# bendalab/audian

Hardware: AMD Instinct MI355X
Metric: Msamples/s spectrogram+bandpass, 64ch x 96kHz (higher is better)
Workload: dtype f32 I/O, f64 IIR state; 1 GPU; BASELINE configs[2]: synthetic 64 ch/GPU x 600 s x 96 kHz float32; bandpass 300-3000 Hz order 2 -> spectrogram nfft 2048 hop 1024 + envelope 20 Hz; channels_per_gpu=64, frames=57600000, spectrogram_frames=56250, parallelism=channel shard x1, streams=one compute stream, envelope_forward=state checkpoints, fused into the band-pass kernel, envelope_buffer=best of 4 allocations by memset time (hipdsp_malloc_probed), spectrogram=FFT waves inside the forward sweep (filtered tiles from LDS)

## Files before the change

audian_amd/_lib.py:

```python

import ctypes
import os

_HERE = os.path.dirname(os.path.abspath(__file__))
LIB_PATH = os.environ.get('AUDIAN_AMD_LIB') or os.path.join(_HERE, 'libhip_dsp.so')

OK, ERR_INVALID, ERR_HIP, ERR_UNSUPPORTED, ERR_TOO_SHORT, ERR_NOMEM = range(6)
MAX_SECTIONS = 4


class HipDspError(RuntimeError):

    def __init__(self, status, message):
        super().__init__(f'libhip_dsp error {status}: {message}')
        self.status = status


if not os.path.exists(LIB_PATH) and os.path.exists('/opt/rocm/bin/hipcc') and \
   os.environ.get('AUDIAN_AMD_NO_AUTOBUILD') != '1':
    import subprocess as _sp
    try:
        _sp.check_call(['make', '-C', os.path.join(_HERE, 'csrc'), '-j4', '-s'])
    except Exception:
        pass

if not os.path.exists(LIB_PATH):
    raise ImportError(
        f'{LIB_PATH} is missing: build the HIP extension first '
        '(`make -C audian_amd/csrc` or `python -c "import __graft_entry__ as g; g.build()"`). '
        'audian_amd has no CPU fallback.')

import sys as _sys
if 'torch' not in _sys.modules and (int(os.environ.get('WORLD_SIZE', '1')) > 1 or
                                    os.environ.get('AUDIAN_AMD_TORCH') == '1'):
    import torch as _torch

lib = ctypes.CDLL(LIB_PATH)


def hip_runtime_path():
    with open('/proc/self/maps') as f:
        return sorted({ln.split()[-1] for ln in f if 'libamdhip64' in ln})

_vp = ctypes.c_void_p
_i64 = ctypes.c_int64
_int = ctypes.c_int
_dbl = ctypes.c_double
_sz = ctypes.c_size_t
_pp = ctypes.POINTER(ctypes.c_void_p)

_SIGNATURES = {
    'hipdsp_version': ([], _int),
    'hipdsp_last_error': ([], ctypes.c_char_p),
    'hipdsp_device_count': ([ctypes.POINTER(_int)], _int),
    'hipdsp_ctx_create': ([_int, _vp, _pp], _int),
    'hipdsp_ctx_destroy': ([_vp], _int),
    'hipdsp_ctx_set_stream': ([_vp, _vp], _int),
    'hipdsp_ctx_synchronize': ([_vp], _int),
    'hipdsp_ctx_set_max_segments': ([_vp, _int], _int),
    'hipdsp_ctx_set_option': ([_vp, ctypes.c_char_p, ctypes.c_longlong], _int),
    'hipdsp_ctx_reserve': ([_vp, _sz], _int),
    'hipdsp_ctx_set_mid_event': ([_vp, _vp], _int),
    'hipdsp_stream_create': ([_vp, _pp], _int),
    'hipdsp_stream_destroy': ([_vp, _vp], _int),
    'hipdsp_graph_begin': ([_vp], _int),
    'hipdsp_graph_end': ([_vp, _pp], _int),
    'hipdsp_graph_launch': ([_vp, _vp], _int),
    'hipdsp_graph_destroy': ([_vp, _vp], _int),
    'hipdsp_malloc': ([_vp, _sz, _pp], _int),
    'hipdsp_malloc_probed': ([_vp, _sz, _int, _pp], _int),
    'hipdsp_free': ([_vp, _vp], _int),
    'hipdsp_pool_stats': ([_vp, ctypes.POINTER(_sz), ctypes.POINTER(ctypes.c_uint64), ctypes.POINTER(ctypes.c_uint64)], _int),
    'hipdsp_pool_trim': ([_vp], _int),
    'hipdsp_memset': ([_vp, _vp, _int, _sz], _int),
    'hipdsp_memcpy_h2d': ([_vp, _vp, _vp, _sz], _int),
    'hipdsp_memcpy_d2h': ([_vp, _vp, _vp, _sz], _int),
    'hipdsp_memcpy_d2d': ([_vp, _vp, _vp, _sz], _int),
    'hipdsp_host_malloc': ([_vp, _sz, _pp], _int),
    'hipdsp_host_free': ([_vp, _vp], _int),
    'hipdsp_memcpy_h2d_async': ([_vp, _vp, _vp, _sz], _int),
    'hipdsp_memcpy2d_d2d': ([_vp, _vp, _sz, _vp, _sz, _sz, _sz], _int),
    'hipdsp_event_create': ([_vp, _pp], _int),
    'hipdsp_event_destroy': ([_vp, _vp], _int),
    'hipdsp_event_record': ([_vp, _vp], _int),
    'hipdsp_event_wait': ([_vp, _vp], _int),
    'hipdsp_event_elapsed_ms': ([_vp, _vp, _vp, ctypes.POINTER(ctypes.c_float)], _int),
    'hipdsp_pack_f64': ([_vp, _vp, _vp, _i64, _i64, _i64], _int),
    'hipdsp_pack_f32': ([_vp, _vp, _vp, _i64, _i64, _i64], _int),
    'hipdsp_unpack_f64': ([_vp, _vp, _i64, _vp, _i64, _i64], _int),
    'hipdsp_unpack_spectrum_f64': ([_vp, _vp, _i64, _vp, _i64, _i64, _i64], _int),
    'hipdsp_sosplan_create': ([_vp, _pp], _int),
    'hipdsp_sosplan_destroy': ([_vp, _vp], _int),
    'hipdsp_sosplan_set': ([_vp, _vp, _vp, _int], _int),
    'hipdsp_sosplan_set_host': ([_vp, _vp, _vp, _int], _int),
    'hipdsp_sosplan_upload': ([_vp, _vp], _int),
    'hipdsp_sos_plan_host': ([_vp, _int, ctypes.POINTER(_i64), ctypes.POINTER(_int), _vp], _int),
    'hipdsp_sos_segments_host': ([_i64, _int, _int, _int, _i64, _i64, _i64, ctypes.POINTER(_i64), ctypes.POINTER(_int)], _int),
    'hipdsp_sosplan_info': ([_vp, _vp, ctypes.POINTER(_i64), ctypes.POINTER(_int)], _int),
    'hipdsp_sosfilt': ([_vp, _vp, _vp, _i64, _vp, _i64, _i64, _i64, _i64], _int),
    'hipdsp_envelope': ([_vp, _vp, _vp, _i64, _vp, _i64, _i64, _i64, _i64, _int, _dbl, _int], _int),
    'hipdsp_envelope_multi': ([_vp, _vp, _int, _vp, _i64, _vp, _i64, _i64, _i64, _i64, _int, _dbl, _int], _int),
    'hipdsp_sosfilt_envelope': ([_vp, _vp, _vp, _vp, _i64, _vp, _i64, _vp, _i64, _i64, _i64, _int, _dbl, _int, _int, _i64], _int),
    'hipdsp_chain_forward': ([_vp, _vp, _vp, _vp, _i64, _vp, _i64, _i64, _i64, _int, _dbl, _int, _int, _dbl, _vp, _vp, _i64, _i64, _i64,
                              _i64, _i64], _int),
    'hipdsp_chain_backward': ([_vp, _vp, _vp, _i64, _vp, _i64, _i64, _i64, _int, _dbl, _int, _int, _int, _dbl, _vp, _i64, _i64], _int),
    'hipdsp_chain_backward_plan': ([_vp, _vp, _i64, _i64, ctypes.POINTER(_i64), ctypes.POINTER(_i64), ctypes.POINTER(_int)], _int),
    'hipdsp_chain_plan': ([_vp, _vp, _vp, _i64, _i64, ctypes.POINTER(_i64), ctypes.POINTER(_int)], _int),
    'hipdsp_spectrogram': ([_vp, _vp, _i64, _i64, _i64, _int, _int, _dbl, _vp, _vp, _i64, _i64], _int),
    'hipdsp_decibel': ([_vp, _vp, _vp, _i64, _dbl, _dbl], _int),
    'hipdsp_decibel_image': ([_vp, _vp, _vp, _i64, _i64, _dbl, _dbl], _int),
    'hipdsp_decibel_image_decimate': ([_vp, _vp, _vp, _i64, _i64, _i64, _i64, _i64, _dbl, _dbl], _int),
    'hipdsp_channel_mean': ([_vp, _vp, _i64, ctypes.POINTER(_int), _int, _i64, _i64, _dbl, _vp], _int),
    'hipdsp_stride_copy': ([_vp, _vp, _i64, _i64, _vp], _int),
    'hipdsp_max_nonneg': ([_vp, _vp, _i64, _vp], _int),
    'hipdsp_band_order_stats': ([_vp, _vp, _i64, _i64, _i64, _i64, _vp], _int),
    'hipdsp_unwrap': ([_vp, _vp, _i64, _i64, _i64, _dbl, _dbl, _int, _int, _vp, _i64], _int),
    'hipdsp_pcm_unpack': ([_vp, _vp, _int, _i64, _i64, _dbl, _vp, _i64], _int),
    'hipdsp_minmax_decimate': ([_vp, _vp, _i64, _i64, _i64, _i64, _i64, _vp, _i64], _int),
    'hipdsp_pcm_minmax': ([_vp, _vp, _int, _i64, _i64, _i64, _dbl, _dbl, _dbl, _int, _int, _vp, _i64], _int),
    'hipdsp_mean_spectrum_db': ([_vp, _vp, _i64, _i64, _i64, _dbl, _dbl, _dbl, _vp], _int),
    'hipdsp_comm_unique_id': ([_vp], _int),
    'hipdsp_comm_create': ([_vp, _vp, _int, _int, _pp], _int),
    'hipdsp_comm_destroy': ([_vp, _vp], _int),
    'hipdsp_allgather_f32': ([_vp, _vp, _vp, _vp, _i64], _int),
    'hipdsp_copy_probe': ([_vp, _vp, _vp, _sz], _int),
    'hipdsp_synth': ([_vp, _vp, _i64, _i64, _i64, _dbl, ctypes.c_uint64, _i64, _i64], _int),
}

for _name, (_args, _res) in _SIGNATURES.items():
    _fn = getattr(lib, _name)
    _fn.argtypes = _args
    _fn.restype = _res


def last_error():
    return lib.hipdsp_last_error().decode('utf-8', 'replace')


def check(status):
    if status == OK:
        return
    msg = last_error()
    if status == ERR_TOO_SHORT:
        raise ValueError(msg)
    if status == ERR_UNSUPPORTED:
        raise NotImplementedError(msg)
    if status == ERR_NOMEM:
        raise MemoryError(msg)
    if status == ERR_INVALID:
        raise ValueError(msg)
    raise HipDspError(status, msg)
```

audian_amd/csrc/chain.hip:

```cpp
#include "chain_fwd.h"

namespace {

__global__ __launch_bounds__(256) void env_nan_fill_kernel(const double *__restrict__ ckpt, long long ckpt_pitch, long long n_tiles,
                                                           int DE, float *__restrict__ env, long long env_pitch, long long T)
{
    const long long ch = blockIdx.y;
    const double *e = ckpt + ch * ckpt_pitch + n_tiles * DE;
    bool bad = false;
    for (int r = 0; r < DE; r++) bad = bad || !(fabs(e[r]) <= 1.7976931348623157e308);
    if (!bad) return;
    for (long long i = (long long)blockIdx.x * blockDim.x + threadIdx.x; i < T; i += (long long)gridDim.x * blockDim.x)
        env[ch * env_pitch + i] = __builtin_nanf("");
}

struct ChainBwdArgs {
    BwdArgs b;
    float *psd;
    long long psd_pitch;
    long long n_valid;
    const float *tables;
    float scale;
    long long units;
    int debug;
// ... 183 lines not shown
            if (rt >= rt_lo) {
                if (tile + TILE <= T) {
#pragma unroll
                    for (int k = 0; k < 8; k++) {
                        float4 v = lds[lds_slot(8 * k + (lane >> 3), lane & 7)];
                        if (a.b.clamp) {
                            v.x = fmaxf(v.x, 0.f); v.y = fmaxf(v.y, 0.f); v.z = fmaxf(v.z, 0.f); v.w = fmaxf(v.w, 0.f);
                        }
                        f4u t; t.x = v.x; t.y = v.y; t.z = v.z; t.w = v.w;
                        *reinterpret_cast<f4u *>(out + (tile + 256 * k + 4 * lane)) = t;
                    }
                    asm volatile("s_waitcnt vmcnt(7)" ::: "memory");
                } else {
#pragma unroll
                    for (int k = 0; k < 8; k++) {
                        float4 v = lds[lds_slot(8 * k + (lane >> 3), lane & 7)];
                        if (a.b.clamp) {
                            v.x = fmaxf(v.x, 0.f); v.y = fmaxf(v.y, 0.f); v.z = fmaxf(v.z, 0.f); v.w = fmaxf(v.w, 0.f);
                        }
                        store_four(out, tile + 256 * k + 4 * lane, v, 0, T, 0);
                    }
                    asm volatile("s_waitcnt vmcnt(0)" ::: "memory");
                }
            } else {
                asm volatile("s_waitcnt vmcnt(0)" ::: "memory");
            }
            WAVE_SYNC();
        }
        asm volatile("s_waitcnt vmcnt(0)" ::: "memory");
    } else {
        __builtin_amdgcn_s_setprio(3);
        float2 *fb = fbs[pair];
        const float *tlf = reinterpret_cast<const float *>(tiles[pair]);
        const float2 *tw2 = tab, *tw3 = tab + TW2, *twn = tab + TW2 + TW3, *win = tab + TW2 + TW3 + TWN;
        float *oc = a.psd + ch * a.psd_pitch;
        v2f cur_[16], nxt_[8];
#pragma unroll
        for (int j = 0; j < 16; j++) cur_[j] = (v2f){0.f, 0.f};
#pragma unroll
        for (int j = 0; j < 8; j++) nxt_[j] = (v2f){0.f, 0.f};
        bool have_next = false;
        float piv = 0.f;
        bool have_piv = false;
        int it = 0;
        for (long long rt = rt_start; rt < rt_hi; rt++) {
            it++;
            const long long tidx = a.b.n_tiles - 1 - rt;
            CHAIN_WAIT_FOR(ready, it, it);
#pragma unroll
            for (int j = 0; j < 16; j++)
                cur_[j] = *reinterpret_cast<const v2f *>(tlf + lds_float_index(2 * lane + 128 * j));
            {
                const bool withhold = (a.debug & 8) && blockIdx.x == 0 && pair == 0 && rt == rt_start;
                if (!withhold) CHAIN_POST(taken, it);
            }
            const long long f = 2 * tidx + 1;
            if (rt >= rt_lo && have_next && f < a.n_valid) {
                v2f w[16];
#pragma unroll
                for (int i = 0; i < 8; i++) { w[i] = cur_[8 + i]; w[8 + i] = nxt_[i]; }
                psd_frame_pivot<NFFT, 64, R1, R2, R3, false>(w, fb, tw2, tw3, twn, win, lane, PsdScale{a.scale, 0.5f * a.scale, 2.f * a.scale}, true,
                                                             bin_sink<false>(oc + f * (long long)F, nullptr, 0), piv, have_piv);
            }
#pragma unroll
            for (int j = 0; j < 8; j++) nxt_[j] = cur_[j];
            have_next = true;
        }
    }
}

#undef CHAIN_WAIT_FOR
#undef CHAIN_POST
#undef CHAIN_FAIR

}

extern "C" {

int hipdsp_chain_forward(hipdsp_ctx *ctx, const hipdsp_sosplan *fplan, const hipdsp_sosplan *eplan,
                         const float *x, int64_t x_pitch, float *yf, int64_t yf_pitch, int64_t channels,
                         int64_t frames, int rectify, double gain, int nfft, int hop, double fs, float *psd,
                         float *db_out, int64_t frames_out, int64_t psd_pitch, int64_t spec_frames,
                         int64_t spec_first, int64_t env_first)
{
    HD_REQUIRE(ctx != nullptr && fplan != nullptr, "NULL argument");
    HD_REQUIRE(channels >= 0 && frames >= 0 && frames_out >= 0, "negative size");
    HD_REQUIRE(frames_out < (1LL << 31) - (1LL << 16), "frames_out %lld: the fused sweep counts frames in 32 bits", (long long)frames_out);
    HD_REQUIRE(spec_first >= 0 && spec_first <= frames, "spec_first %lld not in [0, frames=%lld]", (long long)spec_first,
               (long long)frames);
    HD_REQUIRE(spec_frames >= 0 && spec_first + spec_frames <= frames, "spec_first %lld + spec_frames %lld beyond frames=%lld",
               (long long)spec_first, (long long)spec_frames, (long long)frames);
    HD_REQUIRE(env_first >= 0 && env_first <= frames, "env_first %lld not in [0, frames=%lld]", (long long)env_first,
               (long long)frames);
    HD_REQUIRE(fs > 0, "fs must be positive");
    const int SF = fplan->host->n_sections, SE = eplan ? eplan->host->n_sections : 0;
    HD_REQUIRE(SF > 0 && (SE > 0 || eplan == nullptr), "plan has no coefficients");
    const bool shape_ok = (nfft == 2048 && (hop == 1024 || hop == 512)) || (nfft == 1024 && (hop == 512 || hop == 256)) ||
                          (nfft == 512 && hop == 256) || (nfft == 256 && hop == 128);
    if (!shape_ok || SF > 4 || SE > 2 || frames < 4 * TILE ||
        fplan->host->warm >= (1LL << 40) || (eplan && eplan->host->warm >= (1LL << 40))) {
        hipdsp_set_error("the fused forward sweep covers nfft/hop 2048/1024, 2048/512, 1024/512, 1024/256, 512/256 and 256/128, a band-pass of "
                         "at most four and an envelope of at most two sections that decay, and traces of at least %d "
                         "frames: use hipdsp_sosfilt_envelope + hipdsp_spectrogram", 4 * TILE);
        return HIPDSP_ERR_UNSUPPORTED;
    }
    HD_CHECK_HIP(hipSetDevice(ctx->device));
    {
        const int frc = hd_device_fault(ctx);
        if (frc != HIPDSP_OK) return frc;
    }
    const int edge = eplan ? eplan->host->edge : 0;
    if (eplan && frames - env_first <= edge) {
        hipdsp_set_error("The length of the input vector x must be greater than padlen, which is %d.", edge);
        return HIPDSP_ERR_TOO_SHORT;
    }
    if (channels == 0) return HIPDSP_OK;
    HD_REQUIRE(channels <= 65535, "more than 65535 channels");
    HD_REQUIRE(x != nullptr && yf != nullptr && (psd != nullptr || frames_out == 0), "NULL data pointer");
    HD_REQUIRE(x_pitch >= frames && yf_pitch >= frames, "pitch smaller than row length");
    HD_NO_OVERLAP(x, x_pitch, frames, yf, yf_pitch, frames, channels, "x and yf");
    const long long F = nfft / 2 + 1;
    if (psd_pitch == 0) psd_pitch = frames_out * F;
    HD_REQUIRE(psd_pitch >= frames_out * F, "psd_pitch smaller than one channel");
    const long long sframes = spec_frames > 0 ? spec_frames : frames - spec_first;
    long long nsource = (frames_out - 1) * (long long)hop + nfft;
    if (nsource > sframes) nsource = sframes;
    long long n_valid = 0;
    if (frames_out > 0 && nsource >= nfft) n_valid = (nsource - (nfft - hop)) / hop;
    if (n_valid > frames_out) n_valid = frames_out;
    double wss = 0.0;
    for (int i = 0; i < nfft; i++) {
        const double w = 0.5 - 0.5 * cos(2.0 * M_PI * (double)i / (double)nfft);
        wss += w * w;
    }
    ChainArgs a;
    memset(&a, 0, sizeof(a));
    int rc = hd_fft_tables(ctx, nfft, &a.tables);
    if (rc != HIPDSP_OK) return rc;
    const GridShift gs = hd_grid_shift(spec_first, env_first, hop, edge, SE > 0);
    HD_REQUIRE(gs.lead < TILE, "grid shift %lld", gs.lead);
    const long long T = frames + gs.lead;
    const long long n_tiles = (T + edge + TILE - 1) / TILE;
    const long long ckpt_pitch = (n_tiles + 1) * 2 * SE;
    void *work = nullptr;
    if (SE > 0) {
        rc = hipdsp_scratch(ctx, sizeof(double) * (size_t)ckpt_pitch * (size_t)channels, &work);
        if (rc != HIPDSP_OK) return rc;
    }
    hd_note_sweep(ctx, gs.lead, gs.env0, frames, channels, SE);
    a.c.in = x - gs.lead; a.c.yf = yf - gs.lead; a.c.ckpt = (double *)work;
    a.c.in_pitch = x_pitch; a.c.yf_pitch = yf_pitch; a.c.ckpt_pitch = ckpt_pitch;
    a.c.T = T; a.c.edge = edge; a.c.rectify = rectify; a.c.gain = rectify ? gain : 1.0;
    a.c.lead = gs.lead; a.c.env0 = gs.env0; a.frame_off = gs.frame_off;
    a.psd = psd; a.db = db_out; a.psd_pitch = psd_pitch; a.n_valid = n_valid;
    a.scale = (float)(1.0 / (fs * wss));
    a.scale_half = 0.5f * a.scale; a.scale_twice = 2.f * a.scale;
    a.warm_total = fplan->host->warm;
    a.debug = ctx->chain_debug;
    a.fault = ctx->fault_dev;
    a.split = (ctx->chain_split_frames && nfft == 2048 && hop == 1024 && !db_out && gs.lead == 0 && gs.env0 == 0) ? 1 : 0;
    constexpr int P = CHAIN_P;
    plan_segments_chain(ctx, T, channels, a.warm_total, &a.c.seg_len, &a.c.n_seg);
    a.units = channels * a.c.n_seg;
    if (a.c.n_seg > 1) {
        rc = hd_seg_flags(ctx, (size_t)a.units, &a.c.flags);
        if (rc != HIPDSP_OK) return rc;
    }
    a.n_iter = (int)((a.warm_total + a.c.seg_len + edge + TILE - 1) / TILE) + 1;
    long long blocks = (a.units + P - 1) / P;
    {
        const long long cus = ctx->n_cus - ctx->chain_reserve_cus > 0 ? ctx->n_cus - ctx->chain_reserve_cus : 1;
        if (a.units < cus * P) {
            blocks = a.units < cus ? a.units : cus;
            a.unit_stride = blocks;
        }
    }
    HD_REQUIRE(blocks <= 0x7fffffffLL, "grid too large");
    if (frames_out > n_valid && frames_out - n_valid <= 16 && !(ctx->chain_debug & 32)) {
        a.tail_end = frames_out;
    } else if (frames_out > n_valid) {
        const long long n = (frames_out - n_valid) * F;
        unsigned gx = (unsigned)((n + 1023) / 1024 > 4096 ? 4096 : (n + 1023) / 1024);
        hipLaunchKernelGGL(zero_rows_kernel, dim3(gx, (unsigned)channels), dim3(256), 0, ctx->stream,
                           psd + n_valid * F, (long long)psd_pitch, n, 0.f);
        if (db_out && !(ctx->chain_debug & 32))
            hipLaunchKernelGGL(zero_rows_kernel, dim3(gx, (unsigned)channels), dim3(256), 0, ctx->stream,
                               db_out + n_valid * F, (long long)psd_pitch, n, -INFINITY);
    }
    const SosPlanDev *edev_ = eplan ? eplan->dev : nullptr;
    const bool flags = (ctx->chain_debug & 4) == 0;
    const bool stamp = (ctx->chain_debug & 32) && db_out && SF == 2 && SE == 1 && flags && nfft == 2048 && hop == 1024;
    int (*launch)(int, int, int, int, int, unsigned, hipStream_t, const SosPlanDev *, const SosPlanDev *, const void *, size_t) =
        (nfft == 2048 && hop == 1024) ? hd_chain_fwd_launch_2048_1024 : (nfft == 2048) ? hd_chain_fwd_launch_2048_512 :
        (nfft == 1024 && hop == 512) ? hd_chain_fwd_launch_1024_512 : (nfft == 1024) ? hd_chain_fwd_launch_1024_256 :
        (nfft == 512) ? hd_chain_fwd_launch_512_256 : hd_chain_fwd_launch_256_128;
    if (launch(SF, SE, flags ? 1 : 0, (db_out && !stamp) ? 1 : 0, stamp ? 1 : 0, (unsigned)blocks, ctx->stream, fplan->dev, edev_,
               &a, sizeof(a)) != 0) {
        hipdsp_set_error("the barrier variant of the fused sweep is built for nfft 2048 / hop 1024 and plans of one or two sections");
        return HIPDSP_ERR_UNSUPPORTED;
    }
    if (stamp) return hd_launch_status("chain_fwd_kernel");
    rc = hd_launch_status("chain_fwd_kernel");
    if (rc != HIPDSP_OK) return rc;
    FloodArgs fl;
    memset(&fl, 0, sizeof(fl));
    fl.flags = a.c.flags; fl.n_seg = a.c.n_seg; fl.seg_len = a.c.seg_len;
    fl.y = yf; fl.y_pitch = yf_pitch; fl.T = T; fl.skip = gs.lead;
    fl.psd = psd; fl.db = db_out; fl.psd_pitch = psd_pitch; fl.n_valid = n_valid;
    fl.F = (int)F; fl.nfft = nfft; fl.hop = hop; fl.frame_off = gs.frame_off;
    if (SE == 0) return launch_flood(ctx, fl, channels);
    return hd_launch_env_fix(ctx, eplan->dev, SE, (double *)work, ckpt_pitch, channels, a.c.n_seg, a.c.seg_len, n_tiles, &fl,
                             (int)((gs.env0 - gs.env0 % TILE) / a.c.seg_len));
}

int hipdsp_chain_backward(hipdsp_ctx *ctx, const hipdsp_sosplan *eplan, const float *yf, int64_t yf_pitch, float *env,
                          int64_t env_pitch, int64_t channels, int64_t frames, int rectify, double gain, int clamp,
                          int nfft, int hop, double fs, float *psd, int64_t frames_out, int64_t psd_pitch)
{
    HD_REQUIRE(ctx != nullptr && eplan != nullptr, "NULL argument");
    HD_REQUIRE(channels >= 0 && frames >= 0 && frames_out >= 0, "negative size");
    HD_REQUIRE(fs > 0, "fs must be positive");
    const int SE = eplan->host->n_sections;
    HD_REQUIRE(SE > 0, "plan has no coefficients");
    if (nfft != 2048 || hop != 1024 || SE > 2 || frames < 4 * TILE || eplan->host->warm >= (1LL << 40)) {
        hipdsp_set_error("the backward sweep with the odd frames fused in covers nfft 2048 / hop 1024, envelope plans of at "
                         "most two decaying sections and traces of at least %d frames", 4 * TILE);
        return HIPDSP_ERR_UNSUPPORTED;
    }
    HD_CHECK_HIP(hipSetDevice(ctx->device));
    {
        const int frc = hd_device_fault(ctx);
        if (frc != HIPDSP_OK) return frc;
    }
    const int edge = eplan->host->edge;
    if (frames <= edge) {
        hipdsp_set_error("The length of the input vector x must be greater than padlen, which is %d.", edge);
        return HIPDSP_ERR_TOO_SHORT;
    }
    if (channels == 0) return HIPDSP_OK;
    HD_REQUIRE(channels <= 65535, "more than 65535 channels");
    HD_REQUIRE(yf != nullptr && env != nullptr && (psd != nullptr || frames_out == 0), "NULL data pointer");
    HD_REQUIRE(yf_pitch >= frames && env_pitch >= frames, "pitch smaller than row length");
    HD_NO_OVERLAP(yf, yf_pitch, frames, env, env_pitch, frames, channels, "yf and env");
    const long long F = nfft / 2 + 1;
    if (psd_pitch == 0) psd_pitch = frames_out * F;
    HD_REQUIRE(psd_pitch >= frames_out * F, "psd_pitch smaller than one channel");
    long long nsource = (frames_out - 1) * (long long)hop + nfft;
    if (nsource > frames) nsource = frames;
    long long n_valid = 0;
    if (frames_out > 0 && nsource >= nfft) n_valid = (nsource - (nfft - hop)) / hop;
    if (n_valid > frames_out) n_valid = frames_out;
    double wss = 0.0;
    for (int i = 0; i < nfft; i++) {
        const double w = 0.5 - 0.5 * cos(2.0 * M_PI * (double)i / (double)nfft);
        wss += w * w;
    }
    ChainBwdArgs a;
    memset(&a, 0, sizeof(a));
    int rc = hd_fft_tables(ctx, nfft, &a.tables);
    if (rc != HIPDSP_OK) return rc;
    const long long n_tiles = (frames + edge + TILE - 1) / TILE;
    const long long ckpt_pitch = (n_tiles + 1) * 2 * SE;
    void *work = nullptr;
    if (ctx->sweep_frames != frames || ctx->sweep_channels != channels || ctx->sweep_sections != SE ||
        ctx->sweep_lead != 0 || ctx->sweep_env0 != 0) {
        hipdsp_set_error("hipdsp_chain_backward: the last forward sweep on this context left tile states for %lld channels x "
                         "%lld frames, %d sections, grid shift %lld, envelope from %lld -- not for %lld x %lld, %d on the "
                         "unshifted grid (hipdsp_chain_forward with spec_first = env_first = 0)",
                         ctx->sweep_channels, ctx->sweep_frames, ctx->sweep_sections, ctx->sweep_lead, ctx->sweep_env0,
                         (long long)channels, (long long)frames, SE);
        return HIPDSP_ERR_INVALID;
    }
    rc = hd_scratch_parked(ctx, sizeof(double) * (size_t)ckpt_pitch * (size_t)channels, &work);
    if (rc != HIPDSP_OK) return rc;
    a.b.in = yf; a.b.in_pitch = yf_pitch;
    a.b.out = env; a.b.out_pitch = env_pitch;
    a.b.ckpt = (const double *)work; a.b.ckpt_pitch = ckpt_pitch;
    a.b.T = frames; a.b.skip = 0; a.b.n_tiles = n_tiles; a.b.edge = edge;
    a.b.rectify = rectify; a.b.clamp = clamp; a.b.gain = rectify ? gain : 1.0;
    constexpr int P = 8;
    long long seg_len = 0;
    plan_segments_chain(ctx, n_tiles * TILE, channels, eplan->host->warm, &seg_len, &a.b.n_seg);
    a.b.seg_tiles = seg_len / TILE;
    a.b.warm_tiles = eplan->host->warm / TILE;
    a.psd = psd; a.psd_pitch = psd_pitch; a.n_valid = n_valid;
    a.scale = (float)(1.0 / (fs * wss));
    a.units = channels * a.b.n_seg;
    a.debug = ctx->chain_debug;
    a.fault = ctx->fault_dev;
    const long long blocks = (a.units + P - 1) / P;
    HD_REQUIRE(blocks <= 0x7fffffffLL, "grid too large");
    dim3 grid((unsigned)blocks), block(128 * P);
    if (SE == 1) hipLaunchKernelGGL((chain_bwd_kernel<1, P>), grid, block, 0, ctx->stream, eplan->dev, a);
    else hipLaunchKernelGGL((chain_bwd_kernel<2, P>), grid, block, 0, ctx->stream, eplan->dev, a);
    rc = hd_launch_status("chain_bwd_kernel");
    if (rc != HIPDSP_OK) return rc;
    hipLaunchKernelGGL(env_nan_fill_kernel, dim3(64, (unsigned)channels), dim3(256), 0, ctx->stream, (const double *)work,
                       ckpt_pitch, n_tiles, 2 * SE, env, (long long)env_pitch, (long long)frames);
    return hd_launch_status("env_nan_fill_kernel");
}

int hipdsp_chain_backward_plan(hipdsp_ctx *ctx, const hipdsp_sosplan *eplan, int64_t channels, int64_t frames,
                               int64_t *first_border, int64_t *segment_frames, int *n_segments)
{
    HD_REQUIRE(ctx != nullptr && eplan != nullptr, "NULL argument");
    HD_REQUIRE(first_border != nullptr && segment_frames != nullptr && n_segments != nullptr, "NULL output");
    HD_REQUIRE(channels >= 1 && frames >= 1, "bad size");
    HD_REQUIRE(eplan->host->n_sections > 0, "plan has no coefficients");
    const long long n_tiles = (frames + eplan->host->edge + TILE - 1) / TILE;
    long long len = 0;
    int n = 0;
    plan_segments_chain(ctx, n_tiles * TILE, channels, eplan->host->warm, &len, &n);
    *first_border = n_tiles * TILE - len;
    *segment_frames = len;
    *n_segments = n;
    return HIPDSP_OK;
}

int hipdsp_chain_plan(hipdsp_ctx *ctx, const hipdsp_sosplan *fplan, const hipdsp_sosplan *eplan,
                      int64_t channels, int64_t frames, int64_t *segment_frames, int *n_segments)
{
    HD_REQUIRE(ctx != nullptr && fplan != nullptr, "NULL argument");
    HD_REQUIRE(segment_frames != nullptr && n_segments != nullptr, "NULL output");
    HD_REQUIRE(channels >= 1 && frames >= 1, "bad size");
    HD_REQUIRE(fplan->host->n_sections > 0 && (eplan == nullptr || eplan->host->n_sections > 0), "plan has no coefficients");
    long long len = 0;
    int n = 0;
    plan_segments_chain(ctx, frames, channels, fplan->host->warm, &len, &n);
    *segment_frames = len;
    *n_segments = n;
    return HIPDSP_OK;
}

}
```

audian_amd/csrc/chain_fwd.h:

```cpp
#pragma once
#include "sos_device.h"
#define STOCKHAM_SPLIT_MORE
#include "fft_device.h"
#include <cmath>

#define HD_CHAIN_FWD_DECL(n, h)                                                                                     \
    int hd_chain_fwd_launch_##n##_##h(int SF, int SE, int flags, int want_db, int stamp, unsigned blocks, hipStream_t stream, \
                                      const SosPlanDev *fdev, const SosPlanDev *edev, const void *args, size_t args_size)
HD_CHAIN_FWD_DECL(2048, 1024);
HD_CHAIN_FWD_DECL(2048, 512);
HD_CHAIN_FWD_DECL(1024, 512);
HD_CHAIN_FWD_DECL(1024, 256);
HD_CHAIN_FWD_DECL(512, 256);
HD_CHAIN_FWD_DECL(256, 128);
#undef HD_CHAIN_FWD_DECL

#ifdef CHAIN_AB_PLAIN_SUM
#define CHAIN_MSUM_ADD(x) do { } while (0)
#define CHAIN_MSUM_ON false
#else
#define CHAIN_MSUM_ADD(x) msum_ += (x)
#define CHAIN_MSUM_ON true
#endif

// ... 231 lines not shown
        const float pv = (l == 0) ? ph : pk_last;
        if (LPF == 64 || keep) {
            st_bin(out.psd, bo_h, 0, pv);
            if (DB) st_bin(out.db, bo_h, 0, to_db(pv));
        }
    }
}

#define FPT_OK(hop, g) ((2048 / (hop)) % (g) == 0)
#ifndef CHAIN_FFT_STORES
#define CHAIN_FFT_STORES 1
#endif
template <int SF, int SE, int NP, bool FLAGS, bool DB, int NFFT = 2048, int HOP = 1024, bool STAMP = false>
__global__ __launch_bounds__(128 * NP, NP / 2) void chain_fwd_kernel(const SosPlanDev *__restrict__ PF0,
                                                                   const SosPlanDev *__restrict__ PE0, ChainArgs a)
{
    static_assert(SF > 0 && SE >= 0 && NP % 2 == 0, "band-pass in front; whole waves per SIMD");
    constexpr int DF = 2 * SF, DE = SE > 0 ? 2 * SE : 1;
    static_assert((NFFT == 2048 || NFFT == 1024 || NFFT == 512 || NFFT == 256) && TILE % HOP == 0 && HOP % 128 == 0 &&
                  HOP <= NFFT && NFFT <= TILE, "frames must be register windows of a tile");
    static_assert(NFFT != 256 || HOP == 128, "256-sample frames: the reference's default, 50 % overlap");
    constexpr int M = NFFT / 2, F = M + 1, MP = M + M / 16;
    constexpr int LPF = NFFT >= 1024 ? 64 : (NFFT == 512 ? 32 : 16);
    constexpr int G = 64 / LPF;
    constexpr int R1 = NFFT == 2048 ? 16 : 8, R2 = NFFT == 256 ? 4 : R1, R3 = NFFT == 1024 ? 8 : 4;
    constexpr int TW2 = (R2 - 1) * R1, TW3 = R1 * R2, TWN = M / 2 + 1, NTAB = TW2 + TW3 + TWN + M;
    constexpr int PPL = NFFT / 128;
    static_assert(FPT_OK(HOP, G), "whole groups of frames per tile");
    constexpr int FPT = TILE / HOP;
    constexpr int PREV = (NFFT - HOP) / 128;
    constexpr bool FFT_STORES = CHAIN_FFT_STORES && FLAGS && G != 4;
    __shared__ float4 tiles[NP][64 * 8];
    __shared__ float rprevs[NP][64];
    __shared__ float2 fbs[NP][G * MP];
    __shared__ float2 tab[NTAB];
    __shared__ int ready[NP], taken[NP];
    __shared__ float2 fmeans[2][NP][16];
    __shared__ int prog[2 * NP];
    if (threadIdx.x < NP) { ready[threadIdx.x] = 0; taken[threadIdx.x] = 0; }
    if (threadIdx.x < 2 * NP) prog[threadIdx.x] = 0;
    const int tid = threadIdx.x;
    const int wave = __builtin_amdgcn_readfirstlane(tid >> 6);
    const int lane = tid & 63;
    const int pair = wave < NP ? wave : wave - NP;
#define CHAIN_FAIR(iter, behind_prio, ahead_prio)                                                        \
    do {                                                                                                 \
        if (FLAGS && !(a.debug & 128)) {                                                                 \
            if (lane == 0) __hip_atomic_store(&prog[wave], (iter), __ATOMIC_RELAXED, __HIP_MEMORY_SCOPE_WORKGROUP); \
            const int other_ = __builtin_amdgcn_readfirstlane(                                           \
                __hip_atomic_load(&prog[wave ^ (NP / 2)], __ATOMIC_RELAXED, __HIP_MEMORY_SCOPE_WORKGROUP)); \
            set_issue_priority(other_ < (iter) ? (ahead_prio) : (behind_prio));                          \
        }                                                                                                \
    } while (0)
    __shared__ int abort_wg;
    if (threadIdx.x == 0) abort_wg = 0;
    bool gave_up = false;
#define CHAIN_WAIT_FOR(arr, want, iter)                                             \
    do {                                                                            \
        if (!gave_up) {                                                             \
            for (int spin_ = 0;; spin_++) {                                         \
                if (__builtin_amdgcn_readfirstlane(__hip_atomic_load(&arr[pair], __ATOMIC_RELAXED, __HIP_MEMORY_SCOPE_WORKGROUP)) >= (want)) break; \
                if ((spin_ & 1023) == 1023) {                                       \
                    const bool told = __builtin_amdgcn_readfirstlane(__hip_atomic_load(&abort_wg, __ATOMIC_RELAXED, __HIP_MEMORY_SCOPE_WORKGROUP)) != 0; \
                    if (told || spin_ >= (1 << 23) - 1) {                           \
                        gave_up = true;                                             \
                        if (!told && lane == 0) {                                   \
                            __hip_atomic_store(&abort_wg, 1, __ATOMIC_RELAXED, __HIP_MEMORY_SCOPE_WORKGROUP); \
                            a.fault[1] = (int)blockIdx.x; a.fault[2] = pair; a.fault[3] = (iter); \
                            __hip_atomic_store(&a.fault[0], HD_FAULT_CHAIN_HANDOVER, __ATOMIC_RELEASE, __HIP_MEMORY_SCOPE_SYSTEM); \
                        }                                                           \
                        break;                                                      \
                    }                                                               \
                }                                                                   \
                __builtin_amdgcn_s_sleep(1);                                        \
            }                                                                       \
            __builtin_amdgcn_fence(__ATOMIC_ACQUIRE, "workgroup", "local");        \
        }                                                                           \
    } while (0)
#define CHAIN_POST(arr, value)                                                      \
    do {                                                                            \
        __builtin_amdgcn_fence(__ATOMIC_RELEASE, "workgroup", "local");            \
        if (lane == 0) __hip_atomic_store(&arr[pair], (value), __ATOMIC_RELAXED, __HIP_MEMORY_SCOPE_WORKGROUP); \
    } while (0)
    {
        const float2 *src = reinterpret_cast<const float2 *>(a.tables);
        for (int i = tid; i < NTAB; i += 128 * NP) tab[i] = src[i];
    }
    __syncthreads();

    const long long unit = a.unit_stride ? (long long)pair * a.unit_stride + blockIdx.x : (long long)blockIdx.x * NP + pair;
    const bool unit_ok = unit < a.units;
    const int seg = unit_ok ? (int)(unit % a.c.n_seg) : 0;
    const long long ch = unit_ok ? unit / a.c.n_seg : 0;
    const long long T = a.c.T;
    const int edge = a.c.edge;
    const long long lo = (long long)seg * a.c.seg_len;
    long long hi = lo + a.c.seg_len;
    const bool last_seg = hi >= T;
    if (hi > T) hi = T;
    const long long lead = a.c.lead;
    const long long env_tile0 = a.c.env0 - a.c.env0 % TILE;
    const bool env_true = lo <= env_tile0 && env_tile0 < hi;
    const long long env_start = env_true ? env_tile0 : (lo > env_tile0 ? lo : (1LL << 62));
    long long start = lo - PF0->warm;
    if (start < 0) start = 0;
    long long loop_end = last_seg ? T + edge : hi;
    if (!unit_ok) loop_end = start;
    const int TT = (int)(T / TILE);
    const int lo_t = (int)(lo / TILE), start_t = (int)(start / TILE), base_t = lo_t - (int)(a.warm_total / TILE);
    const int end_t = (int)((loop_end + TILE - 1) / TILE);
    const int hi_full_t = (int)(hi / TILE), hi_ceil_t = (int)((hi + TILE - 1) / TILE);
    const int lead_t = lead > 0 ? 1 : 0;
    const int env_start_t = env_start >= (1LL << 62) ? 0x7fffffff : (int)(env_start / TILE);

    const long long dbg_c0 = (a.debug & 16) ? clock64() : 0, dbg_w0 = (a.debug & 16) ? wall_clock64() : 0;
    long long st_acc[16];
#pragma unroll
    for (int i = 0; i < 16; i++) st_acc[i] = 0;
    long long st_last = STAMP ? clock64() : 0;
#define STAMP_AT(i)                                              \
    do {                                                         \
        if (STAMP) {                                             \
            const long long t_ = clock64();                      \
            st_acc[(i)] += t_ - st_last;                         \
            st_last = t_;                                        \
        }                                                        \
    } while (0)
    if (wave < NP) {
        float4 *lds = tiles[pair];
        float *ldsf = reinterpret_cast<float *>(lds);
        float *rprev = rprevs[pair];
        const float *in = a.c.in + ch * a.c.in_pitch;
        float *yf = a.c.yf + ch * a.c.yf_pitch;
        double *ckpt = SE > 0 ? a.c.ckpt + ch * a.c.ckpt_pitch : nullptr;
        double cf_[DF], ce_[DE];
#pragma unroll
        for (int r = 0; r < DF; r++) cf_[r] = 0.0;
#pragma unroll
        for (int r = 0; r < DE; r++) ce_[r] = 0.0;
        rprev[lane] = 0.f;
        double eprev_ = 0.0;
        v4f nx[8];
        bool pre = false;
        int pending = 0;
        const int top_full_t = TT - 1;
        auto fetch = [&](int t0) {
#pragma unroll
            for (int k = 0; k < 8; k++) nx[k] = asm_load16(in + (long long)t0 * TILE + 256 * k + 4 * lane);
        };
        auto prefetchable = [&](int t0) { return t0 >= start_t && t0 < end_t && t0 < TT && t0 >= lead_t; };
        pre = prefetchable(base_t);
        fetch(pre ? base_t : top_full_t);
        asm volatile("s_waitcnt vmcnt(0)" ::: "memory");

        for (int it = 0; it < a.n_iter; it++) {
            const int tt = base_t + it;
            const bool active = tt >= start_t && tt < end_t;
            if (!(a.debug & 64)) CHAIN_FAIR(it, 1, 0);
            if (FLAGS && pending) {
                CHAIN_WAIT_FOR(taken, pending, it);
                pending = 0;
            }
            if (active) {
                if (pre) {
#pragma unroll
                    for (int k = 0; k < 8; k++) {
                        asm volatile("" : "+v"(nx[k]));
                        lds[lds_slot(8 * k + (lane >> 3), lane & 7)] = make_float4(nx[k].x, nx[k].y, nx[k].z, nx[k].w);
                    }
                } else {
                    const long long tile = (long long)tt * TILE;
#pragma unroll 1
                    for (int k = 0; k < 8; k++) {
                        const long long p = tile + 256 * k + 4 * lane;
                        auto at = [&](long long q) { return in + (q < lead ? lead : (q < T ? q : T - 1)); };
                        auto ok = [&](long long q) { return q >= lead && q < T; };
                        v4f t;
                        t.x = asm_load4(at(p));
                        t.y = asm_load4(at(p + 1));
                        t.z = asm_load4(at(p + 2));
                        t.w = asm_load4(at(p + 3));
                        asm volatile("s_waitcnt vmcnt(0)" ::: "memory");
                        asm volatile("" : "+v"(t));
                        lds[lds_slot(8 * k + (lane >> 3), lane & 7)] =
                            make_float4(ok(p) ? t.x : 0.f, ok(p + 1) ? t.y : 0.f, ok(p + 2) ? t.z : 0.f, ok(p + 3) ? t.w : 0.f);
                    }
                }
            }
            WAVE_SYNC();
            {
                const int next = tt + 1;
                pre = prefetchable(next);
                fetch(pre ? next : top_full_t);
            }
            STAMP_AT(0);
            double etap[DE];
#pragma unroll
            for (int r = 0; r < DE; r++) etap[r] = 0.0;
            double msum_ = 0.0;
            if (active && !(a.debug & 2)) {
                const double tgain = a.c.gain;
                const SosPlanDev *PEt = PLAN_OF(SE > 0 ? PE0 : PF0);
#define CASC_S SF
#define CASC_PLAN() PLAN_OF(PF0)
#define CASC_CARRY cf_
#define CASC_IN(v) (v)
#define CASC_ROLLED_GROUPS
#define CASC_UNIT_OK (SF <= 2)
#define CASC_STAMP(n) STAMP_AT(1 + (n))
#define CASC_TAP(j, e, y)                                                               \
    do {                                                                                \
        const double ed_ = (double)(e);                                                 \
        CHAIN_MSUM_ADD(ed_);                                                            \
        if constexpr (SE > 0) {                                                         \
            if (((j) & 3) == 0) PEt = PLAN_OF(PE0);                                     \
            const double rd_ = fabs(ed_);                                               \
            _Pragma("unroll") for (int r_ = 0; r_ < DE; r_++) etap[r_] = fma(PEt->G[(j) * DE + r_], rd_, etap[r_]); \
        }                                                                               \
    } while (0)
#include "sos_cascade.inc"
#undef CASC_TAP
#undef CASC_STAMP
#undef CASC_UNIT_OK
#undef CASC_ROLLED_GROUPS
#undef CASC_S
#undef CASC_PLAN
#undef CASC_CARRY
#undef CASC_IN
#pragma unroll
                for (int r = 0; r < DE; r++) etap[r] *= tgain;
            }
            if (active && CHAIN_MSUM_ON) {
                constexpr int LR = NFFT / 32, HR = HOP / 32;
                const double pfx = wave_prefix_sum(msum_);
                const double tot = wave_read_lane63(pfx);
                const double yrot = (LR == 64 || lane >= 64 - LR) ? eprev_ : pfx;
                const double xrot = LR == 64 ? yrot : __shfl(yrot, (lane - LR) & 63, 64);
                const double mean = (pfx - xrot) * (1.0 / (double)NFFT);
                eprev_ = pfx - tot;
                const float mhi = (float)mean;
                const float mcorr = (float)((mean - (double)mhi) * (0.5 * (double)NFFT));
                if (((lane + 1) & (HR - 1)) == 0) fmeans[it & 1][pair][(lane + 1) / HR - 1] = make_float2(mhi, mcorr);
            }
            WAVE_SYNC();
            if (FLAGS) { if (active) CHAIN_POST(ready, it + 1); }
            else __syncthreads();
            if (FFT_STORES && active && tt >= lo_t && tt < hi_full_t && tt >= lead_t) {
                asm volatile("s_waitcnt vmcnt(0)" ::: "memory");
                STAMP_AT(4);
            } else if (active && tt >= lo_t && tt < hi_full_t && tt >= lead_t) {
#pragma unroll
                for (int k = 0; k < 8; k++) {
                    const float4 v = lds[lds_slot(8 * k + (lane >> 3), lane & 7)];
                    f4u t; t.x = v.x; t.y = v.y; t.z = v.z; t.w = v.w;
                    *reinterpret_cast<f4u *>(yf + (long long)tt * TILE + 256 * k + 4 * lane) = t;
                }
                asm volatile("s_waitcnt vmcnt(7)" ::: "memory");
                STAMP_AT(4);
            } else {
                if (active && tt >= lo_t && tt < hi_ceil_t) {
                    const long long tile = (long long)tt * TILE;
#pragma unroll
                    for (int k = 0; k < 8; k++)
                        store_four(yf, tile + 256 * k + 4 * lane, lds[lds_slot(8 * k + (lane >> 3), lane & 7)],
                                   lo > lead ? lo : lead, hi, 0);
                }
                asm volatile("s_waitcnt vmcnt(0)" ::: "memory");
            }
            const bool last_tile = tt + 1 >= end_t;
            const bool quiet = SE > 0 && active && tt >= env_start_t && a.c.rectify && tt + 1 < TT &&
                               !(env_true && tt == env_start_t) && (!last_tile || !last_seg) && !(a.debug & 2);
            if (FLAGS) {
                if (active) {
                    if (quiet || SE == 0 || tt < env_start_t) pending = it + 1;
                    else CHAIN_WAIT_FOR(taken, it + 1, it);
                }
            } else {
                __syncthreads();
            }
            if constexpr (SE > 0) {
            if (quiet) {
                if ((tt > lo_t || env_true) && lane == 0) {
#pragma unroll
                    for (int r = 0; r < DE; r++) ckpt[(long long)tt * DE + r] = ce_[r];
                }
#define CASC_S SE
#define CASC_PLAN() PLAN_OF(PE0)
#define CASC_CARRY ce_
#define CASC_IN(v) (v)
#define CASC_F_IN etap
#define CASC_NO_OUTPUT
#define CASC_ROLLED_GROUPS
#define CASC_STAMP(n) STAMP_AT(5 + (n))
#include "sos_cascade.inc"
#undef CASC_STAMP
#undef CASC_ROLLED_GROUPS
#undef CASC_NO_OUTPUT
#undef CASC_F_IN
#undef CASC_S
#undef CASC_PLAN
#undef CASC_CARRY
#undef CASC_IN
                if (last_tile && lane == 0) {
#pragma unroll
                    for (int r = 0; r < DE; r++) ckpt[(long long)(tt + 1) * DE + r] = ce_[r];
                }
                WAVE_SYNC();
            } else if (active && tt >= env_start_t && !(a.debug & 2)) {
                const long long tile = (long long)tt * TILE;
                if (a.c.rectify) {
#pragma unroll
                    for (int q = 0; q < 8; q++) {
                        float4 v = lds[lds_slot(lane, q)];
                        v = make_float4(fabsf(v.x), fabsf(v.y), fabsf(v.z), fabsf(v.w));
                        lds[lds_slot(lane, q)] = v;
                    }
                }
                WAVE_SYNC();
                auto rval = [&](long long j) -> float {
                    return j >= tile ? ldsf[lds_float_index((int)(j - tile))] : rprev[64 - (int)(tile - j)];
                };
                if (tt >= TT) {
                    float pv = 0.f;
                    long long pj = -1;
                    if (lane < edge) {
                        pj = T + lane;
                        if (pj >= tile && pj < tile + TILE) pv = 2.f * rval(T - 1) - rval(T - 2 - lane);
                    }
                    WAVE_SYNC();
                    if (lane < edge && pj >= tile && pj < tile + TILE) ldsf[lds_float_index((int)(pj - tile))] = pv;
                    WAVE_SYNC();
                }
                if (env_true && tt == env_start_t && a.c.env0 > 0) {
                    const SosPlanDev *Pz = PLAN_OF(PE0);
                    const float e0 = env_left_fill(ldsf, lane, (int)(a.c.env0 - tile), edge);
                    const double x0 = a.c.gain * (double)e0;
#pragma unroll
                    for (int r = 0; r < DE; r++) ce_[r] = Pz->zi[r] * x0;
                } else if (env_true && tt == env_start_t) {
                    const SosPlanDev *Pz = PLAN_OF(PE0);
                    const double r0 = (double)ldsf[lds_float_index(0)];
                    const double x0 = a.c.gain * (2.0 * r0 - (double)ldsf[lds_float_index(edge)]);
#pragma unroll
                    for (int r = 0; r < DE; r++) ce_[r] = Pz->zi[r] * x0;
                    for (int i = 0; i < edge; i++) {
                        double cur = a.c.gain * (2.0 * r0 - (double)ldsf[lds_float_index(edge - i)]);
#pragma unroll
                        for (int s2 = 0; s2 < SE; s2++) {
                            const double y = fma(Pz->coef[s2][0], cur, ce_[2 * s2]);
                            ce_[2 * s2] = fma(-Pz->coef[s2][3], y, fma(Pz->coef[s2][1], cur, ce_[2 * s2 + 1]));
                            ce_[2 * s2 + 1] = fma(-Pz->coef[s2][4], y, Pz->coef[s2][2] * cur);
                            cur = y;
                        }
                    }
                }
                if ((tt > lo_t || env_true) && lane == 0) {
#pragma unroll
                    for (int r = 0; r < DE; r++) ckpt[(long long)tt * DE + r] = ce_[r];
                }
                {
                    {
                        const float4 keep0 = lds[lds_slot(62 + ((lane >> 3) & 1), lane & 7)];
                        WAVE_SYNC();
                        if (lane < 16) {
                            rprev[4 * lane] = keep0.x; rprev[4 * lane + 1] = keep0.y;
                            rprev[4 * lane + 2] = keep0.z; rprev[4 * lane + 3] = keep0.w;
                        }
                    }
#define CASC_S SE
#define CASC_PLAN() PLAN_OF(PE0)
#define CASC_CARRY ce_
#define CASC_IN(v) (v)
#define CASC_GAIN a.c.gain
#define CASC_NO_OUTPUT
#define CASC_ROLLED_GROUPS
#include "sos_cascade.inc"
#undef CASC_ROLLED_GROUPS
#undef CASC_NO_OUTPUT
#undef CASC_GAIN
#undef CASC_S
#undef CASC_PLAN
#undef CASC_CARRY
#undef CASC_IN
                    if (last_tile && lane == 0) {
#pragma unroll
                        for (int r = 0; r < DE; r++) ckpt[(long long)(tt + 1) * DE + r] = ce_[r];
                    }
                }
                WAVE_SYNC();
            }
            }
        }
        asm volatile("s_waitcnt vmcnt(0)" ::: "memory");
        if (unit_ok && a.c.flags != nullptr && lane == 0) a.c.flags[unit] = state_not_finite(cf_) ? 1 : 0;
        STAMP_AT(7);
        if ((a.debug & 16) && blockIdx.x == 0 && wave == 0 && lane == 0) {
            long long *dbg = reinterpret_cast<long long *>(a.psd);
            dbg[0] = clock64() - dbg_c0;
            dbg[1] = wall_clock64() - dbg_w0;
        }
    } else {
        PsdScale fscale = {a.scale, a.scale_half, a.scale_twice};
        int foff = a.frame_off, fsplit = a.split, fdebug = a.debug, n_iter = a.n_iter;
        int nvalid = (int)a.n_valid;
        asm volatile("" : "+s"(fscale.one), "+s"(fscale.half), "+s"(fscale.twice), "+s"(foff), "+s"(fsplit), "+s"(fdebug),
                     "+s"(n_iter), "+s"(nvalid));
        if (!(fdebug & 64)) __builtin_amdgcn_s_setprio(3);
        float2 *fb = fbs[pair];
        const float *tlf = reinterpret_cast<const float *>(tiles[pair]);
        const float2 *tw2 = tab, *tw3 = tab + TW2, *twn = tab + TW2 + TW3, *win = tab + TW2 + TW3 + TWN;
        float *oc = a.psd + ch * a.psd_pitch;
        float *dc = DB ? a.db + ch * a.psd_pitch : nullptr;
        float *yfc = a.c.yf + ch * a.c.yf_pitch;
        const int st_lo_t = lo_t > lead_t ? lo_t : lead_t;
        v2f cur_[16], prv_[PREV > 0 ? PREV : 1];
#pragma unroll
        for (int j = 0; j < 16; j++) cur_[j] = (v2f){0.f, 0.f};
#pragma unroll
        for (int j = 0; j < (PREV > 0 ? PREV : 1); j++) prv_[j] = (v2f){0.f, 0.f};
        v2f bb_[G == 4 ? 20 : 1], pv_[4];
#pragma unroll
        for (int j = 0; j < 4; j++) pv_[j] = (v2f){0.f, 0.f};
        bool have_prev = false;
        for (int it = 0; it < n_iter; it++) {
            const int tt = base_t + it;
            const bool active = tt >= start_t && tt < end_t;
            if (!(fdebug & 64)) CHAIN_FAIR(it, 3, 2);
            if (FLAGS) { if (active) CHAIN_WAIT_FOR(ready, it + 1, it); }
            else __syncthreads();
            STAMP_AT(8);
            if (active) {
                if constexpr (G == 4) {
                    const int gq = lane >> 4, l16 = lane & 15;
#pragma unroll
                    for (int j = 0; j < 5; j++)
#pragma unroll
                        for (int tq = 0; tq < 4; tq++) {
                            const int b = 4 * gq - 1 + j;
// ... 119 lines not shown
```

audian_amd/csrc/common.h:

```cpp
#pragma once
#include <hip/hip_runtime.h>
#include <cstdarg>
#include <cstdint>
#include <cstdio>
#include <cstring>
#include "../../include/hip_dsp.h"

void hipdsp_set_error(const char *fmt, ...);

struct hipdsp_ctx {
    int device;
    hipStream_t stream;
    int max_segments;
    int n_cus;
    void *scratch;
    size_t scratch_bytes;
    hipEvent_t mid_event;
    void *fft_tables[20];
    int force_generic_fft;
    void *fft_tables2[20];
    int sos_waves_per_cu;
    int sos_waves_min;
    int chain_pairs;
    int sos_debug;
    int sos_single_wave_wg;
    int sos_prefetch;
    int spec_no_half;
    int spec_fpw, spec_kernel;
    int spec_debug;
    int chain_debug;
    int chain_split_frames;
    int chain_reserve_cus;
    long long *sos_trace;
    long long sos_trace_rows;
    int sos_fair;
    int sos_split;
    int sos_no_pin;
    struct hd_pool *pool;
    volatile int *fault_host;
    int *fault_dev;
    int graphs_alive;
    unsigned char *seg_flags;
    size_t seg_flags_cap;
    long long sweep_lead, sweep_env0, sweep_frames, sweep_channels;
    int sweep_sections;
};

int hd_seg_flags(hipdsp_ctx *ctx, size_t units, unsigned char **out);

#define HD_FAULT_CHAIN_HANDOVER 1
#define HD_FAULT_SPLIT_HANDOVER 2

int hd_device_fault(hipdsp_ctx *ctx);

struct hipdsp_graph {
    hipGraph_t graph;
    hipGraphExec_t exec;
};

#define HD_CHECK_HIP(expr)                                                        \
    do {                                                                          \
        hipError_t _e = (expr);                                                   \
        if (_e != hipSuccess) {                                                   \
            hipdsp_set_error("%s failed: %s (%s:%d)", #expr, hipGetErrorString(_e), \
                             __FILE__, __LINE__);                                 \
            return HIPDSP_ERR_HIP;                                                \
        }                                                                         \
    } while (0)

#define HD_REQUIRE(cond, ...)                                                     \
    do {                                                                          \
        if (!(cond)) {                                                            \
            hipdsp_set_error(__VA_ARGS__);                                        \
            return HIPDSP_ERR_INVALID;                                            \
        }                                                                         \
    } while (0)

static inline int hd_launch_status(const char *what)
{
    hipError_t e = hipGetLastError();
    if (e != hipSuccess) {
        hipdsp_set_error("launch of %s failed: %s", what, hipGetErrorString(e));
        return HIPDSP_ERR_HIP;
    }
    return HIPDSP_OK;
}

static inline bool hd_planar_overlap(const float *a, long long a_pitch, long long a_frames, const float *b, long long b_pitch,
                                     long long b_frames, long long channels)
{
    if (a == nullptr || b == nullptr || channels <= 0 || a_frames <= 0 || b_frames <= 0) return false;
    const char *a0 = (const char *)a, *a1 = (const char *)(a + (channels - 1) * a_pitch + a_frames);
    const char *b0 = (const char *)b, *b1 = (const char *)(b + (channels - 1) * b_pitch + b_frames);
    return a0 < b1 && b0 < a1;
}
#define HD_NO_OVERLAP(a, ap, af, b, bp, bf, channels, what)                                             \
    HD_REQUIRE(!hd_planar_overlap((a), (ap), (af), (b), (bp), (bf), (channels)), what " must not overlap")

int hipdsp_scratch(hipdsp_ctx *ctx, size_t bytes, void **out);
int hd_scratch_parked(hipdsp_ctx *ctx, size_t bytes, void **out);
int hd_fft_tables(hipdsp_ctx *ctx, int nfft, const float **dev);
```

audian_amd/csrc/ctx.hip:

```cpp
#include "common.h"
#include <map>
#include <unordered_map>
#include <vector>

static thread_local char g_err[512] = "";

struct hd_block {
    void *ptr;
    hipStream_t stream;
    hipEvent_t freed;
};

struct hd_pool {
    std::multimap<size_t, hd_block> cached;
    std::unordered_map<void *, size_t> live;
    std::vector<hipEvent_t> spare_events;
    size_t cached_bytes = 0;
    size_t limit = (size_t)1 << 30;
    size_t max_block = (size_t)256 << 20;
    unsigned long long hits = 0, misses = 0;
};

static void pool_trim(hd_pool *p)
{
    for (auto &kv : p->cached) {
        (void)hipFree(kv.second.ptr);
        if (kv.second.freed) p->spare_events.push_back(kv.second.freed);
    }
    p->cached.clear();
    p->cached_bytes = 0;
}

static void pool_destroy_events(hd_pool *p)
{
    for (hipEvent_t e : p->spare_events) (void)hipEventDestroy(e);
    p->spare_events.clear();
}

void hipdsp_set_error(const char *fmt, ...)
{
    va_list ap;
    va_start(ap, fmt);
    vsnprintf(g_err, sizeof(g_err), fmt, ap);
    va_end(ap);
}

extern "C" {

int hipdsp_version(void) { return HIPDSP_VERSION; }

const char *hipdsp_last_error(void) { return g_err; }

int hipdsp_device_count(int *count)
{
    HD_REQUIRE(count != nullptr, "count is NULL");
    HD_CHECK_HIP(hipGetDeviceCount(count));
    return HIPDSP_OK;
}

int hipdsp_ctx_create(int device, void *stream, hipdsp_ctx **out)
{
    HD_REQUIRE(out != nullptr, "out is NULL");
    *out = nullptr;
    int n = 0;
    HD_CHECK_HIP(hipGetDeviceCount(&n));
    HD_REQUIRE(device >= 0 && device < n, "device %d out of range (%d devices)", device, n);
    HD_CHECK_HIP(hipSetDevice(device));
    hipDeviceProp_t prop;
    HD_CHECK_HIP(hipGetDeviceProperties(&prop, device));
    if (strncmp(prop.gcnArchName, "gfx950", 6) != 0) {
        hipdsp_set_error("device %d is %s; libhip_dsp is built for gfx950 (MI355X) only",
                         device, prop.gcnArchName);
        return HIPDSP_ERR_UNSUPPORTED;
    }
    hipdsp_ctx *ctx = new hipdsp_ctx();
    ctx->device = device;
    ctx->stream = (hipStream_t)stream;
    ctx->max_segments = 0;
    ctx->n_cus = prop.multiProcessorCount;
    ctx->scratch = nullptr;
    ctx->scratch_bytes = 0;
    ctx->mid_event = nullptr;
    for (int i = 0; i < 20; i++) ctx->fft_tables[i] = nullptr;
    ctx->force_generic_fft = 0;
    ctx->spec_fpw = ctx->spec_kernel = 0;
    ctx->chain_debug = 0;
    ctx->sos_no_pin = 0;
    ctx->sos_trace = nullptr;
    ctx->sos_fair = 0;
    ctx->chain_reserve_cus = 0;
    ctx->chain_split_frames = 0;
    ctx->sos_waves_per_cu = 0;
    ctx->sos_waves_min = 0;
    ctx->sos_trace_rows = 0;
    ctx->sos_single_wave_wg = 0;
    ctx->sos_debug = 0;
    ctx->chain_pairs = 0;
    ctx->spec_no_half = 0;
    ctx->pool = new hd_pool();
    ctx->sos_prefetch = 1;
    for (int i = 0; i < 20; i++) ctx->fft_tables2[i] = nullptr;
    ctx->fault_host = nullptr;
    ctx->fault_dev = nullptr;
    ctx->graphs_alive = 0;
    ctx->seg_flags = nullptr;
    ctx->seg_flags_cap = 0;
    {
        void *h = nullptr, *d = nullptr;
        hipError_t e = hipHostMalloc(&h, 64, hipHostMallocMapped);
        if (e == hipSuccess) {
            memset(h, 0, 64);
            e = hipHostGetDevicePointer(&d, h, 0);
        }
        if (e != hipSuccess) {
            if (h) (void)hipHostFree(h);
            delete ctx->pool;
            delete ctx;
            HD_CHECK_HIP(e);
        }
        ctx->fault_host = (volatile int *)h;
        ctx->fault_dev = (int *)d;
    }
    {
        void *f = nullptr;
        const hipError_t e = hipMalloc(&f, (size_t)1 << 20);
        if (e != hipSuccess) {
            (void)hipHostFree((void *)ctx->fault_host);
            delete ctx->pool;
            delete ctx;
            HD_CHECK_HIP(e);
        }
        ctx->seg_flags = (unsigned char *)f;
        ctx->seg_flags_cap = (size_t)1 << 20;
    }
    *out = ctx;
    return HIPDSP_OK;
}

int hipdsp_ctx_destroy(hipdsp_ctx *ctx)
{
    if (!ctx) return HIPDSP_OK;
    if (ctx->pool) {
        pool_trim(ctx->pool);
        pool_destroy_events(ctx->pool);
        delete ctx->pool;
    }
    if (ctx->scratch) (void)hipFree(ctx->scratch);
    if (ctx->seg_flags) (void)hipFree(ctx->seg_flags);
    if (ctx->fault_host) (void)hipHostFree((void *)ctx->fault_host);
    for (int i = 0; i < 20; i++)
        if (ctx->fft_tables[i]) (void)hipFree(ctx->fft_tables[i]);
    for (int i = 0; i < 20; i++)
        if (ctx->fft_tables2[i]) (void)hipFree(ctx->fft_tables2[i]);
    delete ctx;
    return HIPDSP_OK;
}

int hipdsp_ctx_set_stream(hipdsp_ctx *ctx, void *stream)
{
    HD_REQUIRE(ctx != nullptr, "ctx is NULL");
    ctx->stream = (hipStream_t)stream;
    return HIPDSP_OK;
}

int hipdsp_ctx_synchronize(hipdsp_ctx *ctx)
{
    HD_REQUIRE(ctx != nullptr, "ctx is NULL");
    HD_CHECK_HIP(hipStreamSynchronize(ctx->stream));
    return hd_device_fault(ctx);
}

int hipdsp_ctx_set_max_segments(hipdsp_ctx *ctx, int max_segments)
{
    HD_REQUIRE(ctx != nullptr, "ctx is NULL");
    HD_REQUIRE(max_segments >= 0, "max_segments must be >= 0");
    ctx->max_segments = max_segments;
    return HIPDSP_OK;
}

int hipdsp_ctx_set_option(hipdsp_ctx *ctx, const char *name, long long value)
{
    HD_REQUIRE(ctx != nullptr && name != nullptr, "NULL argument");
    if (strcmp(name, "max_segments") == 0) return hipdsp_ctx_set_max_segments(ctx, (int)value);
    if (strcmp(name, "force_generic_fft") == 0) { ctx->force_generic_fft = value != 0; return HIPDSP_OK; }
    if (strcmp(name, "spec_fpw") == 0) { ctx->spec_fpw = (int)value; return HIPDSP_OK; }
    if (strcmp(name, "sos_waves_per_cu") == 0) { ctx->sos_waves_per_cu = (int)value; return HIPDSP_OK; }
    if (strcmp(name, "sos_waves_min") == 0) { ctx->sos_waves_min = (int)value; return HIPDSP_OK; }
    if (strcmp(name, "chain_pairs") == 0) {
        HD_REQUIRE(value >= 0 && value <= 8, "chain_pairs %lld not in [0, 8]", value);
        ctx->chain_pairs = (int)value;
        return HIPDSP_OK;
    }
    if (strcmp(name, "sos_debug") == 0) { ctx->sos_debug = (int)value; return HIPDSP_OK; }
    if (strcmp(name, "sos_single_wave_wg") == 0) { ctx->sos_single_wave_wg = value != 0; return HIPDSP_OK; }
    if (strcmp(name, "sos_prefetch") == 0) { ctx->sos_prefetch = value != 0; return HIPDSP_OK; }
    if (strcmp(name, "pool_limit_mb") == 0) {
        HD_REQUIRE(value >= 0, "pool_limit_mb must be >= 0");
        ctx->pool->limit = (size_t)value << 20;
        ctx->pool->max_block = ctx->pool->limit > ((size_t)256 << 20) ? ctx->pool->limit : ((size_t)256 << 20);
        if (ctx->pool->cached_bytes > ctx->pool->limit) {
            HD_CHECK_HIP(hipStreamSynchronize(ctx->stream));
            pool_trim(ctx->pool);
        }
        return HIPDSP_OK;
    }
    if (strcmp(name, "spec_no_half") == 0) { ctx->spec_no_half = value != 0; return HIPDSP_OK; }
    if (strcmp(name, "spec_kernel") == 0) { ctx->spec_kernel = (int)value; return HIPDSP_OK; }
    if (strcmp(name, "spec_debug") == 0) { ctx->spec_debug = (int)value; return HIPDSP_OK; }
    if (strcmp(name, "chain_debug") == 0) { ctx->chain_debug = (int)value; return HIPDSP_OK; }
    if (strcmp(name, "sos_no_pin") == 0) { ctx->sos_no_pin = value != 0; return HIPDSP_OK; }
    if (strcmp(name, "sos_split") == 0) {
#ifdef HIPDSP_WITH_ENVSPLIT
        ctx->sos_split = value != 0;
        return HIPDSP_OK;
#else
        if (value == 0) return HIPDSP_OK;
        hipdsp_set_error("\"sos_split\": this library was built without envsplit.hip (make SPLIT=1)");
        return HIPDSP_ERR_UNSUPPORTED;
#endif
    }
    if (strcmp(name, "sos_fair") == 0) { ctx->sos_fair = value != 0; return HIPDSP_OK; }
    if (strcmp(name, "sos_trace_rows") == 0) { ctx->sos_trace_rows = value; return HIPDSP_OK; }
    if (strcmp(name, "sos_trace") == 0) {
        HD_REQUIRE(value == 0 || ctx->sos_trace_rows > 0, "set \"sos_trace_rows\" (capacity of the buffer in rows of 9 int64) first");
        ctx->sos_trace = reinterpret_cast<long long *>((uintptr_t)value);
        return HIPDSP_OK;
    }
    if (strcmp(name, "chain_split_frames") == 0) { ctx->chain_split_frames = value != 0; return HIPDSP_OK; }
    if (strcmp(name, "chain_reserve_cus") == 0) {
        HD_REQUIRE(value >= 0 && value < ctx->n_cus, "chain_reserve_cus %lld not in [0, %d)", value, ctx->n_cus);
        ctx->chain_reserve_cus = (int)value;
        return HIPDSP_OK;
    }
    if (strcmp(name, "n_cus") == 0) {
        HD_REQUIRE(value >= 1 && value <= 1024, "n_cus out of range");
        HD_REQUIRE(value > ctx->chain_reserve_cus, "n_cus %lld would leave no CU beside the %d of \"chain_reserve_cus\"", value,
                   ctx->chain_reserve_cus);
        ctx->n_cus = (int)value;
        return HIPDSP_OK;
    }
    hipdsp_set_error("unknown option '%s'", name);
    return HIPDSP_ERR_INVALID;
}

int hipdsp_ctx_set_mid_event(hipdsp_ctx *ctx, void *event)
{
    HD_REQUIRE(ctx != nullptr, "ctx is NULL");
    ctx->mid_event = (hipEvent_t)event;
    return HIPDSP_OK;
}

int hipdsp_ctx_reserve(hipdsp_ctx *ctx, size_t bytes)
{
    void *p;
    return hipdsp_scratch(ctx, bytes, &p);
}

int hipdsp_malloc(hipdsp_ctx *ctx, size_t bytes, void **dptr)
{
    HD_REQUIRE(ctx != nullptr && dptr != nullptr, "NULL argument");
    *dptr = nullptr;
    if (bytes == 0) return HIPDSP_OK;
    HD_CHECK_HIP(hipSetDevice(ctx->device));
    hd_pool *p = ctx->pool;
    const size_t want = (bytes + 511) & ~(size_t)511;
    hipStreamCaptureStatus capturing = hipStreamCaptureStatusNone;
    if (ctx->stream) (void)hipStreamIsCapturing(ctx->stream, &capturing);
    auto it = p->cached.lower_bound(want);
    while (it != p->cached.end() && it->first <= want + want / 4 + 4096 && it->second.stream != ctx->stream &&
           (it->second.freed == nullptr || capturing != hipStreamCaptureStatusNone))
        ++it;
    if (it != p->cached.end() && it->first <= want + want / 4 + 4096) {
        const hd_block b = it->second;
        if (b.freed) {
            if (b.stream != ctx->stream) HD_CHECK_HIP(hipStreamWaitEvent(ctx->stream, b.freed, 0));
            p->spare_events.push_back(b.freed);
        }
        *dptr = b.ptr;
        p->live[*dptr] = it->first;
        p->cached_bytes -= it->first;
        p->cached.erase(it);
        p->hits++;
        return HIPDSP_OK;
    }
    hipError_t e = hipMalloc(dptr, want);
    if (e == hipErrorOutOfMemory && !p->cached.empty()) {
        (void)hipGetLastError();
        pool_trim(p);
        e = hipMalloc(dptr, want);
    }
    if (e == hipErrorOutOfMemory) {
        (void)hipGetLastError();
        hipdsp_set_error("hipMalloc(%zu bytes) out of memory", bytes);
        return HIPDSP_ERR_NOMEM;
    }
    HD_CHECK_HIP(e);
    p->live[*dptr] = want;
    p->misses++;
    return HIPDSP_OK;
}

int hipdsp_malloc_probed(hipdsp_ctx *ctx, size_t bytes, int tries, void **dptr)
{
    HD_REQUIRE(ctx != nullptr && dptr != nullptr, "NULL argument");
    *dptr = nullptr;
    hipStreamCaptureStatus capturing = hipStreamCaptureStatusNone;
    if (ctx->stream) (void)hipStreamIsCapturing(ctx->stream, &capturing);
    if (tries > 8) tries = 8;
    if (tries <= 1 || bytes < ((size_t)64 << 20) || capturing != hipStreamCaptureStatusNone) return hipdsp_malloc(ctx, bytes, dptr);
    void *cand[8];
    float ms[8];
    int n = 0;
    for (; n < tries; n++) {
        const int rc = hipdsp_malloc(ctx, bytes, &cand[n]);
        if (rc != HIPDSP_OK) {
            if (n == 0) return rc;
            (void)hipGetLastError();
            break;
        }
    }
    hipEvent_t e0 = nullptr, e1 = nullptr;
    hipError_t e = hipEventCreate(&e0);
    if (e == hipSuccess) e = hipEventCreate(&e1);
    int best = 0;
    if (e == hipSuccess) {
        for (int i = 0; i < n && e == hipSuccess; i++) {
            e = hipMemsetAsync(cand[i], 0, bytes, ctx->stream);
            if (e == hipSuccess) e = hipEventRecord(e0, ctx->stream);
            for (int k = 0; k < 3 && e == hipSuccess; k++) e = hipMemsetAsync(cand[i], 0, bytes, ctx->stream);
            if (e == hipSuccess) e = hipEventRecord(e1, ctx->stream);
            if (e == hipSuccess) e = hipEventSynchronize(e1);
            ms[i] = 0.f;
            if (e == hipSuccess) e = hipEventElapsedTime(&ms[i], e0, e1);
            if (e == hipSuccess && ms[i] < ms[best]) best = i;
        }
    }
    if (e0) (void)hipEventDestroy(e0);
    if (e1) (void)hipEventDestroy(e1);
    for (int i = 0; i < n; i++)
        if (i != best) (void)hipdsp_free(ctx, cand[i]);
    if (e != hipSuccess) {
        (void)hipdsp_free(ctx, cand[best]);
        HD_CHECK_HIP(e);
    }
    *dptr = cand[best];
    return HIPDSP_OK;
}

int hipdsp_free(hipdsp_ctx *ctx, void *dptr)
{
    HD_REQUIRE(ctx != nullptr, "ctx is NULL");
    if (!dptr) return HIPDSP_OK;
    hd_pool *p = ctx->pool;
    auto it = p->live.find(dptr);
    if (it == p->live.end()) {
        HD_CHECK_HIP(hipFree(dptr));
        return HIPDSP_OK;
    }
    const size_t size = it->second;
    p->live.erase(it);
    if (size <= p->max_block && p->cached_bytes + size <= p->limit) {
        hd_block b{dptr, ctx->stream, nullptr};
        hipStreamCaptureStatus st = hipStreamCaptureStatusNone;
        if (ctx->stream) (void)hipStreamIsCapturing(ctx->stream, &st);
        if (st == hipStreamCaptureStatusNone) {
            hipError_t e = hipSuccess;
            if (!p->spare_events.empty()) {
                b.freed = p->spare_events.back();
                p->spare_events.pop_back();
            } else {
                e = hipEventCreateWithFlags(&b.freed, hipEventDisableTiming);
                if (e != hipSuccess) b.freed = nullptr;
            }
// ... 119 lines not shown
int hipdsp_stream_create(hipdsp_ctx *ctx, void **stream)
{
    HD_REQUIRE(ctx != nullptr && stream != nullptr, "NULL argument");
    HD_CHECK_HIP(hipSetDevice(ctx->device));
    hipStream_t s;
    HD_CHECK_HIP(hipStreamCreateWithFlags(&s, hipStreamNonBlocking));
    *stream = (void *)s;
    return HIPDSP_OK;
}

int hipdsp_stream_destroy(hipdsp_ctx *ctx, void *stream)
{
    HD_REQUIRE(ctx != nullptr, "ctx is NULL");
    if (stream) {
        if (ctx->stream == (hipStream_t)stream) ctx->stream = nullptr;
        HD_CHECK_HIP(hipStreamDestroy((hipStream_t)stream));
    }
    return HIPDSP_OK;
}

int hipdsp_graph_begin(hipdsp_ctx *ctx)
{
    HD_REQUIRE(ctx != nullptr, "ctx is NULL");
    HD_REQUIRE(ctx->stream != nullptr, "stream capture needs a non-default stream "
               "(hipdsp_stream_create + hipdsp_ctx_set_stream)");
    HD_CHECK_HIP(hipSetDevice(ctx->device));
    HD_CHECK_HIP(hipStreamBeginCapture(ctx->stream, hipStreamCaptureModeThreadLocal));
    return HIPDSP_OK;
}

int hipdsp_graph_end(hipdsp_ctx *ctx, hipdsp_graph **out)
{
    HD_REQUIRE(ctx != nullptr && out != nullptr, "NULL argument");
    *out = nullptr;
    hipGraph_t g = nullptr;
    HD_CHECK_HIP(hipStreamEndCapture(ctx->stream, &g));
    hipGraphExec_t exec = nullptr;
    hipError_t e = hipGraphInstantiate(&exec, g, nullptr, nullptr, 0);
    if (e != hipSuccess) {
        (void)hipGraphDestroy(g);
        HD_CHECK_HIP(e);
    }
    hipdsp_graph *h = new hipdsp_graph();
    h->graph = g;
    h->exec = exec;
    ctx->graphs_alive++;
    *out = h;
    return HIPDSP_OK;
}

int hipdsp_graph_launch(hipdsp_ctx *ctx, hipdsp_graph *graph)
{
    HD_REQUIRE(ctx != nullptr && graph != nullptr, "NULL argument");
    HD_CHECK_HIP(hipGraphLaunch(graph->exec, ctx->stream));
    return HIPDSP_OK;
}

int hipdsp_graph_destroy(hipdsp_ctx *ctx, hipdsp_graph *graph)
{
    HD_REQUIRE(ctx != nullptr, "ctx is NULL");
    if (graph) {
        (void)hipGraphExecDestroy(graph->exec);
        (void)hipGraphDestroy(graph->graph);
        delete graph;
        if (ctx->graphs_alive > 0) ctx->graphs_alive--;
    }
    return HIPDSP_OK;
}

int hipdsp_event_create(hipdsp_ctx *ctx, void **event)
{
    HD_REQUIRE(ctx != nullptr && event != nullptr, "NULL argument");
    hipEvent_t ev;
    HD_CHECK_HIP(hipEventCreate(&ev));
    *event = (void *)ev;
    return HIPDSP_OK;
}

int hipdsp_event_destroy(hipdsp_ctx *ctx, void *event)
{
    HD_REQUIRE(ctx != nullptr, "ctx is NULL");
    if (event) HD_CHECK_HIP(hipEventDestroy((hipEvent_t)event));
    return HIPDSP_OK;
}

int hipdsp_event_record(hipdsp_ctx *ctx, void *event)
{
    HD_REQUIRE(ctx != nullptr && event != nullptr, "NULL argument");
    HD_CHECK_HIP(hipEventRecord((hipEvent_t)event, ctx->stream));
    return HIPDSP_OK;
}

int hipdsp_event_wait(hipdsp_ctx *ctx, void *event)
{
    HD_REQUIRE(ctx != nullptr && event != nullptr, "NULL argument");
    HD_CHECK_HIP(hipStreamWaitEvent(ctx->stream, (hipEvent_t)event, 0));
    return HIPDSP_OK;
}

int hipdsp_event_elapsed_ms(hipdsp_ctx *ctx, void *start, void *stop, float *ms)
{
    HD_REQUIRE(ctx != nullptr && start && stop && ms, "NULL argument");
    HD_CHECK_HIP(hipEventSynchronize((hipEvent_t)stop));
    HD_CHECK_HIP(hipEventElapsedTime(ms, (hipEvent_t)start, (hipEvent_t)stop));
    return hd_device_fault(ctx);
}

}

int hd_device_fault(hipdsp_ctx *ctx)
{
    if (!ctx || !ctx->fault_host) return HIPDSP_OK;
    const int code = ctx->fault_host[0];
    if (code == 0) return HIPDSP_OK;
    const int a = ctx->fault_host[1], b = ctx->fault_host[2], c = ctx->fault_host[3];
    ctx->fault_host[0] = 0;
    if (code == HD_FAULT_CHAIN_HANDOVER)
        hipdsp_set_error("chain_fwd_kernel: a wave of workgroup %d (pair %d) gave up waiting for its partner's "
                         "LDS hand-over in iteration %d; the outputs of that launch are invalid", a, b, c);
    else
        hipdsp_set_error("a kernel reported device fault %d (%d, %d, %d)", code, a, b, c);
    return HIPDSP_ERR_HIP;
}

int hd_seg_flags(hipdsp_ctx *ctx, size_t units, unsigned char **out)
{
    if (units > ctx->seg_flags_cap) {
        hipStreamCaptureStatus st = hipStreamCaptureStatusNone;
        if (ctx->stream) (void)hipStreamIsCapturing(ctx->stream, &st);
        if (st != hipStreamCaptureStatusNone || ctx->graphs_alive > 0) {
            hipdsp_set_error("a sweep of %zu (channel, segment) units during a stream capture or next to captured graphs of "
                             "this context: run one of that size once before capturing", units);
            return HIPDSP_ERR_INVALID;
        }
        HD_CHECK_HIP(hipStreamSynchronize(ctx->stream));
        if (ctx->seg_flags) HD_CHECK_HIP(hipFree(ctx->seg_flags));
        ctx->seg_flags = nullptr;
        ctx->seg_flags_cap = 0;
        void *f = nullptr;
        const hipError_t e = hipMalloc(&f, units);
        if (e == hipErrorOutOfMemory) {
            (void)hipGetLastError();
            hipdsp_set_error("hipMalloc(%zu bytes) for the segment flags: out of memory", units);
            return HIPDSP_ERR_NOMEM;
        }
        HD_CHECK_HIP(e);
        ctx->seg_flags = (unsigned char *)f;
        ctx->seg_flags_cap = units;
    }
    *out = ctx->seg_flags;
    return HIPDSP_OK;
}

int hd_scratch_parked(hipdsp_ctx *ctx, size_t bytes, void **out)
{
    HD_REQUIRE(ctx != nullptr && out != nullptr, "NULL argument");
    if (ctx->sweep_frames < 0 || ctx->scratch == nullptr || bytes > ctx->scratch_bytes) {
        hipdsp_set_error("no forward sweep's tile states are parked in this context's scratch (another call has used the "
                         "scratch since, or none has run): run the forward sweep again");
        return HIPDSP_ERR_INVALID;
    }
    *out = ctx->scratch;
    return HIPDSP_OK;
}

int hipdsp_scratch(hipdsp_ctx *ctx, size_t bytes, void **out)
{
    HD_REQUIRE(ctx != nullptr && out != nullptr, "NULL argument");
    ctx->sweep_frames = -1;
    if (bytes > ctx->scratch_bytes) {
        hipStreamCaptureStatus st = hipStreamCaptureStatusNone;
        if (ctx->stream) (void)hipStreamIsCapturing(ctx->stream, &st);
        if (st != hipStreamCaptureStatusNone) {
            hipdsp_set_error("scratch of %zu bytes needed during stream capture; call "
                             "hipdsp_ctx_reserve() before capturing", bytes);
            return HIPDSP_ERR_INVALID;
        }
        if (ctx->scratch && ctx->graphs_alive > 0) {
            hipdsp_set_error("scratch would have to grow from %zu to %zu bytes while %d captured graph(s) of this "
                             "context still point into it; hipdsp_ctx_reserve() the largest size before capturing",
                             ctx->scratch_bytes, bytes, ctx->graphs_alive);
            return HIPDSP_ERR_INVALID;
        }
        HD_CHECK_HIP(hipStreamSynchronize(ctx->stream));
        if (ctx->scratch) HD_CHECK_HIP(hipFree(ctx->scratch));
        ctx->scratch = nullptr;
        ctx->scratch_bytes = 0;
        hipError_t e = hipMalloc(&ctx->scratch, bytes);
        if (e == hipErrorOutOfMemory) {
            (void)hipGetLastError();
            hipdsp_set_error("scratch hipMalloc(%zu bytes) out of memory", bytes);
            return HIPDSP_ERR_NOMEM;
        }
        HD_CHECK_HIP(e);
        ctx->scratch_bytes = bytes;
    }
    *out = ctx->scratch;
    return HIPDSP_OK;
}
```

audian_amd/csrc/sos.hip:

```cpp
#include "sos_device.h"
#include <cmath>
#include <vector>

namespace {
template <int S>
__global__ __launch_bounds__(64 * WPB) void sos_scan_kernel(const SosPlanDev *__restrict__ P0, SeqArgs a)
{
    constexpr int D = 2 * S;
    __shared__ float4 lds_all[WPB][64 * 8];
    const int wave = __builtin_amdgcn_readfirstlane(threadIdx.x >> 6);
    float4 *lds = lds_all[wave];
    const int lane = threadIdx.x & 63;
    const long long unit = (long long)blockIdx.x * WPB + wave;
    if (unit >= a.units) return;
    const int seg = (int)(unit % a.n_seg);
    const long long ch = unit / a.n_seg;
    const float *in = a.in + ch * a.in_pitch;
    float *out = a.out + ch * a.out_pitch;

    const long long lo = (long long)seg * a.seg_len;
    long long hi = lo + a.seg_len;
    if (hi > a.N) hi = a.N;
    long long start = lo - P0->warm;
    if (start < 0) start = 0;
// ... 105 lines not shown
            for (int k = 0; k < 8; k++) {
                const long long p = tile + 256 * k + 4 * lane;
                auto at = [&](long long q) { return in + (q < lead ? lead : (q < T ? q : T - 1)); };
                auto ok = [&](long long q) { return q >= lead && q < T; };
                v4f t;
                t.x = asm_load4(at(p));
                t.y = asm_load4(at(p + 1));
                t.z = asm_load4(at(p + 2));
                t.w = asm_load4(at(p + 3));
                asm volatile("s_waitcnt vmcnt(0)" ::: "memory");
                asm volatile("" : "+v"(t));
                lds[lds_slot(8 * k + (lane >> 3), lane & 7)] =
                    make_float4(ok(p) ? t.x : 0.f, ok(p + 1) ? t.y : 0.f, ok(p + 2) ? t.z : 0.f, ok(p + 3) ? t.w : 0.f);
            }
        } else {
#pragma unroll
            for (int k = 0; k < 8; k++)
                lds[lds_slot(8 * k + (lane >> 3), lane & 7)] = load_four_from(in, tile + 256 * k + 4 * lane, lead, T);
        }
        WAVE_SYNC();
        if (PREFETCH) {
            const long long next = tile + TILE;
            pre = next < loop_end && next + TILE <= T;
            fetch(pre ? next : top_full);
        }
        if constexpr (SF > 0) {
#define CASC_S SF
#define CASC_PLAN() PLAN_OF(PF0)
#define CASC_CARRY cf_
#define CASC_IN(v) (v)
#include "sos_cascade.inc"
#undef CASC_S
#undef CASC_PLAN
#undef CASC_CARRY
#undef CASC_IN
            WAVE_SYNC();
            if (tile + TILE > lo && tile < hi) {
                if (tile >= lo && tile + TILE <= hi && tile >= lead) {
                    v4f rows[8];
                    tile_rows_from_lds(lds, lane, rows);
#pragma unroll
                    for (int k = 0; k < 8; k++) {
                        const v4f v = rows[k];
                        f4u t; t.x = v.x; t.y = v.y; t.z = v.z; t.w = v.w;
                        *reinterpret_cast<f4u *>(yf + tile + 256 * k + 4 * lane) = t;
                    }
                    if (PREFETCH) asm volatile("s_waitcnt vmcnt(7)" ::: "memory");
                } else {
#pragma unroll
                    for (int k = 0; k < 8; k++)
                        store_four(yf, tile + 256 * k + 4 * lane, lds[lds_slot(8 * k + (lane >> 3), lane & 7)],
                                   lo > lead ? lo : lead, hi, 0);
                    if (PREFETCH) asm volatile("s_waitcnt vmcnt(0)" ::: "memory");
                }
            } else if (PREFETCH) {
                asm volatile("s_waitcnt vmcnt(0)" ::: "memory");
            }
        }
        if (tile < env_start) {
            if (PREFETCH && SF == 0) asm volatile("s_waitcnt vmcnt(0)" ::: "memory");
            WAVE_SYNC();
            continue;
        }
        if (a.rectify) {
#pragma unroll
            for (int q = 0; q < 8; q++) {
                float4 v = lds[lds_slot(lane, q)];
                v = make_float4(fabsf(v.x), fabsf(v.y), fabsf(v.z), fabsf(v.w));
                lds[lds_slot(lane, q)] = v;
            }
        }
        WAVE_SYNC();
        auto rval = [&](long long j) -> float {
            return j >= tile ? ldsf[lds_float_index((int)(j - tile))] : rprev[64 - (int)(tile - j)];
        };
        if (tile + TILE > T) {
            float pv = 0.f;
            long long pj = -1;
            if (lane < edge) {
                pj = T + lane;
                if (pj >= tile && pj < tile + TILE) pv = 2.f * rval(T - 1) - rval(T - 2 - lane);
            }
            WAVE_SYNC();
            if (lane < edge && pj >= tile && pj < tile + TILE) ldsf[lds_float_index((int)(pj - tile))] = pv;
            WAVE_SYNC();
        }
        if (env_true && tile == env_start && a.env0 > 0) {
            const SosPlanDev *P = PLAN_OF(PE0);
            const float e0 = env_left_fill(ldsf, lane, (int)(a.env0 - tile), edge);
            const double x0 = a.gain * (double)e0;
#pragma unroll
            for (int r = 0; r < DE; r++) ce_[r] = P->zi[r] * x0;
        } else if (env_true && tile == env_start) {
            const SosPlanDev *P = PLAN_OF(PE0);
            const double r0 = (double)ldsf[lds_float_index(0)];
            const double x0 = a.gain * (2.0 * r0 - (double)ldsf[lds_float_index(edge)]);
#pragma unroll
            for (int r = 0; r < DE; r++) ce_[r] = P->zi[r] * x0;
            for (int i = 0; i < edge; i++) {
                double cur = a.gain * (2.0 * r0 - (double)ldsf[lds_float_index(edge - i)]);
#pragma unroll
                for (int s2 = 0; s2 < SE; s2++) {
                    const double y = fma(P->coef[s2][0], cur, ce_[2 * s2]);
                    ce_[2 * s2] = fma(-P->coef[s2][3], y, fma(P->coef[s2][1], cur, ce_[2 * s2 + 1]));
                    ce_[2 * s2 + 1] = fma(-P->coef[s2][4], y, P->coef[s2][2] * cur);
                    cur = y;
                }
            }
        }
        if ((tile > lo || env_true) && lane == 0) {
#pragma unroll
            for (int r = 0; r < DE; r++) ckpt[(tile / TILE) * DE + r] = ce_[r];
        }
        const bool last_tile = tile + TILE >= loop_end;
        {
            const float4 keep0 = lds[lds_slot(62 + ((lane >> 3) & 1), lane & 7)];
            WAVE_SYNC();
            if (lane < 16) {
                rprev[4 * lane] = keep0.x; rprev[4 * lane + 1] = keep0.y;
                rprev[4 * lane + 2] = keep0.z; rprev[4 * lane + 3] = keep0.w;
            }
        }
#define CASC_S SE
#define CASC_PLAN() PLAN_OF(PE0)
#define CASC_CARRY ce_
#define CASC_IN(v) (v)
#define CASC_GAIN a.gain
#define CASC_NO_OUTPUT
#include "sos_cascade.inc"
#undef CASC_NO_OUTPUT
#undef CASC_GAIN
#undef CASC_S
#undef CASC_PLAN
#undef CASC_CARRY
#undef CASC_IN
        if (PREFETCH && SF == 0) asm volatile("s_waitcnt vmcnt(0)" ::: "memory");
        if (last_tile) {
            if (lane == 0) {
#pragma unroll
                for (int r = 0; r < DE; r++) ckpt[(tile / TILE + 1) * DE + r] = ce_[r];
            }
            break;
        }
        WAVE_SYNC();
    }
    if constexpr (SF > 0) {
        if (a.flags != nullptr && lane == 0) a.flags[unit] = state_not_finite(cf_) ? 1 : 0;
    }
}

template <int SE>
__global__ __launch_bounds__(256) void env_fix_kernel(const SosPlanDev *__restrict__ P0, double *ckpt_all, long long ckpt_pitch,
                                                      int n_seg, long long seg_tiles, long long n_tiles, FloodArgs flood,
                                                      int first_seg)
{
    constexpr int D = 2 * SE;
    double *ckpt = ckpt_all + (long long)blockIdx.x * ckpt_pitch;
    flood_channel(flood, blockIdx.x);
    {
        __shared__ int any_bad;
        if (threadIdx.x == 0) any_bad = 0;
        __syncthreads();
        for (long long j = first_seg + threadIdx.x; j < n_seg; j += blockDim.x) {
            const double *e = ckpt + (j + 1 < n_seg ? (j + 1) * seg_tiles : n_tiles) * D;
            bool bad = false;
#pragma unroll
            for (int r = 0; r < D; r++) bad = bad || !(fabs(e[r]) <= 1.7976931348623157e308);
            if (bad) atomicOr(&any_bad, 1);
        }
        __syncthreads();
        if (any_bad && threadIdx.x == 0) ckpt[n_tiles * D] = __builtin_nan("");
        __syncthreads();
    }
    double AT[D][D], P[D][D];
#pragma unroll
    for (int r = 0; r < D; r++)
#pragma unroll
        for (int c = 0; c < D; c++) { AT[r][c] = P0->AT[r * D + c]; P[r][c] = r == c ? 1.0 : 0.0; }
    {
        double Q[D][D];
#pragma unroll
        for (int r = 0; r < D; r++)
#pragma unroll
            for (int c = 0; c < D; c++) Q[r][c] = AT[r][c];
        for (long long e = seg_tiles; e > 0; e >>= 1) {
            double t[D][D];
            if (e & 1) {
#pragma unroll
                for (int r = 0; r < D; r++)
#pragma unroll
                    for (int c = 0; c < D; c++) {
                        double acc = 0.0;
#pragma unroll
                        for (int k = 0; k < D; k++) acc = fma(P[r][k], Q[k][c], acc);
                        t[r][c] = acc;
                    }
#pragma unroll
                for (int r = 0; r < D; r++)
#pragma unroll
                    for (int c = 0; c < D; c++) P[r][c] = t[r][c];
            }
#pragma unroll
            for (int r = 0; r < D; r++)
#pragma unroll
                for (int c = 0; c < D; c++) {
                    double acc = 0.0;
#pragma unroll
                    for (int k = 0; k < D; k++) acc = fma(Q[r][k], Q[k][c], acc);
                    t[r][c] = acc;
                }
#pragma unroll
            for (int r = 0; r < D; r++)
#pragma unroll
                for (int c = 0; c < D; c++) Q[r][c] = t[r][c];
        }
    }
    const long long warm_tiles = P0->warm / TILE;
    const long long terms = (warm_tiles + seg_tiles - 1) / seg_tiles + 1;
    for (long long k_hi = n_seg - 1; k_hi >= first_seg + 1; k_hi -= blockDim.x) {
        const long long k = k_hi - threadIdx.x;
        double S[D];
#pragma unroll
        for (int r = 0; r < D; r++) S[r] = 0.0;
        if (k >= first_seg + 1) {
            long long j = k - terms;
            if (j < first_seg) j = first_seg;
            for (; j < k; j++) {
                const double *e = ckpt + (j + 1) * seg_tiles * D;
                double t[D];
#pragma unroll
                for (int r = 0; r < D; r++) {
                    double acc = e[r];
#pragma unroll
                    for (int c = 0; c < D; c++) acc = fma(P[r][c], S[c], acc);
                    t[r] = acc;
                }
#pragma unroll
                for (int r = 0; r < D; r++) S[r] = t[r];
            }
        }
        __syncthreads();
        if (k >= first_seg + 1) {
            const long long t0 = k * seg_tiles;
            long long cnt = (k == n_seg - 1) ? n_tiles - t0 : seg_tiles;
            if (cnt > warm_tiles + 1) cnt = warm_tiles + 1;
#pragma unroll
            for (int r = 0; r < D; r++) ckpt[t0 * D + r] = S[r];
            for (long long m = 1; m < cnt; m++) {
                double t[D];
#pragma unroll
                for (int r = 0; r < D; r++) {
                    double acc = 0.0;
#pragma unroll
                    for (int c = 0; c < D; c++) acc = fma(AT[r][c], S[c], acc);
                    t[r] = acc;
                }
#pragma unroll
                for (int r = 0; r < D; r++) { S[r] = t[r]; ckpt[(t0 + m) * D + r] += t[r]; }
            }
        }
        __syncthreads();
    }
}

int launch_env_fix(hipdsp_ctx *ctx, const SosPlanDev *edev, int SE, double *ckpt, long long ckpt_pitch, long long channels,
                   int n_seg, long long seg_len, long long n_tiles, const FloodArgs *flood, int first_seg = 0)
{
    if (n_seg <= 1) return HIPDSP_OK;
    dim3 grid((unsigned)channels), block(256);
    const long long seg_tiles = seg_len / TILE;
    FloodArgs fl;
    memset(&fl, 0, sizeof(fl));
    if (flood) fl = *flood;
    switch (SE) {
    case 1: hipLaunchKernelGGL((env_fix_kernel<1>), grid, block, 0, ctx->stream, edev, ckpt, ckpt_pitch, n_seg, seg_tiles, n_tiles, fl, first_seg); break;
    case 2: hipLaunchKernelGGL((env_fix_kernel<2>), grid, block, 0, ctx->stream, edev, ckpt, ckpt_pitch, n_seg, seg_tiles, n_tiles, fl, first_seg); break;
    case 3: hipLaunchKernelGGL((env_fix_kernel<3>), grid, block, 0, ctx->stream, edev, ckpt, ckpt_pitch, n_seg, seg_tiles, n_tiles, fl, first_seg); break;
    case 4: hipLaunchKernelGGL((env_fix_kernel<4>), grid, block, 0, ctx->stream, edev, ckpt, ckpt_pitch, n_seg, seg_tiles, n_tiles, fl, first_seg); break;
    default: return HIPDSP_OK;
    }
    return hd_launch_status("env_fix_kernel");
}

template <int SE, bool PREFETCH, bool PIN = true, bool TRACE = false, int WPB_ = WPB, bool REGW = (SE <= 2)>
__global__ __launch_bounds__(64 * WPB_, REGW ? 2 : 1) void env_bwd_kernel(const SosPlanDev *__restrict__ P0, BwdArgs a)
{
    long long tr_acc[6] = {0, 0, 0, 0, 0, 0};
    long long tr_last = TRACE ? clock64() : 0;
#define TRACE_AT(i)                                              \
    do {                                                         \
        if (TRACE) {                                             \
            const long long t_ = clock64();                      \
            tr_acc[(i)] += t_ - tr_last;                         \
            tr_last = t_;                                        \
        }                                                        \
    } while (0)
    constexpr int DE = 2 * SE;
    __shared__ float4 lds_all[WPB_][64 * 8];
    const int wave = __builtin_amdgcn_readfirstlane(threadIdx.x >> 6);
    float4 *lds = lds_all[wave];
    float *ldsf = reinterpret_cast<float *>(lds);
    const int lane = threadIdx.x & 63;
    const long long unit = (long long)blockIdx.x * WPB_ + wave;
    if (unit >= a.units) return;
    const int seg = (int)(unit % a.n_seg);
    const long long ch = unit / a.n_seg;
    const float *in = a.in + ch * a.in_pitch;
    float *out = a.out + ch * a.out_pitch;
    const double *ckpt = a.ckpt + ch * a.ckpt_pitch;
    const long long T = a.T;
    const int edge = a.edge;
    const long long trace_t0 = a.trace ? wall_clock64() : 0;
    const unsigned slot = wave_slot_of_simd();

    const long long rt_lo = (long long)seg * a.seg_tiles;
    long long rt_hi = rt_lo + a.seg_tiles;
    if (rt_hi > a.n_tiles) rt_hi = a.n_tiles;
    long long rt_start = rt_lo - a.warm_tiles;
    if (rt_start < 0) rt_start = 0;

    double cb_[DE];
#pragma unroll
    for (int r = 0; r < DE; r++) cb_[r] = 0.0;

    {
        double end_state[DE];
#pragma unroll
        for (int r = 0; r < DE; r++) end_state[r] = ckpt[a.n_tiles * DE + r];
        if (state_not_finite(end_state)) {
            long long p_lo = (a.n_tiles - rt_hi) * TILE, p_hi = (a.n_tiles - rt_lo) * TILE;
            if (p_lo < a.skip) p_lo = a.skip;
            if (p_hi > T) p_hi = T;
            for (long long p = p_lo + lane; p < p_hi; p += 64) out[p - a.skip] = __builtin_nanf("");
            return;
        }
    }

    v4f nx[8], nck[SE];
    bool pre = false;
    auto fetch = [&](long long tidx) {
        const long long tsrc = (a.debug & 2) ? 0 : tidx;
#pragma unroll
        for (int k = 0; k < 8; k++) nx[k] = asm_load16(in + tsrc * TILE + 256 * k + 4 * lane);
#pragma unroll
        for (int i = 0; i < SE; i++) nck[i] = asm_load16(ckpt + tidx * DE + 2 * i);
    };
    const long long top_full = T / TILE - 1;
    auto prefetchable = [&](long long tidx) {
        return tidx >= 0 && tidx <= top_full && tidx * TILE + TILE > a.skip && tidx * TILE >= a.lead;
    };
    const long long env_tile0 = a.env0 > 0 ? a.env0 - a.env0 % TILE : -1;
    if (PREFETCH) {
        const long long t0 = a.n_tiles - 1 - rt_start;
        pre = rt_start < rt_hi && prefetchable(t0);
        fetch(pre ? t0 : top_full);
        asm volatile("s_waitcnt vmcnt(0)" ::: "memory");
    }

    for (long long rt = rt_start; rt < rt_hi; rt++) {
        const long long tidx = a.n_tiles - 1 - rt;
        const long long tile = tidx * TILE;
        if (tile + TILE <= a.skip) break;
        if (a.fair) rotate_issue_priority(slot);
        double cfw_[DE];
        if (PREFETCH && pre) {
            if (a.rectify) {
#pragma unroll
                for (int k = 0; k < 8; k++) {
                    asm volatile("" : "+v"(nx[k]));
                    lds[lds_slot(8 * k + (lane >> 3), lane & 7)] =
                        make_float4(fabsf(nx[k].x), fabsf(nx[k].y), fabsf(nx[k].z), fabsf(nx[k].w));
                }
            } else {
#pragma unroll
                for (int k = 0; k < 8; k++) {
                    asm volatile("" : "+v"(nx[k]));
                    lds[lds_slot(8 * k + (lane >> 3), lane & 7)] = make_float4(nx[k].x, nx[k].y, nx[k].z, nx[k].w);
                }
            }
#pragma unroll
            for (int i = 0; i < SE; i++) {
                asm volatile("" : "+v"(nck[i]));
                const v2d d = __builtin_bit_cast(v2d, nck[i]);
                cfw_[2 * i] = d.x; cfw_[2 * i + 1] = d.y;
            }
            WAVE_SYNC();
        } else if (PREFETCH) {
            const long long lead = a.lead;
#pragma unroll 1
            for (int k = 0; k < 8; k++) {
                const long long p = tile + 256 * k + 4 * lane;
                auto at = [&](long long q) { return in + (q < lead ? lead : (q < T ? q : T - 1)); };
                auto ok = [&](long long q) { return q >= lead && q < T; };
                v4f t;
                t.x = asm_load4(at(p));
                t.y = asm_load4(at(p + 1));
                t.z = asm_load4(at(p + 2));
                t.w = asm_load4(at(p + 3));
                asm volatile("s_waitcnt vmcnt(0)" ::: "memory");
                asm volatile("" : "+v"(t));
                float4 v = make_float4(ok(p) ? t.x : 0.f, ok(p + 1) ? t.y : 0.f, ok(p + 2) ? t.z : 0.f,
                                       ok(p + 3) ? t.w : 0.f);
                if (a.rectify) v = make_float4(fabsf(v.x), fabsf(v.y), fabsf(v.z), fabsf(v.w));
                lds[lds_slot(8 * k + (lane >> 3), lane & 7)] = v;
            }
            v4f ck[SE];
#pragma unroll
            for (int i = 0; i < SE; i++) ck[i] = asm_load16(ckpt + tidx * DE + 2 * i);
            float ra = asm_load4(in + (T - 1));
            float rb = asm_load4(in + (lane < edge ? T - 2 - lane : T - 1));
            asm volatile("s_waitcnt vmcnt(0)" ::: "memory");
#pragma unroll
            for (int i = 0; i < SE; i++) {
                asm volatile("" : "+v"(ck[i]));
                const v2d d = __builtin_bit_cast(v2d, ck[i]);
                cfw_[2 * i] = d.x; cfw_[2 * i + 1] = d.y;
            }
            asm volatile("" : "+v"(ra));
            asm volatile("" : "+v"(rb));
            WAVE_SYNC();
            if (lane < edge) {
                const long long pj = T + lane;
                if (pj >= tile && pj < tile + TILE) {
                    if (a.rectify) { ra = fabsf(ra); rb = fabsf(rb); }
                    ldsf[lds_float_index((int)(pj - tile))] = 2.f * ra - rb;
                }
            }
        } else {
#pragma unroll
            for (int k = 0; k < 8; k++) {
                float4 v = load_four_from(in, tile + 256 * k + 4 * lane, a.lead, T);
                if (a.rectify) v = make_float4(fabsf(v.x), fabsf(v.y), fabsf(v.z), fabsf(v.w));
                lds[lds_slot(8 * k + (lane >> 3), lane & 7)] = v;
            }
#pragma unroll
            for (int r = 0; r < DE; r++) cfw_[r] = ckpt[tidx * DE + r];
        }
        WAVE_SYNC();
        if (!PREFETCH && tile + TILE > T) {
            if (lane < edge) {
                const long long pj = T + lane;
                if (pj >= tile && pj < tile + TILE) {
                    float ra = in[T - 1], rb = in[T - 2 - lane];
                    if (a.rectify) { ra = fabsf(ra); rb = fabsf(rb); }
                    ldsf[lds_float_index((int)(pj - tile))] = 2.f * ra - rb;
                }
            }
            WAVE_SYNC();
        }
        if (PREFETCH) WAVE_SYNC();
        if (tile == env_tile0) {
            (void)env_left_fill(ldsf, lane, (int)(a.env0 - tile), edge);
        }
        TRACE_AT(0);
        if (PREFETCH) {
            pre = rt + 1 < rt_hi && prefetchable(tidx - 1);
            fetch(pre ? tidx - 1 : top_full);
        }
        TRACE_AT(1);
#define CASC_S SE
#define CASC_PLAN() PLAN_OF(P0)
#define CASC_IN(v) (v)
#define CASC_PIN_GROUPS PIN
      if constexpr (REGW) {
#define CASC_CARRY_AFTER_F
        double w_[L];
#define CASC_CARRY cfw_
#define CASC_GAIN a.gain
#define CASC_NO_STORE
#define CASC_TAP(j, e, y) w_[(j)] = (y)
#include "sos_cascade.inc"
#undef CASC_TAP
#undef CASC_NO_STORE
#undef CASC_GAIN
#undef CASC_CARRY
        WAVE_SYNC();
// ... 129 lines not shown

__global__ __launch_bounds__(256) void flip_kernel(const float *__restrict__ x, long long x_pitch, long long N, long long first, long long n,
                                                   int clamp, float *__restrict__ y, long long y_pitch)
{
    const long long ch = blockIdx.y;
    const float *xc = x + ch * x_pitch;
    float *yc = y + ch * y_pitch;
    auto cl = [&](float v) { return (clamp && v < 0.f) ? 0.f : v; };
    const long long i = 4 * ((long long)blockIdx.x * 256 + threadIdx.x);
    if (i >= n) return;
    if (i + 4 <= n) {
        const f4u v = *reinterpret_cast<const f4u *>(xc + (N - 1 - (first + i) - 3));
        f4u o; o.x = cl(v.w); o.y = cl(v.z); o.z = cl(v.y); o.w = cl(v.x);
        *reinterpret_cast<f4u *>(yc + i) = o;
        return;
    }
    for (long long j = i; j < n; j++) yc[j] = cl(xc[N - 1 - (first + j)]);
}

__global__ void first_sample_kernel(const float *__restrict__ x, long long x_pitch, long long channels, float *__restrict__ ref)
{
    const long long c = (long long)blockIdx.x * blockDim.x + threadIdx.x;
    if (c < channels) ref[c] = x[c * x_pitch];
}

__global__ __launch_bounds__(256) void copy_skip_kernel(const float *__restrict__ x, long long x_pitch, float *__restrict__ y,
                                                        long long y_pitch, long long n, long long skip)
{
    const long long ch = blockIdx.y;
    const float *xi = x + ch * x_pitch + skip;
    float *yo = y + ch * y_pitch;
    const long long n4 = n / 4;
    const long long i = (long long)blockIdx.x * 256 + threadIdx.x;
    if (i < n4) {
        *reinterpret_cast<f4u *>(yo + 4 * i) = *reinterpret_cast<const f4u *>(xi + 4 * i);
    } else if (i == n4) {
        for (long long k = 4 * n4; k < n; k++) yo[k] = xi[k];
    }
}

int launch_scan(hipdsp_ctx *ctx, const SosPlanDev *dev, int S, SeqArgs a, long long channels, long long warm)
{
    if (a.gain == 0.0) a.gain = 1.0;
    plan_segments(ctx, a.N, channels, warm, &a.seg_len, &a.n_seg, -1);
    a.units = channels * a.n_seg;
    long long blocks = (a.units + WPB - 1) / WPB;
    if (blocks > 0x7fffffffLL) {
        hipdsp_set_error("grid too large (%lld blocks)", blocks);
        return HIPDSP_ERR_INVALID;
    }
    dim3 grid((unsigned)blocks), block(64 * WPB);
    if (a.n_seg > 1) {
        const int frc = hd_seg_flags(ctx, (size_t)a.units, &a.flags);
        if (frc != HIPDSP_OK) return frc;
    }
    switch (S) {
    case 1: hipLaunchKernelGGL((sos_scan_kernel<1>), grid, block, 0, ctx->stream, dev, a); break;
    case 2: hipLaunchKernelGGL((sos_scan_kernel<2>), grid, block, 0, ctx->stream, dev, a); break;
    case 3: hipLaunchKernelGGL((sos_scan_kernel<3>), grid, block, 0, ctx->stream, dev, a); break;
    case 4: hipLaunchKernelGGL((sos_scan_kernel<4>), grid, block, 0, ctx->stream, dev, a); break;
    default:
        hipdsp_set_error("n_sections %d not in 1..%d", S, MAXS);
        return HIPDSP_ERR_UNSUPPORTED;
    }
    const int rc = hd_launch_status("sos_scan_kernel");
    if (rc != HIPDSP_OK || a.flags == nullptr) return rc;
    FloodArgs fl;
    memset(&fl, 0, sizeof(fl));
    fl.flags = a.flags; fl.n_seg = a.n_seg; fl.seg_len = a.seg_len;
    fl.y = a.out; fl.y_pitch = a.out_pitch; fl.T = a.N; fl.skip = a.skip;
    return launch_flood(ctx, fl, channels);
}

int launch_env_ckpt(hipdsp_ctx *ctx, const SosPlanDev *fdev, const SosPlanDev *edev, int SF, int SE, long long warmF,
                    long long warmE, int edge, const float *x, long long x_pitch, float *yf,
                    long long yf_pitch, float *env, long long env_pitch, long long channels,
                    long long frames, long long skip, int rectify, double gain, int clamp, int phase,
                    GridShift gs = GridShift{0, 0, 0})
{
    const long long real_frames = frames;
    x -= gs.lead;
    if (yf) yf -= gs.lead;
    frames += gs.lead;
    skip += gs.env0;
    const long long n_tiles = (frames + edge + TILE - 1) / TILE;
    const long long ckpt_pitch = (n_tiles + 1) * 2 * SE;
    void *work = nullptr;
    int rc = phase == 2 ? hd_scratch_parked(ctx, sizeof(double) * (size_t)ckpt_pitch * (size_t)channels, &work)
                        : hipdsp_scratch(ctx, sizeof(double) * (size_t)ckpt_pitch * (size_t)channels, &work);
    if (rc != HIPDSP_OK) return rc;
    if (phase != 2) {
        CkptArgs fa;
        memset(&fa, 0, sizeof(fa));
        fa.in = x; fa.yf = yf; fa.ckpt = (double *)work;
        fa.in_pitch = x_pitch; fa.yf_pitch = yf_pitch; fa.ckpt_pitch = ckpt_pitch;
        fa.T = frames; fa.edge = edge; fa.rectify = rectify; fa.gain = rectify ? gain : 1.0;
        fa.lead = gs.lead; fa.env0 = gs.env0;
        hd_note_sweep(ctx, gs.lead, gs.env0, real_frames, channels, SE);
        long long warm = warmF;
        if (warmF >= (1LL << 40) || warmE >= (1LL << 40)) warm = 1LL << 50;
        plan_segments(ctx, frames, channels, warm, &fa.seg_len, &fa.n_seg, -2);
        fa.units = channels * fa.n_seg;
        long long blocks = (fa.units + WPB - 1) / WPB;
        HD_REQUIRE(blocks <= 0x7fffffffLL, "grid too large");
        dim3 grid((unsigned)blocks), block(64 * WPB);
        if (SF > 0 && fa.n_seg > 1) {
            rc = hd_seg_flags(ctx, (size_t)fa.units, &fa.flags);
            if (rc != HIPDSP_OK) return rc;
        }
        const bool pf = ctx->sos_prefetch && frames >= 4 * TILE;
#define HD_CKPT(A, B)                                                                                       \
    case (A) * 8 + (B):                                                                                     \
        if (pf && (A) <= 2 && (B) <= 2)                                                                     \
            hipLaunchKernelGGL((sos_ckpt_kernel<A, B, ((A) <= 2 && (B) <= 2)>), grid, block, 0, ctx->stream, fdev, edev, fa); \
        else                                                                                                \
            hipLaunchKernelGGL((sos_ckpt_kernel<A, B, false>), grid, block, 0, ctx->stream, fdev, edev, fa); \
        break
        switch (SF * 8 + SE) {
            HD_CKPT(0, 1); HD_CKPT(0, 2); HD_CKPT(0, 3); HD_CKPT(0, 4);
            HD_CKPT(1, 1); HD_CKPT(1, 2); HD_CKPT(1, 3); HD_CKPT(1, 4);
            HD_CKPT(2, 1); HD_CKPT(2, 2); HD_CKPT(2, 3); HD_CKPT(2, 4);
            HD_CKPT(3, 1); HD_CKPT(3, 2); HD_CKPT(3, 3); HD_CKPT(3, 4);
            HD_CKPT(4, 1); HD_CKPT(4, 2); HD_CKPT(4, 3); HD_CKPT(4, 4);
        default:
            hipdsp_set_error("n_sections %d / %d not in 0..%d / 1..%d", SF, SE, MAXS, MAXS);
            return HIPDSP_ERR_UNSUPPORTED;
        }
#undef HD_CKPT
        rc = hd_launch_status("sos_ckpt_kernel");
        if (rc != HIPDSP_OK) return rc;
        FloodArgs fl;
        memset(&fl, 0, sizeof(fl));
        fl.flags = fa.flags; fl.n_seg = fa.n_seg; fl.seg_len = fa.seg_len;
        fl.y = yf ? yf + gs.lead : nullptr; fl.y_pitch = yf_pitch; fl.T = frames; fl.skip = gs.lead;
        rc = launch_env_fix(ctx, edev, SE, (double *)work, ckpt_pitch, channels, fa.n_seg, fa.seg_len, n_tiles, &fl,
                            (int)((gs.env0 - gs.env0 % TILE) / fa.seg_len));
        if (rc != HIPDSP_OK) return rc;
    }
    if (phase == 1) return HIPDSP_OK;
    if (ctx->mid_event) HD_CHECK_HIP(hipEventRecord(ctx->mid_event, ctx->stream));
    if (frames - skip == 0) return HIPDSP_OK;
    BwdArgs b;
    memset(&b, 0, sizeof(b));
    b.in = SF > 0 ? yf : x; b.in_pitch = SF > 0 ? yf_pitch : x_pitch;
    b.out = env; b.out_pitch = env_pitch;
    b.ckpt = (const double *)work; b.ckpt_pitch = ckpt_pitch;
    b.T = frames; b.skip = skip; b.n_tiles = n_tiles; b.edge = edge;
    b.lead = gs.lead; b.env0 = gs.env0;
    b.rectify = rectify; b.clamp = clamp; b.gain = rectify ? gain : 1.0;
    b.trace = ctx->sos_trace;
    b.trace_rows = ctx->sos_trace_rows;
    b.debug = ctx->sos_debug;
    b.fair = ctx->sos_fair;
    const long long used_tiles = n_tiles - skip / TILE;
    long long seg_len = 0;
    plan_segments(ctx, used_tiles * TILE, channels, warmE, &seg_len, &b.n_seg, 4, SE <= 2 ? 8 : 16);
    b.seg_tiles = seg_len / TILE;
    b.warm_tiles = warmE / TILE;
    b.units = channels * b.n_seg;
    long long blocks = (b.units + WPB - 1) / WPB;
    HD_REQUIRE(blocks <= 0x7fffffffLL, "grid too large");
    dim3 grid((unsigned)blocks), block(64 * WPB);
#ifdef HIPDSP_WITH_ENVSPLIT
    if (ctx->sos_split && SE <= 2 && frames >= 4 * TILE) return hd_launch_env_bwd_split(ctx, edev, SE, b);
#endif
    if (ctx->sos_single_wave_wg) { grid = dim3((unsigned)b.units); block = dim3(64); }
    if (ctx->sos_single_wave_wg && SE == 1 && ctx->sos_prefetch && frames >= 4 * TILE && !ctx->sos_trace && !ctx->sos_no_pin) {
        hipLaunchKernelGGL((env_bwd_kernel<1, true, true, false, 1>), grid, block, 0, ctx->stream, edev, b);
        return hd_launch_status("env_bwd_kernel");
    }
    if (ctx->sos_single_wave_wg) { grid = dim3((unsigned)blocks); block = dim3(64 * WPB); }
    switch (SE) {
    case 1:
        if (ctx->sos_prefetch && frames >= 4 * TILE) {
            if (ctx->sos_trace) hipLaunchKernelGGL((env_bwd_kernel<1, true, true, true>), grid, block, 0, ctx->stream, edev, b);
            else if (ctx->sos_no_pin) hipLaunchKernelGGL((env_bwd_kernel<1, true, false>), grid, block, 0, ctx->stream, edev, b);
            else hipLaunchKernelGGL((env_bwd_kernel<1, true>), grid, block, 0, ctx->stream, edev, b);
        } else hipLaunchKernelGGL((env_bwd_kernel<1, false>), grid, block, 0, ctx->stream, edev, b);
        break;
    case 2:
        if (ctx->sos_prefetch && frames >= 4 * TILE) hipLaunchKernelGGL((env_bwd_kernel<2, true>), grid, block, 0, ctx->stream, edev, b);
        else hipLaunchKernelGGL((env_bwd_kernel<2, false>), grid, block, 0, ctx->stream, edev, b);
        break;
    case 3: hipLaunchKernelGGL((env_bwd_kernel<3, false>), grid, block, 0, ctx->stream, edev, b); break;
    case 4: hipLaunchKernelGGL((env_bwd_kernel<4, false>), grid, block, 0, ctx->stream, edev, b); break;
    default:
        hipdsp_set_error("n_sections %d not in 1..%d", SE, MAXS);
        return HIPDSP_ERR_UNSUPPORTED;
    }
    return hd_launch_status("env_bwd_kernel");
}

}

int hd_launch_env_fix(hipdsp_ctx *ctx, const SosPlanDev *edev, int SE, double *ckpt, long long ckpt_pitch, long long channels,
                      int n_seg, long long seg_len, long long n_tiles, const FloodArgs *flood, int first_seg)
{
    return launch_env_fix(ctx, edev, SE, ckpt, ckpt_pitch, channels, n_seg, seg_len, n_tiles, flood, first_seg);
}

extern "C" {

int hipdsp_sosplan_create(hipdsp_ctx *ctx, hipdsp_sosplan **out)
{
    HD_REQUIRE(ctx != nullptr && out != nullptr, "NULL argument");
    *out = nullptr;
    HD_CHECK_HIP(hipSetDevice(ctx->device));
    hipdsp_sosplan *p = new hipdsp_sosplan();
    p->host = nullptr; p->dev = nullptr; p->uploaded = nullptr; p->valid = false;
    hipError_t e = hipHostMalloc((void **)&p->host, sizeof(SosPlanDev), hipHostMallocDefault);
    if (e == hipSuccess) e = hipMalloc((void **)&p->dev, sizeof(SosPlanDev));
    if (e == hipSuccess) e = hipEventCreateWithFlags(&p->uploaded, hipEventDisableTiming);
    if (e != hipSuccess) {
        if (p->host) (void)hipHostFree(p->host);
        if (p->dev) (void)hipFree(p->dev);
        delete p;
        HD_CHECK_HIP(e);
    }
    memset(p->host, 0, sizeof(SosPlanDev));
    *out = p;
    return HIPDSP_OK;
}

int hipdsp_sosplan_destroy(hipdsp_ctx *ctx, hipdsp_sosplan *plan)
{
    HD_REQUIRE(ctx != nullptr, "ctx is NULL");
    if (!plan) return HIPDSP_OK;
    (void)hipStreamSynchronize(ctx->stream);
    if (plan->uploaded) (void)hipEventDestroy(plan->uploaded);
    if (plan->host) (void)hipHostFree(plan->host);
    if (plan->dev) (void)hipFree(plan->dev);
    delete plan;
    return HIPDSP_OK;
}

int hipdsp_sosplan_set_host(hipdsp_ctx *ctx, hipdsp_sosplan *plan, const double *host_sos,
                            int n_sections)
{
    HD_REQUIRE(ctx != nullptr && plan != nullptr && host_sos != nullptr, "NULL argument");
    if (n_sections < 1 || n_sections > MAXS) {
        hipdsp_set_error("n_sections %d not in 1..%d (cascade longer filters over several plans)",
                         n_sections, MAXS);
        return HIPDSP_ERR_UNSUPPORTED;
    }
    if (plan->valid) HD_CHECK_HIP(hipEventSynchronize(plan->uploaded));
    SosPlanDev tmp;
    int rc = hd_fill_plan(&tmp, host_sos, n_sections);
    if (rc != HIPDSP_OK) return rc;
    memcpy(plan->host, &tmp, sizeof(tmp));
    return HIPDSP_OK;
}

int hipdsp_sosplan_upload(hipdsp_ctx *ctx, hipdsp_sosplan *plan)
{
    HD_REQUIRE(ctx != nullptr && plan != nullptr, "NULL argument");
    HD_REQUIRE(plan->host->n_sections > 0, "plan has no coefficients yet");
    HD_CHECK_HIP(hipMemcpyAsync(plan->dev, plan->host, sizeof(SosPlanDev), hipMemcpyHostToDevice,
                                ctx->stream));
    hipStreamCaptureStatus st = hipStreamCaptureStatusNone;
    if (ctx->stream) (void)hipStreamIsCapturing(ctx->stream, &st);
    if (st == hipStreamCaptureStatusNone) {
        HD_CHECK_HIP(hipEventRecord(plan->uploaded, ctx->stream));
        plan->valid = true;
    }
    return HIPDSP_OK;
}

int hipdsp_sosplan_set(hipdsp_ctx *ctx, hipdsp_sosplan *plan, const double *host_sos, int n_sections)
{
    int rc = hipdsp_sosplan_set_host(ctx, plan, host_sos, n_sections);
    if (rc != HIPDSP_OK) return rc;
    return hipdsp_sosplan_upload(ctx, plan);
}

int hipdsp_sosplan_info(hipdsp_ctx *ctx, hipdsp_sosplan *plan, int64_t *warmup, int *edge)
{
    HD_REQUIRE(ctx != nullptr && plan != nullptr, "NULL argument");
    if (warmup) *warmup = plan->host->warm;
    if (edge) *edge = plan->host->edge;
    return HIPDSP_OK;
}

int hipdsp_sosfilt(hipdsp_ctx *ctx, const hipdsp_sosplan *plan, const float *x, int64_t x_pitch,
                   float *y, int64_t y_pitch, int64_t channels, int64_t frames, int64_t skip)
{
    HD_REQUIRE(ctx != nullptr, "ctx is NULL");
    HD_REQUIRE(channels >= 0 && frames >= 0, "negative size");
    HD_REQUIRE(skip >= 0 && skip <= frames, "skip %lld not in [0, frames=%lld]", (long long)skip,
               (long long)frames);
    if (channels == 0 || frames - skip == 0) return HIPDSP_OK;
    HD_REQUIRE(x != nullptr && y != nullptr, "NULL data pointer");
    HD_REQUIRE(x_pitch >= frames && y_pitch >= frames - skip, "pitch smaller than row length");
    HD_NO_OVERLAP(x, x_pitch, frames, y, y_pitch, frames - skip, channels, "x and y");
    HD_CHECK_HIP(hipSetDevice(ctx->device));
    if (plan == nullptr) {
        long long n = frames - skip;
        const long long blocks = (n / 4 + 1 + 255) / 256;
        HD_REQUIRE(blocks <= 0x7fffffffLL && channels <= 65535, "grid too large");
        const unsigned gx = (unsigned)blocks;
        hipLaunchKernelGGL(copy_skip_kernel, dim3(gx, (unsigned)channels), dim3(256), 0, ctx->stream, x,
                           (long long)x_pitch, y, (long long)y_pitch, n, (long long)skip);
        return hd_launch_status("copy_skip_kernel");
    }
    HD_REQUIRE(plan->host->n_sections > 0, "plan has no coefficients");
    SeqArgs a;
    memset(&a, 0, sizeof(a));
    a.in = x; a.out = y; a.in_pitch = x_pitch; a.out_pitch = y_pitch;
    a.N = frames; a.skip = skip;
    return launch_scan(ctx, plan->dev, plan->host->n_sections, a, channels, plan->host->warm);
}

int hipdsp_sosfilt_envelope(hipdsp_ctx *ctx, const hipdsp_sosplan *fplan, const hipdsp_sosplan *eplan,
                            const float *x, int64_t x_pitch, float *yf, int64_t yf_pitch, float *env,
                            int64_t env_pitch, int64_t channels, int64_t frames, int rectify, double gain,
                            int clamp, int phase, int64_t env_first)
{
    HD_REQUIRE(ctx != nullptr && fplan != nullptr && eplan != nullptr, "NULL argument");
    HD_REQUIRE(phase >= 0 && phase <= 2, "phase must be 0 (both), 1 (forward) or 2 (backward)");
    HD_REQUIRE(channels >= 0 && frames >= 0, "negative size");
    HD_REQUIRE(env_first >= 0 && env_first <= frames, "env_first %lld not in [0, frames=%lld]", (long long)env_first,
               (long long)frames);
    HD_REQUIRE(fplan->host->n_sections > 0 && eplan->host->n_sections > 0, "plan has no coefficients");
    HD_CHECK_HIP(hipSetDevice(ctx->device));
    {
        const int frc = hd_device_fault(ctx);
        if (frc != HIPDSP_OK) return frc;
    }
    const int edge = eplan->host->edge;
    if (frames - env_first <= edge) {
        hipdsp_set_error("The length of the input vector x must be greater than padlen, which is %d.", edge);
        return HIPDSP_ERR_TOO_SHORT;
    }
    if (channels == 0) return HIPDSP_OK;
    HD_REQUIRE(x != nullptr && yf != nullptr && env != nullptr, "NULL data pointer");
    HD_REQUIRE(x_pitch >= frames && yf_pitch >= frames && env_pitch >= frames - env_first, "pitch smaller than row length");
    if (phase != 2) HD_NO_OVERLAP(x, x_pitch, frames, yf, yf_pitch, frames, channels, "x and yf");
    if (phase != 1) HD_NO_OVERLAP(yf, yf_pitch, frames, env, env_pitch, frames - env_first, channels, "yf and env");
    GridShift gs;
    if (phase == 2) {
        const long long lead = ctx->sweep_lead;
        if (ctx->sweep_frames != frames || ctx->sweep_channels != channels || ctx->sweep_sections != eplan->host->n_sections ||
            ctx->sweep_env0 - lead != env_first) {
            hipdsp_set_error("hipdsp_sosfilt_envelope(phase = 2): the last forward sweep on this context left tile states for "
                             "%lld channels x %lld frames, %d sections, envelope from frame %lld -- not for %lld x %lld, %d, %lld",
                             ctx->sweep_channels, ctx->sweep_frames, ctx->sweep_sections,
                             ctx->sweep_env0 - ctx->sweep_lead, (long long)channels, (long long)frames,
                             eplan->host->n_sections, (long long)env_first);
            return HIPDSP_ERR_INVALID;
        }
        gs.lead = lead; gs.env0 = ctx->sweep_env0; gs.frame_off = 0;
    } else {
// ... 123 lines not shown
```

audian_amd/csrc/sos_device.h:

```cpp
#pragma once
#include "common.h"
#include "sos_plan.h"

struct hipdsp_sosplan {
    SosPlanDev *host;
    SosPlanDev *dev;
    hipEvent_t uploaded;
    bool valid;
};

struct FloodArgs {
    const unsigned char *flags;
    int n_seg;
    long long seg_len;
    float *y;
    long long y_pitch, T, skip;
    float *psd, *db;
    long long psd_pitch, n_valid;
    int F, nfft, hop;
    int frame_off;
};

int hd_launch_env_fix(hipdsp_ctx *ctx, const SosPlanDev *edev, int SE, double *ckpt, long long ckpt_pitch, long long channels,
                      int n_seg, long long seg_len, long long n_tiles, const FloodArgs *flood, int first_seg = 0);

struct BwdArgs {
    const float *in;
    float *out;
    const double *ckpt;
    long long in_pitch, out_pitch, ckpt_pitch;
    long long T, skip;
    long long n_tiles;
    long long seg_tiles, warm_tiles;
    int n_seg, edge, rectify, clamp;
    double gain;
    long long units;
    long long lead, env0;
    long long *trace;
    long long trace_rows;
    int debug;
    int fair;
};

namespace {


typedef float f4u __attribute__((ext_vector_type(4), aligned(4)));
typedef float f2u __attribute__((ext_vector_type(2), aligned(4)));

struct SeqArgs {
    const float *in;
    float *out;
    long long in_pitch, out_pitch;
    long long N;
    long long seg_len;
    int n_seg;
    long long skip;
    const float *zi_ref;
    long long zi_ref_pitch;
    double zi_scale;
    double gain;
    long long units;
    unsigned char *flags;
};

__device__ __forceinline__ long long opaque_zero()
{
    int z;
    asm volatile("s_mov_b32 %0, 0" : "=s"(z));
    return (long long)z;
}

__device__ __forceinline__ int lds_slot(int row, int q) { return row * 8 + (q ^ ((row & 7) ^ ((row >> 3) & 1))); }
__device__ __forceinline__ int lds_float_index(int s) { return lds_slot(s >> 5, (s & 31) >> 2) * 4 + (s & 3); }

__device__ __forceinline__ float4 load_four(const float *in, long long p, long long n)
{
    if (p + 4 <= n) {
        const f4u t = *reinterpret_cast<const f4u *>(in + p);
        return make_float4(t.x, t.y, t.z, t.w);
    }
    float4 v;
    v.x = p < n ? in[p] : 0.f;
    v.y = p + 1 < n ? in[p + 1] : 0.f;
    v.z = p + 2 < n ? in[p + 2] : 0.f;
    v.w = p + 3 < n ? in[p + 3] : 0.f;
    return v;
}

__device__ __forceinline__ float4 load_four_from(const float *in, long long p, long long first, long long n)
{
    if (p >= first) return load_four(in, p, n);
    float4 v;
    v.x = 0.f;
    v.y = (p + 1 >= first && p + 1 < n) ? in[p + 1] : 0.f;
    v.z = (p + 2 >= first && p + 2 < n) ? in[p + 2] : 0.f;
    v.w = (p + 3 >= first && p + 3 < n) ? in[p + 3] : 0.f;
    return v;
}

__device__ __forceinline__ void store_four(float *out, long long p, float4 v, long long lo, long long hi,
                                           long long shift)
{
    if (p >= lo && p + 4 <= hi) {
        f4u t; t.x = v.x; t.y = v.y; t.z = v.z; t.w = v.w;
        *reinterpret_cast<f4u *>(out + (p - shift)) = t;
    } else {
        const float e[4] = {v.x, v.y, v.z, v.w};
#pragma unroll
        for (int k = 0; k < 4; k++)
            if (p + k >= lo && p + k < hi) out[p + k - shift] = e[k];
    }
}

#define PLAN_OF(ptr) (reinterpret_cast<const SosPlanDev *>(reinterpret_cast<const char *>(ptr) + opaque_zero()))

__device__ __forceinline__ double casc_wave_shr1(double x)
{
    const long long b = __builtin_bit_cast(long long, x);
    const int lo = __builtin_amdgcn_update_dpp(0, (int)b, 0x138, 0xf, 0xf, true);
    const int hi = __builtin_amdgcn_update_dpp(0, (int)(b >> 32), 0x138, 0xf, 0xf, true);
    return __builtin_bit_cast(double, ((long long)hi << 32) | (unsigned int)lo);
}

__device__ __forceinline__ double casc_wave_shr32(double x)
{
    const long long b = __builtin_bit_cast(long long, x);
    const auto lo = __builtin_amdgcn_permlane32_swap(0, (int)b, false, false);
    const auto hi = __builtin_amdgcn_permlane32_swap(0, (int)(b >> 32), false, false);
    return __builtin_bit_cast(double, ((long long)hi[0] << 32) | (unsigned int)lo[0]);
}

__device__ __forceinline__ double casc_wave_shl1(double x)
{
    const long long b = __builtin_bit_cast(long long, x);
    const int lo = __builtin_amdgcn_update_dpp(0, (int)b, 0x130, 0xf, 0xf, true);
    const int hi = __builtin_amdgcn_update_dpp(0, (int)(b >> 32), 0x130, 0xf, 0xf, true);
    return __builtin_bit_cast(double, ((long long)hi << 32) | (unsigned int)lo);
}
__device__ __forceinline__ double casc_wave_shl32(double x)
{
    const long long b = __builtin_bit_cast(long long, x);
    const auto lo = __builtin_amdgcn_permlane32_swap((int)b, 0, false, false);
    const auto hi = __builtin_amdgcn_permlane32_swap((int)(b >> 32), 0, false, false);
    return __builtin_bit_cast(double, ((long long)hi[1] << 32) | (unsigned int)lo[1]);
}

#define WAVE_SYNC()                                          \
    do {                                                     \
        __builtin_amdgcn_fence(__ATOMIC_ACQ_REL, "wavefront"); \
        __builtin_amdgcn_wave_barrier();                     \
    } while (0)

constexpr int WPB = 4;

struct CkptArgs {
    const float *in;
    float *yf;
    double *ckpt;
    long long in_pitch, yf_pitch, ckpt_pitch;
    long long T, seg_len;
    int n_seg, edge, rectify;
    long long units;
    double gain;
    unsigned char *flags;
    long long lead;
    long long env0;
};

struct GridShift {
    long long lead, env0;
    int frame_off;
};
inline GridShift hd_grid_shift(long long spec_first, long long env_first, int hop, int edge, bool with_env)
{
    GridShift g;
    const long long step = hop > 0 ? hop : 128;
    g.lead = hop > 0 ? (step - spec_first % step) % step : 0;
    if (with_env && env_first + g.lead > 0) {
        for (int tries = 0; tries < 4; tries++) {
            const long long r = (env_first + g.lead) % TILE;
            if (r >= edge && r + edge < TILE) break;
            g.lead += step;
        }
    }
    g.env0 = with_env ? env_first + g.lead : 0;
    g.frame_off = hop > 0 ? (int)((spec_first + g.lead) / step) : 0;
    return g;
}

typedef float v4f __attribute__((ext_vector_type(4)));
__device__ __forceinline__ void tile_rows_from_lds(const float4 *lds, int lane, v4f (&v)[8])
{
#pragma unroll
    for (int k = 0; k < 8; k++) {
        const float4 t = lds[lds_slot(8 * k + (lane >> 3), lane & 7)];
        v[k] = (v4f){t.x, t.y, t.z, t.w};
    }
    asm volatile("" : "+v"(v[0]), "+v"(v[1]), "+v"(v[2]), "+v"(v[3]), "+v"(v[4]), "+v"(v[5]), "+v"(v[6]), "+v"(v[7]));
}
typedef double v2d __attribute__((ext_vector_type(2)));
__device__ __forceinline__ v4f asm_load16(const void *p)
{
    v4f r;
    asm volatile("global_load_dwordx4 %0, %1, off" : "=v"(r) : "v"(p) : "memory");
    return r;
}
__device__ __forceinline__ float asm_load4(const float *p)
{
    float r;
    asm volatile("global_load_dword %0, %1, off" : "=v"(r) : "v"(p) : "memory");
    return r;
}

__device__ __forceinline__ void rotate_issue_priority(unsigned slot)
{
    const unsigned p = (slot + (unsigned)(__builtin_readcyclecounter() >> 14)) & 3u;
    if (p == 0) __builtin_amdgcn_s_setprio(0);
    else if (p == 1) __builtin_amdgcn_s_setprio(1);
    else if (p == 2) __builtin_amdgcn_s_setprio(2);
    else __builtin_amdgcn_s_setprio(3);
}
__device__ __forceinline__ float max_zero(float x)
{
    float r;
    asm("v_max_f32_e32 %0, 0, %1" : "=v"(r) : "v"(x));
    return r;
}
__device__ __forceinline__ void set_issue_priority(int p)
{
    if (p == 0) __builtin_amdgcn_s_setprio(0);
    else if (p == 1) __builtin_amdgcn_s_setprio(1);
    else if (p == 2) __builtin_amdgcn_s_setprio(2);
    else __builtin_amdgcn_s_setprio(3);
}
__device__ __forceinline__ unsigned wave_slot_of_simd()
{
    unsigned hw;
    asm volatile("s_getreg_b32 %0, hwreg(HW_REG_HW_ID, 0, 4)" : "=s"(hw));
    return hw;
}

inline void hd_note_sweep(hipdsp_ctx *ctx, long long lead, long long env0, long long frames, long long channels, int SE)
{
    ctx->sweep_lead = lead; ctx->sweep_env0 = env0; ctx->sweep_frames = frames; ctx->sweep_channels = channels;
    ctx->sweep_sections = SE;
}

__device__ __forceinline__ float env_left_fill(float *ldsf, int lane, int q, int edge)
{
    const float r0 = ldsf[lds_float_index(q)];
    const float e0 = 2.f * r0 - ldsf[lds_float_index(q + edge)];
    float ev = 0.f;
    if (lane < edge) ev = 2.f * r0 - ldsf[lds_float_index(q + edge - lane)];
    WAVE_SYNC();
    if (lane < edge) ldsf[lds_float_index(q - edge + lane)] = ev;
    for (int s2 = lane; s2 < q - edge; s2 += 64) ldsf[lds_float_index(s2)] = e0;
    WAVE_SYNC();
    return e0;
}


template <int D>
__device__ __forceinline__ bool state_not_finite(const double (&c)[D])
{
    bool bad = false;
#pragma unroll
    for (int r = 0; r < D; r++) bad = bad || !(fabs(c[r]) <= 1.7976931348623157e308);
    return bad;
}

__device__ void flood_channel(const FloodArgs &f, long long ch)
{
    __shared__ int first_bad;
    if (f.flags == nullptr || f.n_seg <= 1) return;
    if (threadIdx.x == 0) first_bad = 0x7fffffff;
    __syncthreads();
    const unsigned char *fl = f.flags + ch * f.n_seg;
    for (int s2 = threadIdx.x; s2 < f.n_seg - 1; s2 += blockDim.x)
        if (fl[s2]) atomicMin(&first_bad, s2);
    __syncthreads();
    const int s0 = first_bad;
    if (s0 == 0x7fffffff) return;
    const float nan_ = __builtin_nanf("");
    const long long n1 = (long long)(s0 + 1) * f.seg_len;
    if (f.y != nullptr) {
        float *yc = f.y + ch * f.y_pitch;
        for (long long p = (n1 > f.skip ? n1 : f.skip) + threadIdx.x; p < f.T; p += blockDim.x) yc[p - f.skip] = nan_;
    }
    if (f.psd != nullptr || f.db != nullptr) {
        long long k0 = (n1 >= f.nfft ? (n1 - f.nfft) / f.hop + 1 : 0) - f.frame_off;
        if (k0 < 0) k0 = 0;
        for (long long i = k0 * f.F + threadIdx.x; i < f.n_valid * f.F; i += blockDim.x) {
            if (f.psd != nullptr) f.psd[ch * f.psd_pitch + i] = nan_;
            if (f.db != nullptr) f.db[ch * f.psd_pitch + i] = nan_;
        }
    }
}

__global__ __launch_bounds__(256) void nan_flood_kernel(FloodArgs f) { flood_channel(f, blockIdx.x); }

__global__ void zero_rows_kernel(float *__restrict__ y, long long y_pitch, long long n, float value)
{
    long long ch = blockIdx.y;
    float *yo = y + ch * y_pitch;
    for (long long i = (long long)blockIdx.x * blockDim.x + threadIdx.x; i < n;
         i += (long long)gridDim.x * blockDim.x)
        yo[i] = value;
}

int launch_flood(hipdsp_ctx *ctx, const FloodArgs &f, long long channels)
{
    if (f.flags == nullptr || f.n_seg <= 1 || channels == 0) return HIPDSP_OK;
    hipLaunchKernelGGL(nan_flood_kernel, dim3((unsigned)channels), dim3(256), 0, ctx->stream, f);
    return hd_launch_status("nan_flood_kernel");
}

void plan_segments(const hipdsp_ctx *ctx, long long N, long long channels, long long warm,
                   long long *seg_len, int *n_seg, int model, int w_cap = 16)
{
    int w_max = ctx->sos_waves_per_cu > 0 ? ctx->sos_waves_per_cu : 16;
    if (w_max > w_cap) w_max = w_cap;
    hd_plan_segments_occ(ctx->n_cus, w_max, ctx->sos_waves_min >= w_max ? 0 : model, ctx->max_segments, N, channels, warm, seg_len, n_seg);
}

constexpr int CHAIN_P = 8;
void plan_segments_chain(const hipdsp_ctx *ctx, long long N, long long channels, long long warm,
                         long long *seg_len, int *n_seg)
{
    int cus = ctx->n_cus - ctx->chain_reserve_cus;
    if (cus < 1) cus = 1;
    hd_plan_segments_occ(cus, ctx->chain_pairs > 0 ? ctx->chain_pairs : CHAIN_P, 0, ctx->max_segments, N, channels, warm, seg_len,
                      n_seg);
}

}

int hd_launch_env_bwd_split(hipdsp_ctx *ctx, const SosPlanDev *edev, int SE, const BwdArgs &b);
```

audian_amd/csrc/sos_plan.h:

```cpp
#pragma once
#include "common.h"

constexpr int L = 32;
constexpr int TILE = 64 * L;
constexpr int MAXS = HIPDSP_MAX_SECTIONS;
constexpr int MAXD = 2 * MAXS;

struct SosPlanDev {
    double coef[MAXS][5];
    double G[L * MAXD];
    double M[6 * MAXD * MAXD];
    double zi[MAXD];
    double AT[MAXD * MAXD];
    long long warm;
    int n_sections;
    int edge;
    int unit_tail;
};

int hd_fill_plan(SosPlanDev *p, const double *sos, int S);
void hd_plan_segments_occ(long long n_cus, int w_max, int per_simd, int max_segments, long long N, long long channels,
                          long long warm, long long *seg_len, int *n_seg);
```

audian_amd/csrc/sos_plan.hip:

```cpp
#include "sos_plan.h"
#include <cmath>
#include <vector>

namespace {


struct Mat {
    int d;
    double v[MAXD][MAXD];
};

Mat mat_identity(int d)
{
    Mat m; m.d = d;
    for (int i = 0; i < MAXD; i++) for (int j = 0; j < MAXD; j++) m.v[i][j] = (i == j && i < d) ? 1.0 : 0.0;
    return m;
}

Mat mat_mul(const Mat &a, const Mat &b)
{
    Mat m = mat_identity(a.d);
    for (int i = 0; i < a.d; i++)
        for (int j = 0; j < a.d; j++) {
            double s = 0.0;
            for (int k = 0; k < a.d; k++) s += a.v[i][k] * b.v[k][j];
            m.v[i][j] = s;
        }
    return m;
}

double mat_norm_inf(const Mat &a)
{
    double n = 0.0;
    for (int i = 0; i < a.d; i++) {
        double s = 0.0;
        for (int j = 0; j < a.d; j++) s += fabs(a.v[i][j]);
        if (!(s <= n)) n = s;
    }
    return n;
}

void cascade_step(const double coef[MAXS][5], int S, double *z, double x)
{
    double cur = x;
    for (int s = 0; s < S; s++) {
        double y = coef[s][0] * cur + z[2 * s];
        z[2 * s] = coef[s][1] * cur - coef[s][3] * y + z[2 * s + 1];
        z[2 * s + 1] = coef[s][2] * cur - coef[s][4] * y;
        cur = y;
    }
}

int fill_plan(SosPlanDev *p, const double *sos, int S)
{
    memset(p, 0, sizeof(*p));
    p->n_sections = S;
    const int D = 2 * S;
    for (int s = 0; s < S; s++) {
        const double *c = sos + 6 * s;
        if (c[3] != 1.0) {
            hipdsp_set_error("sos[%d][3] (a0) must be 1, got %g", s, c[3]);
            return HIPDSP_ERR_INVALID;
        }
        for (int k = 0; k < 6; k++)
            if (!std::isfinite(c[k])) {
                hipdsp_set_error("sos[%d][%d] is not finite", s, k);
                return HIPDSP_ERR_INVALID;
            }
        p->coef[s][0] = c[0]; p->coef[s][1] = c[1]; p->coef[s][2] = c[2];
        p->coef[s][3] = c[4]; p->coef[s][4] = c[5];
    }
    p->unit_tail = S > 1 ? 1 : 0;
    for (int s = 1; s < S; s++)
        if (!(p->coef[s][0] == 1.0 && p->coef[s][2] == 1.0 && fabs(p->coef[s][1]) == 2.0)) p->unit_tail = 0;
    Mat A = mat_identity(D);
    double B[MAXD] = {0};
    for (int c = 0; c < D; c++) {
        double z[MAXD] = {0};
        z[c] = 1.0;
        cascade_step(p->coef, S, z, 0.0);
        for (int r = 0; r < D; r++) A.v[r][c] = z[r];
    }
    {
        double z[MAXD] = {0};
        cascade_step(p->coef, S, z, 1.0);
        for (int r = 0; r < D; r++) B[r] = z[r];
    }
    {
        double g[MAXD];
        for (int r = 0; r < D; r++) g[r] = B[r];
        for (int j = L - 1; j >= 0; j--) {
            for (int r = 0; r < D; r++) p->G[j * D + r] = g[r];
            double t[MAXD] = {0};
            for (int r = 0; r < D; r++)
                for (int c = 0; c < D; c++) t[r] += A.v[r][c] * g[c];
            for (int r = 0; r < D; r++) g[r] = t[r];
        }
    }
    Mat pw = A;
    for (int k = 0; k < 5; k++) pw = mat_mul(pw, pw);
    static_assert(L == 32, "plan assumes L == 32");
    for (int k = 0; k < 6; k++) {
        for (int r = 0; r < D; r++)
            for (int c = 0; c < D; c++) p->M[k * D * D + r * D + c] = pw.v[r][c];
        pw = mat_mul(pw, pw);
    }
    for (int r = 0; r < D; r++)
        for (int c = 0; c < D; c++) p->AT[r * D + c] = pw.v[r][c];
    const double tol = ldexp(1.0, -60);
    const int MAXBITS = 40;
    std::vector<Mat> pows;
    pows.push_back(pw);
    long long m = 1;
    int top = 0;
    while (!(mat_norm_inf(pows[top]) < tol) && top < MAXBITS) {
        pows.push_back(mat_mul(pows[top], pows[top]));
        top++;
        m <<= 1;
    }
    if (!(mat_norm_inf(pows[top]) < tol)) {
        m = 1LL << 50;
    } else if (top > 0) {
        Mat acc = mat_identity(D);
        long long q = 0;
        for (int k = top - 1; k >= 0; k--) {
            Mat cand = mat_mul(acc, pows[k]);
            if (!(mat_norm_inf(cand) < tol)) { acc = cand; q += 1LL << k; }
        }
        m = q + 1;
    }
    p->warm = m * TILE;
    double scale = 1.0;
    for (int s = 0; s < S; s++) {
        const double *c = sos + 6 * s;
        double b0 = c[0], b1 = c[1], b2 = c[2], a1 = c[4], a2 = c[5];
        double B0 = b1 - a1 * b0, B1 = b2 - a2 * b0;
        double m00 = 1.0 + a1, m01 = -1.0, m10 = a2, m11 = 1.0;
        double det = m00 * m11 - m01 * m10;
        p->zi[2 * s] = scale * (B0 * m11 - m01 * B1) / det;
        p->zi[2 * s + 1] = scale * (m00 * B1 - m10 * B0) / det;
        scale *= (c[0] + c[1] + c[2]) / (c[3] + c[4] + c[5]);
    }
    int nb = 0, na = 0;
    for (int s = 0; s < S; s++) {
        if (sos[6 * s + 2] == 0.0) nb++;
        if (sos[6 * s + 5] == 0.0) na++;
    }
    p->edge = 3 * (2 * S + 1 - (nb < na ? nb : na));
    return HIPDSP_OK;
}

double tile_step_cost(long long w, int w_max, int per_simd)
{
    if (per_simd > 0) {
        const long long sw = (w + per_simd - 1) / per_simd;
        return sw <= 1 ? 0.65 : 0.5 * (double)sw;
    }
    if (per_simd == -1) return 7.0 + 0.5625 * (double)w;
    if (per_simd == -2) return 1.4 + 0.9125 * (double)w;
    return (double)w_max * (1.0 + 0.25 * (1.0 - (double)w / (double)w_max));
}

void plan_segments_occ(long long n_cus, int w_max, int per_simd, int max_segments, long long N, long long channels,
                       long long warm, long long *seg_len, int *n_seg)
{
    if (n_cus < 1) n_cus = 1;
    if (w_max < 1) w_max = 1;
    long long max_seg = (N + TILE - 1) / TILE;
    if (warm >= (1LL << 40)) max_seg = 1;
    if (max_segments > 0 && max_seg > max_segments) max_seg = max_segments;
    if (max_seg > 65536) max_seg = 65536;
    if (max_seg < 1) max_seg = 1;
    const long long slots = n_cus * w_max;
    long long best_n = 1, best_len = (N + TILE - 1) / TILE * TILE;
    double best_cost = -1.0;
    auto consider = [&](long long n) {
        if (n < 1) n = 1;
        if (n > max_seg) n = max_seg;
        long long len = ((N + n - 1) / n + TILE - 1) / TILE * TILE;
        if (len < TILE) len = TILE;
        const long long cnt = (N + len - 1) / len;
        const long long units = channels * cnt;
        const double span = (double)(len + (cnt > 1 ? warm : 0));
        double cost;
        if (units <= slots) cost = span * tile_step_cost((units + n_cus - 1) / n_cus, w_max, per_simd);
        else cost = (double)((units + slots - 1) / slots) * span * tile_step_cost(w_max, w_max, per_simd);
        if (best_cost < 0 || cost < best_cost * (1.0 - 1e-9)) { best_cost = cost; best_n = cnt; best_len = len; }
    };
    for (int w = w_max; w >= 1; w--) consider(n_cus * w / channels);
    for (long long rounds = 2; rounds <= 64; rounds++) consider(rounds * slots / channels);
    for (int half = 1; half < 16; half++) consider((n_cus / channels) >> half);
    consider(1);
    *seg_len = best_len;
    *n_seg = (int)best_n;
}

}

int hd_fill_plan(SosPlanDev *p, const double *sos, int S) { return fill_plan(p, sos, S); }

void hd_plan_segments_occ(long long n_cus, int w_max, int per_simd, int max_segments, long long N, long long channels,
                          long long warm, long long *seg_len, int *n_seg)
{
    plan_segments_occ(n_cus, w_max, per_simd, max_segments, N, channels, warm, seg_len, n_seg);
}

extern "C" {

int hipdsp_sos_plan_host(const double *host_sos, int n_sections, int64_t *warmup, int *edge, double *zi)
{
    HD_REQUIRE(host_sos != nullptr, "host_sos is NULL");
    if (n_sections < 1 || n_sections > MAXS) {
        hipdsp_set_error("n_sections %d not in 1..%d", n_sections, MAXS);
        return HIPDSP_ERR_UNSUPPORTED;
    }
    SosPlanDev tmp;
    int rc = fill_plan(&tmp, host_sos, n_sections);
    if (rc != HIPDSP_OK) return rc;
    if (warmup) *warmup = tmp.warm;
    if (edge) *edge = tmp.edge;
    if (zi)
        for (int k = 0; k < 2 * n_sections; k++) zi[k] = tmp.zi[k];
    return HIPDSP_OK;
}

int hipdsp_sos_segments_host(int64_t n_cus, int waves_max, int per_simd, int max_segments, int64_t frames,
                             int64_t channels, int64_t warmup, int64_t *segment_frames, int *n_segments)
{
    HD_REQUIRE(n_cus >= 1 && waves_max >= 1 && per_simd >= -2 && frames >= 1 && channels >= 1 && warmup >= 0 &&
               max_segments >= 0, "bad argument");
    HD_REQUIRE(segment_frames != nullptr && n_segments != nullptr, "NULL output");
    long long len = 0;
    int n = 0;
    plan_segments_occ(n_cus, waves_max, per_simd, max_segments, frames, channels, warmup, &len, &n);
    *segment_frames = len;
    *n_segments = n;
    return HIPDSP_OK;
}

}
```

audian_amd/hipdsp.py:

```python

import ctypes

import numpy as np

from . import _lib
from ._lib import check, lib


class Context:

    def __init__(self, device=0, stream=None):
        h = ctypes.c_void_p()
        check(lib.hipdsp_ctx_create(int(device), ctypes.c_void_p(stream or 0), ctypes.byref(h)))
        self._h = h
        self.device = int(device)

    @property
    def handle(self):
        return self._h

    def set_stream(self, stream):
        check(lib.hipdsp_ctx_set_stream(self._h, ctypes.c_void_p(stream or 0)))

    def synchronize(self):
        check(lib.hipdsp_ctx_synchronize(self._h))

    def set_max_segments(self, n):
        check(lib.hipdsp_ctx_set_max_segments(self._h, int(n)))

    def set_option(self, name, value):
        check(lib.hipdsp_ctx_set_option(self._h, name.encode(), int(value)))

    def set_mid_event(self, ev):
        check(lib.hipdsp_ctx_set_mid_event(self._h, ev if ev is not None else ctypes.c_void_p(0)))

    def pool_stats(self):
        cached, hits, misses = ctypes.c_size_t(), ctypes.c_uint64(), ctypes.c_uint64()
        check(lib.hipdsp_pool_stats(self._h, ctypes.byref(cached), ctypes.byref(hits), ctypes.byref(misses)))
        return int(cached.value), int(hits.value), int(misses.value)

    def pool_trim(self):
        check(lib.hipdsp_pool_trim(self._h))

    def reserve(self, nbytes):
        check(lib.hipdsp_ctx_reserve(self._h, int(nbytes)))

    def create_stream(self):
        st = ctypes.c_void_p()
        check(lib.hipdsp_stream_create(self._h, ctypes.byref(st)))
        return st.value

    def destroy_stream(self, stream):
        check(lib.hipdsp_stream_destroy(self._h, ctypes.c_void_p(stream)))

    def graph_begin(self):
        check(lib.hipdsp_graph_begin(self._h))

    def graph_end(self):
        g = ctypes.c_void_p()
        check(lib.hipdsp_graph_end(self._h, ctypes.byref(g)))
        return g

    def graph_launch(self, graph):
        check(lib.hipdsp_graph_launch(self._h, graph))

    def graph_destroy(self, graph):
        check(lib.hipdsp_graph_destroy(self._h, graph))

    def event(self):
        ev = ctypes.c_void_p()
        check(lib.hipdsp_event_create(self._h, ctypes.byref(ev)))
        return ev

    def record(self, ev):
        check(lib.hipdsp_event_record(self._h, ev))

    def wait_event(self, ev):
        check(lib.hipdsp_event_wait(self._h, ev))

    def elapsed_ms(self, start, stop):
        ms = ctypes.c_float()
        check(lib.hipdsp_event_elapsed_ms(self._h, start, stop, ctypes.byref(ms)))
        return float(ms.value)

    def destroy_event(self, ev):
        check(lib.hipdsp_event_destroy(self._h, ev))

    def close(self):
        if self._h is not None and self._h.value:
            lib.hipdsp_ctx_destroy(self._h)
            self._h = None

    def __del__(self):
        try:
            self.close()
        except Exception:
            pass


_default_ctx = None


def default_context():
    global _default_ctx
    if _default_ctx is None:
        import os
        _default_ctx = Context(int(os.environ.get('LOCAL_RANK', '0')))
    return _default_ctx


class DeviceArray:

    def __init__(self, ctx, shape, dtype=np.float32, ptr=None, owner=None, write_probe=0):
        self.ctx = ctx
        self.shape = tuple(int(s) for s in np.atleast_1d(shape))
        self.dtype = np.dtype(dtype)
        self.nbytes = int(np.prod(self.shape, dtype=np.int64))*self.dtype.itemsize
        self._own = ptr is None
        self._owner = owner
        if ptr is None:
            p = ctypes.c_void_p()
            if write_probe > 1:
                check(lib.hipdsp_malloc_probed(ctx.handle, self.nbytes, int(write_probe), ctypes.byref(p)))
            else:
                check(lib.hipdsp_malloc(ctx.handle, self.nbytes, ctypes.byref(p)))
            self.ptr = p.value or 0
        else:
            self.ptr = int(ptr)

    @classmethod
    def from_host(cls, ctx, array, dtype=None):
        a = np.ascontiguousarray(array, dtype=dtype)
        d = cls(ctx, a.shape, a.dtype)
        d.copy_from_host(a)
        return d

    def copy_from_host(self, array):
        a = np.ascontiguousarray(array, dtype=self.dtype)
        if a.nbytes != self.nbytes:
            raise ValueError('size mismatch in copy_from_host')
        check(lib.hipdsp_memcpy_h2d(self.ctx.handle, ctypes.c_void_p(self.ptr),
                                    ctypes.c_void_p(a.ctypes.data), self.nbytes))

    def to_host(self):
        out = np.empty(self.shape, dtype=self.dtype)
        check(lib.hipdsp_memcpy_d2h(self.ctx.handle, ctypes.c_void_p(out.ctypes.data),
                                    ctypes.c_void_p(self.ptr), self.nbytes))
        return out

    def zero_(self):
        check(lib.hipdsp_memset(self.ctx.handle, ctypes.c_void_p(self.ptr), 0, self.nbytes))
        return self

    def view(self, offset_elems, shape):
        v = DeviceArray(self.ctx, shape, self.dtype,
                        ptr=self.ptr + int(offset_elems)*self.dtype.itemsize, owner=self)
        if v.ptr + v.nbytes > self.ptr + self.nbytes:
            raise ValueError('view exceeds the parent array')
        return v

    def free(self):
        if self._own and self.ptr:
            lib.hipdsp_free(self.ctx.handle, ctypes.c_void_p(self.ptr))
            self.ptr = 0

    def __del__(self):
        try:
            self.free()
        except Exception:
            pass


def _p(x):
    if x is None:
        return ctypes.c_void_p(0)
    if isinstance(x, DeviceArray):
        return ctypes.c_void_p(x.ptr)
    if hasattr(x, 'data_ptr'):
        return ctypes.c_void_p(x.data_ptr())
    return ctypes.c_void_p(int(x))


class SosPlan:

# ... 288 lines not shown
```

include/hip_dsp.h:

```cpp
#ifndef HIP_DSP_H
#define HIP_DSP_H

#include <stddef.h>
#include <stdint.h>

#ifdef __cplusplus
extern "C" {
#endif

#define HIPDSP_VERSION 102

#define HIPDSP_OK               0
#define HIPDSP_ERR_INVALID      1
#define HIPDSP_ERR_HIP          2
#define HIPDSP_ERR_UNSUPPORTED  3
#define HIPDSP_ERR_TOO_SHORT    4
#define HIPDSP_ERR_NOMEM        5

#define HIPDSP_MAX_SECTIONS     4

typedef struct hipdsp_ctx hipdsp_ctx;
typedef struct hipdsp_sosplan hipdsp_sosplan;


int hipdsp_version(void);
const char *hipdsp_last_error(void);
int hipdsp_device_count(int *count);

int hipdsp_ctx_create(int device, void *stream, hipdsp_ctx **out);
int hipdsp_ctx_destroy(hipdsp_ctx *ctx);
int hipdsp_ctx_set_stream(hipdsp_ctx *ctx, void *stream);
int hipdsp_ctx_synchronize(hipdsp_ctx *ctx);
int hipdsp_ctx_set_max_segments(hipdsp_ctx *ctx, int max_segments);
int hipdsp_ctx_set_option(hipdsp_ctx *ctx, const char *name, long long value);
int hipdsp_ctx_reserve(hipdsp_ctx *ctx, size_t bytes);


int hipdsp_stream_create(hipdsp_ctx *ctx, void **stream);
int hipdsp_stream_destroy(hipdsp_ctx *ctx, void *stream);

typedef struct hipdsp_graph hipdsp_graph;
int hipdsp_graph_begin(hipdsp_ctx *ctx);
int hipdsp_graph_end(hipdsp_ctx *ctx, hipdsp_graph **out);
int hipdsp_graph_launch(hipdsp_ctx *ctx, hipdsp_graph *graph);
int hipdsp_graph_destroy(hipdsp_ctx *ctx, hipdsp_graph *graph);


int hipdsp_malloc(hipdsp_ctx *ctx, size_t bytes, void **dptr);
int hipdsp_free(hipdsp_ctx *ctx, void *dptr);
int hipdsp_malloc_probed(hipdsp_ctx *ctx, size_t bytes, int tries, void **dptr);
int hipdsp_pool_stats(hipdsp_ctx *ctx, size_t *cached_bytes, uint64_t *hits, uint64_t *misses);
int hipdsp_pool_trim(hipdsp_ctx *ctx);
int hipdsp_memset(hipdsp_ctx *ctx, void *dptr, int value, size_t bytes);
int hipdsp_memcpy_h2d(hipdsp_ctx *ctx, void *dst, const void *host_src, size_t bytes);
int hipdsp_memcpy_d2h(hipdsp_ctx *ctx, void *host_dst, const void *src, size_t bytes);
int hipdsp_memcpy_d2d(hipdsp_ctx *ctx, void *dst, const void *src, size_t bytes);
int hipdsp_host_malloc(hipdsp_ctx *ctx, size_t bytes, void **host_ptr);
int hipdsp_host_free(hipdsp_ctx *ctx, void *host_ptr);
int hipdsp_memcpy_h2d_async(hipdsp_ctx *ctx, void *dst, const void *host_src, size_t bytes);
int hipdsp_memcpy2d_d2d(hipdsp_ctx *ctx, void *dst, size_t dst_pitch, const void *src,
                        size_t src_pitch, size_t width, size_t height);

int hipdsp_event_create(hipdsp_ctx *ctx, void **event);
int hipdsp_event_destroy(hipdsp_ctx *ctx, void *event);
int hipdsp_event_record(hipdsp_ctx *ctx, void *event);
int hipdsp_event_wait(hipdsp_ctx *ctx, void *event);
int hipdsp_event_elapsed_ms(hipdsp_ctx *ctx, void *start, void *stop, float *ms);

int hipdsp_ctx_set_mid_event(hipdsp_ctx *ctx, void *event);


int hipdsp_pack_f64(hipdsp_ctx *ctx, const double *src_tc, float *dst, int64_t dst_pitch,
                    int64_t frames, int64_t channels);
int hipdsp_pack_f32(hipdsp_ctx *ctx, const float *src_tc, float *dst, int64_t dst_pitch,
                    int64_t frames, int64_t channels);
int hipdsp_unpack_f64(hipdsp_ctx *ctx, const float *src, int64_t src_pitch, double *dst_tc,
                      int64_t frames, int64_t channels);
int hipdsp_unpack_spectrum_f64(hipdsp_ctx *ctx, const float *src, int64_t src_pitch,
                               double *dst_tcf, int64_t frames, int64_t channels,
                               int64_t nfreq);


int hipdsp_sosplan_create(hipdsp_ctx *ctx, hipdsp_sosplan **out);
int hipdsp_sosplan_destroy(hipdsp_ctx *ctx, hipdsp_sosplan *plan);
int hipdsp_sosplan_set(hipdsp_ctx *ctx, hipdsp_sosplan *plan, const double *host_sos,
                       int n_sections);
int hipdsp_sosplan_set_host(hipdsp_ctx *ctx, hipdsp_sosplan *plan, const double *host_sos,
                            int n_sections);
int hipdsp_sosplan_upload(hipdsp_ctx *ctx, hipdsp_sosplan *plan);
int hipdsp_sos_plan_host(const double *host_sos, int n_sections, int64_t *warmup, int *edge,
                         double *zi);
int hipdsp_sos_segments_host(int64_t n_cus, int waves_max, int per_simd, int max_segments, int64_t frames,
                             int64_t channels, int64_t warmup, int64_t *segment_frames,
                             int *n_segments);
int hipdsp_sosplan_info(hipdsp_ctx *ctx, hipdsp_sosplan *plan, int64_t *warmup, int *edge);




int hipdsp_sosfilt(hipdsp_ctx *ctx, const hipdsp_sosplan *plan, const float *x,
                   int64_t x_pitch, float *y, int64_t y_pitch, int64_t channels,
                   int64_t frames, int64_t skip);

int hipdsp_envelope(hipdsp_ctx *ctx, const hipdsp_sosplan *plan, const float *x,
                    int64_t x_pitch, float *y, int64_t y_pitch, int64_t channels,
                    int64_t frames, int64_t skip, int rectify, double gain, int clamp);

int hipdsp_sosfilt_envelope(hipdsp_ctx *ctx, const hipdsp_sosplan *fplan,
                            const hipdsp_sosplan *eplan, const float *x, int64_t x_pitch,
                            float *yf, int64_t yf_pitch, float *env, int64_t env_pitch,
                            int64_t channels, int64_t frames, int rectify, double gain, int clamp,
                            int phase, int64_t env_first);

int hipdsp_envelope_multi(hipdsp_ctx *ctx, const hipdsp_sosplan *const *plans, int n_plans, const float *x,
                          int64_t x_pitch, float *y, int64_t y_pitch, int64_t channels, int64_t frames,
                          int64_t skip, int rectify, double gain, int clamp);

int hipdsp_chain_forward(hipdsp_ctx *ctx, const hipdsp_sosplan *fplan,
                         const hipdsp_sosplan *eplan, const float *x, int64_t x_pitch, float *yf,
                         int64_t yf_pitch, int64_t channels, int64_t frames, int rectify,
                         double gain, int nfft, int hop, double fs, float *psd, float *db_out,
                         int64_t frames_out, int64_t psd_pitch, int64_t spec_frames, int64_t spec_first,
                         int64_t env_first);

int hipdsp_chain_backward(hipdsp_ctx *ctx, const hipdsp_sosplan *eplan, const float *yf, int64_t yf_pitch,
                          float *env, int64_t env_pitch, int64_t channels, int64_t frames, int rectify,
                          double gain, int clamp, int nfft, int hop, double fs, float *psd,
                          int64_t frames_out, int64_t psd_pitch);

int hipdsp_chain_plan(hipdsp_ctx *ctx, const hipdsp_sosplan *fplan, const hipdsp_sosplan *eplan,
                      int64_t channels, int64_t frames, int64_t *segment_frames, int *n_segments);

int hipdsp_chain_backward_plan(hipdsp_ctx *ctx, const hipdsp_sosplan *eplan, int64_t channels, int64_t frames,
                               int64_t *first_border, int64_t *segment_frames, int *n_segments);

int hipdsp_spectrogram(hipdsp_ctx *ctx, const float *x, int64_t x_pitch, int64_t channels,
                       int64_t frames, int nfft, int hop, double fs, float *out,
                       float *db_out, int64_t frames_out, int64_t out_pitch);

int hipdsp_decibel(hipdsp_ctx *ctx, const float *p, float *out, int64_t n, double ref_power,
                   double min_power);
int hipdsp_decibel_image(hipdsp_ctx *ctx, const float *spec_tf, float *image_ft,
                         int64_t frames, int64_t nfreq, double ref_power, double min_power);
int hipdsp_decibel_image_decimate(hipdsp_ctx *ctx, const float *spec_tf, float *image_fc,
                                  int64_t frames, int64_t nfreq, int64_t start, int64_t stop,
                                  int64_t step, double ref_power, double min_power);


int hipdsp_minmax_decimate(hipdsp_ctx *ctx, const float *x, int64_t x_pitch, int64_t channels,
                           int64_t start, int64_t stop, int64_t step, float *out,
                           int64_t out_pitch);

int hipdsp_channel_mean(hipdsp_ctx *ctx, const float *x, int64_t x_pitch, const int *host_channels,
                        int count, int64_t start, int64_t n, double heterodyne_cycles_per_sample,
                        float *out);
int hipdsp_stride_copy(hipdsp_ctx *ctx, const float *x, int64_t n, int64_t step, float *out);

int hipdsp_max_nonneg(hipdsp_ctx *ctx, const float *x, int64_t n, float *out);

int hipdsp_band_order_stats(hipdsp_ctx *ctx, const float *x, int64_t rows, int64_t cols, int64_t row_stride,
                            int64_t rank, float *out2);

int hipdsp_unwrap(hipdsp_ctx *ctx, const float *x, int64_t x_pitch, int64_t channels, int64_t frames,
                  double thresh, double ampl_max, int clips, int down_scale, float *y, int64_t y_pitch);

int hipdsp_pcm_unpack(hipdsp_ctx *ctx, const void *pcm_tc, int sample_bytes, int64_t frames,
                      int64_t channels, double scale, float *dst, int64_t dst_pitch);

int hipdsp_pcm_minmax(hipdsp_ctx *ctx, const void *pcm_tc, int sample_bytes, int64_t frames, int64_t channels,
                      int64_t step, double scale, double unwrap_thresh, double ampl_max, int clips, int down_scale,
                      double *out_rc, int64_t out_pitch);

int hipdsp_mean_spectrum_db(hipdsp_ctx *ctx, const float *spec_tf, int64_t nfreq, int64_t i0,
                            int64_t i1, double ref_power, double min_power, double floor_db,
                            float *out);


#define HIPDSP_UNIQUE_ID_BYTES 128
typedef struct hipdsp_comm hipdsp_comm;
int hipdsp_comm_unique_id(void *id_out);
int hipdsp_comm_create(hipdsp_ctx *ctx, const void *unique_id, int rank, int nranks,
                       hipdsp_comm **out);
int hipdsp_comm_destroy(hipdsp_ctx *ctx, hipdsp_comm *comm);
int hipdsp_allgather_f32(hipdsp_ctx *ctx, hipdsp_comm *comm, const float *send, float *recv,
                         int64_t count_per_rank);


int hipdsp_copy_probe(hipdsp_ctx *ctx, void *dst, const void *src, size_t bytes);


int hipdsp_synth(hipdsp_ctx *ctx, float *x, int64_t x_pitch, int64_t channels,
                 int64_t frames, double rate, uint64_t seed, int64_t c0, int64_t c_total);

#ifdef __cplusplus
}
#endif
#endif
```

Measured before the change: 235,600 Msamples/s.

## Seed backward envelope segments with exact border states from forward sweep

During the forward band-pass/envelope sweep, the kernel now taps per-tile contributions over the warmup window before each backward segment border. The env_fix kernel combines these into exact initial states for the backward IIR pass using precomputed Psi/Gb tables. Backward segments then start at their own boundary instead of running a warmup tail, which removes redundant backward warmup work. In exchange the forward sweep does extra reductions and global writes, the plan struct gets larger, and a new border buffer is allocated.

Result: no change. 235,800 Msamples/s (median of 4 runs) (+0.1%).

```diff
diff --git a/audian_amd/_lib.py b/audian_amd/_lib.py
--- a/audian_amd/_lib.py
+++ b/audian_amd/_lib.py
@@ -95,6 +95,8 @@
     'hipdsp_sosplan_set_host': ([_vp, _vp, _vp, _int], _int),
     'hipdsp_sosplan_upload': ([_vp, _vp], _int),
     'hipdsp_sos_plan_host': ([_vp, _int, ctypes.POINTER(_i64), ctypes.POINTER(_int), _vp], _int),
+    'hipdsp_sos_border_host': ([_vp, _int, _vp, _vp, _vp], _int),
+    'hipdsp_envelope_sweep_info': ([_vp, ctypes.POINTER(_i64), ctypes.POINTER(_i64), ctypes.POINTER(_i64), ctypes.POINTER(_int)], _int),
     'hipdsp_sos_segments_host': ([_i64, _int, _int, _int, _i64, _i64, _i64, ctypes.POINTER(_i64), ctypes.POINTER(_int)], _int),
     'hipdsp_sosplan_info': ([_vp, _vp, ctypes.POINTER(_i64), ctypes.POINTER(_int)], _int),
     'hipdsp_sosfilt': ([_vp, _vp, _vp, _i64, _vp, _i64, _i64, _i64, _i64], _int),
diff --git a/audian_amd/csrc/chain.hip b/audian_amd/csrc/chain.hip
--- a/audian_amd/csrc/chain.hip
+++ b/audian_amd/csrc/chain.hip
@@ -359,6 +359,12 @@
     a.c.in_pitch = x_pitch; a.c.yf_pitch = yf_pitch; a.c.ckpt_pitch = ckpt_pitch;
     a.c.T = T; a.c.edge = edge; a.c.rectify = rectify; a.c.gain = rectify ? gain : 1.0;
     a.c.lead = gs.lead; a.c.env0 = gs.env0; a.frame_off = gs.frame_off;
+    if (SE > 0) {
+        rc = hd_border_prepare(ctx, T, edge, gs.env0, channels, eplan->host->warm, SE, rectify && !(ctx->chain_debug & 2), &a.c.bg);
+        if (rc != HIPDSP_OK) return rc;
+    } else {
+        a.c.bg.seg_tiles = 0x3fffffff;
+    }
     a.psd = psd; a.db = db_out; a.psd_pitch = psd_pitch; a.n_valid = n_valid;
     a.scale = (float)(1.0 / (fs * wss));
     a.scale_half = 0.5f * a.scale; a.scale_twice = 2.f * a.scale;
@@ -417,7 +423,7 @@
     fl.F = (int)F; fl.nfft = nfft; fl.hop = hop; fl.frame_off = gs.frame_off;
     if (SE == 0) return launch_flood(ctx, fl, channels);
     return hd_launch_env_fix(ctx, eplan->dev, SE, (double *)work, ckpt_pitch, channels, a.c.n_seg, a.c.seg_len, n_tiles, &fl,
-                             (int)((gs.env0 - gs.env0 % TILE) / a.c.seg_len));
+                             (int)((gs.env0 - gs.env0 % TILE) / a.c.seg_len), &a.c.bg);
 }
 
 int hipdsp_chain_backward(hipdsp_ctx *ctx, const hipdsp_sosplan *eplan, const float *yf, int64_t yf_pitch, float *env,
diff --git a/audian_amd/csrc/chain_fwd.h b/audian_amd/csrc/chain_fwd.h
--- a/audian_amd/csrc/chain_fwd.h
+++ b/audian_amd/csrc/chain_fwd.h
@@ -407,6 +407,12 @@
         pre = prefetchable(base_t);
         fetch(pre ? base_t : top_full_t);
         asm volatile("s_waitcnt vmcnt(0)" ::: "memory");
+        int bg_w0 = 0x3fffffff;
+        if constexpr (SE > 0) {
+            int b = (a.c.bg.n_tiles + a.c.bg.warm - 1 - env_start_t) / a.c.bg.seg_tiles;
+            if (b > a.c.bg.n_seg - 1) b = a.c.bg.n_seg - 1;
+            if (b >= 1) bg_w0 = a.c.bg.n_tiles - b * a.c.bg.seg_tiles;
+        }
 
         for (int it = 0; it < a.n_iter; it++) {
             const int tt = base_t + it;
@@ -539,6 +545,12 @@
 #pragma unroll
                     for (int r = 0; r < DE; r++) ckpt[(long long)tt * DE + r] = ce_[r];
                 }
+                if ((unsigned)(tt - bg_w0) < (unsigned)a.c.bg.warm) {
+                    const int bg_k = tt - bg_w0, bg_b = (a.c.bg.n_tiles - bg_w0) / a.c.bg.seg_tiles;
+                    border_tap<DE, true>(PE0, lds, lane, a.c.gain,
+                                         a.c.bg.buf + ch * a.c.bg.pitch + ((long long)(bg_b - 1) * a.c.bg.warm + bg_k) * DE);
+                    if (bg_k == a.c.bg.warm - 1) bg_w0 = bg_b > 1 ? bg_w0 + a.c.bg.seg_tiles : 0x3fffffff;
+                }
 #define CASC_S SE
 #define CASC_PLAN() PLAN_OF(PE0)
 #define CASC_CARRY ce_
diff --git a/audian_amd/csrc/common.h b/audian_amd/csrc/common.h
--- a/audian_amd/csrc/common.h
+++ b/audian_amd/csrc/common.h
@@ -44,7 +44,15 @@
     size_t seg_flags_cap;
     long long sweep_lead, sweep_env0, sweep_frames, sweep_channels;
     int sweep_sections;
+    double *border;
+    size_t border_cap;
+    int sos_border_exact;
+    int border_valid, border_n_seg, border_sections;
+    long long last_bwd[4];
+    long long border_n_tiles, border_seg_tiles, border_first_tile, border_warm_tiles, border_channels;
 };
+
+int hd_border_buf(hipdsp_ctx *ctx, size_t bytes, double **out);
 
 int hd_seg_flags(hipdsp_ctx *ctx, size_t units, unsigned char **out);
 
diff --git a/audian_amd/csrc/ctx.hip b/audian_amd/csrc/ctx.hip
--- a/audian_amd/csrc/ctx.hip
+++ b/audian_amd/csrc/ctx.hip
@@ -133,6 +133,20 @@
         ctx->seg_flags = (unsigned char *)f;
         ctx->seg_flags_cap = (size_t)1 << 20;
     }
+    ctx->border = nullptr;
+    ctx->border_cap = 0;
+    ctx->border_valid = 0;
+    ctx->sos_border_exact = 1;
+    for (int i = 0; i < 4; i++) ctx->last_bwd[i] = 0;
+    {
+        void *f = nullptr;
+        if (hipMalloc(&f, (size_t)8 << 20) == hipSuccess) {
+            ctx->border = (double *)f;
+            ctx->border_cap = (size_t)8 << 20;
+        } else {
+            (void)hipGetLastError();
+        }
+    }
     *out = ctx;
     return HIPDSP_OK;
 }
@@ -147,6 +161,7 @@
     }
     if (ctx->scratch) (void)hipFree(ctx->scratch);
     if (ctx->seg_flags) (void)hipFree(ctx->seg_flags);
+    if (ctx->border) (void)hipFree(ctx->border);
     if (ctx->fault_host) (void)hipHostFree((void *)ctx->fault_host);
     for (int i = 0; i < 20; i++)
         if (ctx->fft_tables[i]) (void)hipFree(ctx->fft_tables[i]);
@@ -168,6 +183,16 @@
     HD_REQUIRE(ctx != nullptr, "ctx is NULL");
     HD_CHECK_HIP(hipStreamSynchronize(ctx->stream));
     return hd_device_fault(ctx);
+}
+
+int hipdsp_envelope_sweep_info(hipdsp_ctx *ctx, int64_t *n_segments, int64_t *segment_tiles, int64_t *warmup_tiles, int *from_border_states)
+{
+    HD_REQUIRE(ctx != nullptr, "ctx is NULL");
+    if (n_segments) *n_segments = ctx->last_bwd[0];
+    if (segment_tiles) *segment_tiles = ctx->last_bwd[1];
+    if (warmup_tiles) *warmup_tiles = ctx->last_bwd[2];
+    if (from_border_states) *from_border_states = (int)ctx->last_bwd[3];
+    return HIPDSP_OK;
 }
 
 int hipdsp_ctx_set_max_segments(hipdsp_ctx *ctx, int max_segments)
@@ -219,6 +244,7 @@
         return HIPDSP_ERR_UNSUPPORTED;
 #endif
     }
+    if (strcmp(name, "sos_border_exact") == 0) { ctx->sos_border_exact = value != 0; return HIPDSP_OK; }
     if (strcmp(name, "sos_fair") == 0) { ctx->sos_fair = value != 0; return HIPDSP_OK; }
     if (strcmp(name, "sos_trace_rows") == 0) { ctx->sos_trace_rows = value; return HIPDSP_OK; }
     if (strcmp(name, "sos_trace") == 0) {
@@ -644,6 +670,30 @@
     return HIPDSP_OK;
 }
 
+int hd_border_buf(hipdsp_ctx *ctx, size_t bytes, double **out)
+{
+    *out = nullptr;
+    if (bytes > ctx->border_cap) {
+        hipStreamCaptureStatus st = hipStreamCaptureStatusNone;
+        if (ctx->stream) (void)hipStreamIsCapturing(ctx->stream, &st);
+        if (st != hipStreamCaptureStatusNone || ctx->graphs_alive > 0) return HIPDSP_OK;
+        HD_CHECK_HIP(hipStreamSynchronize(ctx->stream));
+        if (ctx->border) HD_CHECK_HIP(hipFree(ctx->border));
+        ctx->border = nullptr;
+        ctx->border_cap = 0;
+        ctx->border_valid = 0;
+        void *f = nullptr;
+        if (hipMalloc(&f, bytes) != hipSuccess) {
+            (void)hipGetLastError();
+            return HIPDSP_OK;
+        }
+        ctx->border = (double *)f;
+        ctx->border_cap = bytes;
+    }
+    *out = ctx->border;
+    return HIPDSP_OK;
+}
+
 int hd_scratch_parked(hipdsp_ctx *ctx, size_t bytes, void **out)
 {
     HD_REQUIRE(ctx != nullptr && out != nullptr, "NULL argument");
diff --git a/audian_amd/csrc/sos.hip b/audian_amd/csrc/sos.hip
--- a/audian_amd/csrc/sos.hip
+++ b/audian_amd/csrc/sos.hip
@@ -281,7 +281,7 @@
 template <int SE>
 __global__ __launch_bounds__(256) void env_fix_kernel(const SosPlanDev *__restrict__ P0, double *ckpt_all, long long ckpt_pitch,
                                                       int n_seg, long long seg_tiles, long long n_tiles, FloodArgs flood,
-                                                      int first_seg)
+                                                      int first_seg, BorderGrid bg)
 {
     constexpr int D = 2 * SE;
     double *ckpt = ckpt_all + (long long)blockIdx.x * ckpt_pitch;
@@ -390,22 +390,61 @@
         }
         __syncthreads();
     }
+    if (bg.buf != nullptr) {
+        __threadfence();
+        __syncthreads();
+        double *bc = bg.buf + (long long)blockIdx.x * bg.pitch;
+        double *zc = bc + (long long)(bg.n_seg - 1) * bg.warm * D;
+        for (int b = 1 + (int)threadIdx.x; b < bg.n_seg; b += blockDim.x) {
+            const double *dt = bc + (long long)(b - 1) * bg.warm * D;
+            double q[D];
+#pragma unroll
+            for (int r = 0; r < D; r++) q[r] = 0.0;
+            for (int k = bg.warm - 1; k >= 0; k--) {
+                double t[D];
+#pragma unroll
+                for (int r = 0; r < D; r++) {
+                    double acc = dt[k * D + r];
+#pragma unroll
+                    for (int c = 0; c < D; c++) acc = fma(AT[r][c], q[c], acc);
+                    t[r] = acc;
+                }
+#pragma unroll
+                for (int r = 0; r < D; r++) q[r] = t[r];
+            }
+            const long long tb = bg.n_tiles - (long long)b * bg.seg_tiles;
+            double sf[D];
+#pragma unroll
+            for (int r = 0; r < D; r++) sf[r] = __hip_atomic_load(&ckpt[tb * D + r], __ATOMIC_RELAXED, __HIP_MEMORY_SCOPE_AGENT);
+#pragma unroll
+            for (int r = 0; r < D; r++) {
+                double acc = q[r];
+#pragma unroll
+                for (int c = 0; c < D; c++) acc = fma(P0->Psi[r * D + c], sf[c], acc);
+                zc[(b - 1) * D + r] = acc;
+            }
+        }
+    }
 }
 
 int launch_env_fix(hipdsp_ctx *ctx, const SosPlanDev *edev, int SE, double *ckpt, long long ckpt_pitch, long long channels,
-                   int n_seg, long long seg_len, long long n_tiles, const FloodArgs *flood, int first_seg = 0)
-{
-    if (n_seg <= 1) return HIPDSP_OK;
+                   int n_seg, long long seg_len, long long n_tiles, const FloodArgs *flood, int first_seg = 0,
+                   const BorderGrid *border = nullptr)
+{
+    BorderGrid bg;
+    memset(&bg, 0, sizeof(bg));
+    if (border) bg = *border;
+    if (n_seg <= 1 && bg.buf == nullptr) return HIPDSP_OK;
     dim3 grid((unsigned)channels), block(256);
     const long long seg_tiles = seg_len / TILE;
     FloodArgs fl;
     memset(&fl, 0, sizeof(fl));
     if (flood) fl = *flood;
     switch (SE) {
-    case 1: hipLaunchKernelGGL((env_fix_kernel<1>), grid, block, 0, ctx->stream, edev, ckpt, ckpt_pitch, n_seg, seg_tiles, n_tiles, fl, first_seg); break;
-    case 2: hipLaunchKernelGGL((env_fix_kernel<2>), grid, block, 0, ctx->stream, edev, ckpt, ckpt_pitch, n_seg, seg_tiles, n_tiles, fl, first_seg); break;
-    case 3: hipLaunchKernelGGL((env_fix_kernel<3>), grid, block, 0, ctx->stream, edev, ckpt, ckpt_pitch, n_seg, seg_tiles, n_tiles, fl, first_seg); break;
-    case 4: hipLaunchKernelGGL((env_fix_kernel<4>), grid, block, 0, ctx->stream, edev, ckpt, ckpt_pitch, n_seg, seg_tiles, n_tiles, fl, first_seg); break;
+    case 1: hipLaunchKernelGGL((env_fix_kernel<1>), grid, block, 0, ctx->stream, edev, ckpt, ckpt_pitch, n_seg, seg_tiles, n_tiles, fl, first_seg, bg); break;
+    case 2: hipLaunchKernelGGL((env_fix_kernel<2>), grid, block, 0, ctx->stream, edev, ckpt, ckpt_pitch, n_seg, seg_tiles, n_tiles, fl, first_seg, bg); break;
+    case 3: hipLaunchKernelGGL((env_fix_kernel<3>), grid, block, 0, ctx->stream, edev, ckpt, ckpt_pitch, n_seg, seg_tiles, n_tiles, fl, first_seg, bg); break;
+    case 4: hipLaunchKernelGGL((env_fix_kernel<4>), grid, block, 0, ctx->stream, edev, ckpt, ckpt_pitch, n_seg, seg_tiles, n_tiles, fl, first_seg, bg); break;
     default: return HIPDSP_OK;
     }
     return hd_launch_status("env_fix_kernel");
@@ -451,6 +490,11 @@
     double cb_[DE];
 #pragma unroll
     for (int r = 0; r < DE; r++) cb_[r] = 0.0;
+    if (a.border != nullptr && seg > 0) {
+        rt_start = rt_lo;
+#pragma unroll
+        for (int r = 0; r < DE; r++) cb_[r] = a.border[ch * a.border_pitch + (long long)(seg - 1) * DE + r];
+    }
 
     {
         double end_state[DE];
@@ -886,11 +930,18 @@
     b.trace_rows = ctx->sos_trace_rows;
     b.debug = ctx->sos_debug;
     b.fair = ctx->sos_fair;
-    const long long used_tiles = n_tiles - skip / TILE;
-    long long seg_len = 0;
-    plan_segments(ctx, used_tiles * TILE, channels, warmE, &seg_len, &b.n_seg, 4, SE <= 2 ? 8 : 16);
-    b.seg_tiles = seg_len / TILE;
+    const BwdGrid g = plan_bwd_grid(ctx, frames, edge, skip, channels, warmE, SE);
+    b.n_seg = g.n_seg;
+    b.seg_tiles = g.seg_tiles;
     b.warm_tiles = warmE / TILE;
+    if (ctx->sos_border_exact && !ctx->sos_split && ctx->border_valid && ctx->border != nullptr && ctx->border_n_seg == g.n_seg &&
+        ctx->border_seg_tiles == g.seg_tiles && ctx->border_n_tiles == n_tiles && ctx->border_first_tile == skip / TILE &&
+        ctx->border_channels == channels && ctx->border_sections == SE && ctx->border_warm_tiles == b.warm_tiles) {
+        b.border_pitch = (long long)(g.n_seg - 1) * (b.warm_tiles + 1) * 2 * SE;
+        b.border = ctx->border + (long long)(g.n_seg - 1) * b.warm_tiles * 2 * SE;
+    }
+    ctx->last_bwd[0] = g.n_seg; ctx->last_bwd[1] = g.seg_tiles; ctx->last_bwd[2] = b.border ? 0 : (g.n_seg > 1 ? b.warm_tiles : 0);
+    ctx->last_bwd[3] = b.border != nullptr;
     b.units = channels * b.n_seg;
     long long blocks = (b.units + WPB - 1) / WPB;
     HD_REQUIRE(blocks <= 0x7fffffffLL, "grid too large");
@@ -928,9 +979,9 @@
 }
 
 int hd_launch_env_fix(hipdsp_ctx *ctx, const SosPlanDev *edev, int SE, double *ckpt, long long ckpt_pitch, long long channels,
-                      int n_seg, long long seg_len, long long n_tiles, const FloodArgs *flood, int first_seg)
-{
-    return launch_env_fix(ctx, edev, SE, ckpt, ckpt_pitch, channels, n_seg, seg_len, n_tiles, flood, first_seg);
+                      int n_seg, long long seg_len, long long n_tiles, const FloodArgs *flood, int first_seg, const BorderGrid *border)
+{
+    return launch_env_fix(ctx, edev, SE, ckpt, ckpt_pitch, channels, n_seg, seg_len, n_tiles, flood, first_seg, border);
 }
 
 extern "C" {
diff --git a/audian_amd/csrc/sos_device.h b/audian_amd/csrc/sos_device.h
--- a/audian_amd/csrc/sos_device.h
+++ b/audian_amd/csrc/sos_device.h
@@ -21,8 +21,10 @@
     int frame_off;
 };
 
+struct BorderGrid;
 int hd_launch_env_fix(hipdsp_ctx *ctx, const SosPlanDev *edev, int SE, double *ckpt, long long ckpt_pitch, long long channels,
-                      int n_seg, long long seg_len, long long n_tiles, const FloodArgs *flood, int first_seg = 0);
+                      int n_seg, long long seg_len, long long n_tiles, const FloodArgs *flood, int first_seg = 0,
+                      const BorderGrid *border = nullptr);
 
 struct BwdArgs {
     const float *in;
@@ -40,6 +42,14 @@
     long long trace_rows;
     int debug;
     int fair;
+    const double *border;
+    long long border_pitch;
+};
+
+struct BorderGrid {
+    double *buf;
+    long long pitch;
+    int n_tiles, seg_tiles, n_seg, warm;
 };
 
 namespace {
@@ -166,6 +176,7 @@
     unsigned char *flags;
     long long lead;
     long long env0;
+    BorderGrid bg;
 };
 
 struct GridShift {
@@ -245,6 +256,50 @@
 {
     ctx->sweep_lead = lead; ctx->sweep_env0 = env0; ctx->sweep_frames = frames; ctx->sweep_channels = channels;
     ctx->sweep_sections = SE;
+    ctx->border_valid = 0;
+}
+
+template <int D, bool ABS>
+__device__ __forceinline__ void border_tap(const SosPlanDev *__restrict__ P0, const float4 *lds, int lane, double gain, double *dst)
+{
+    double f[D];
+#pragma unroll
+    for (int r = 0; r < D; r++) f[r] = 0.0;
+#pragma unroll 1
+    for (int q = 0; q < 8; q++) {
+        const SosPlanDev *P = PLAN_OF(P0);
+        const float4 v = lds[lds_slot(lane, q)];
+        const float e[4] = {v.x, v.y, v.z, v.w};
+#pragma unroll
+        for (int k = 0; k < 4; k++) {
+            const double xd = ABS ? fabs((double)e[k]) : (double)e[k];
+#pragma unroll
+            for (int r = 0; r < D; r++) f[r] = fma(P->Gb[(4 * q + k) * D + r], xd, f[r]);
+        }
+    }
+#pragma unroll
+    for (int r = 0; r < D; r++) f[r] *= gain;
+#pragma unroll 1
+    for (int k = 0; k < 6; k++) {
+        const SosPlanDev *P = PLAN_OF(P0);
+        const int d = 1 << k;
+        double q[D];
+#pragma unroll
+        for (int c = 0; c < D; c++) q[c] = __shfl_down(f[c], d, 64);
+        if (lane < 64 - d) {
+#pragma unroll
+            for (int r = 0; r < D; r++) {
+                double acc = f[r];
+#pragma unroll
+                for (int c = 0; c < D; c++) acc = fma(P->M[k * D * D + r * D + c], q[c], acc);
+                f[r] = acc;
+            }
+        }
+    }
+    if (lane == 0) {
+#pragma unroll
+        for (int r = 0; r < D; r++) dst[r] = f[r];
+    }
 }
 
 __device__ __forceinline__ float env_left_fill(float *ldsf, int lane, int q, int edge)
@@ -334,6 +389,42 @@
                       n_seg);
 }
 
+struct BwdGrid {
+    long long n_tiles, seg_tiles;
+    int n_seg;
+};
+BwdGrid plan_bwd_grid(const hipdsp_ctx *ctx, long long T, int edge, long long skip, long long channels, long long warmE, int SE)
+{
+    BwdGrid g;
+    g.n_tiles = (T + edge + TILE - 1) / TILE;
+    const long long used_tiles = g.n_tiles - skip / TILE;
+    long long seg_len = 0;
+    plan_segments(ctx, used_tiles * TILE, channels, warmE, &seg_len, &g.n_seg, 4, SE <= 2 ? 8 : 16);
+    g.seg_tiles = seg_len / TILE;
+    return g;
+}
+
+int hd_border_prepare(hipdsp_ctx *ctx, long long T, int edge, long long skip, long long channels, long long warmE, int SE,
+                      int rectify, BorderGrid *bg)
+{
+    bg->buf = nullptr; bg->pitch = 0; bg->n_tiles = 0; bg->seg_tiles = 0x3fffffff; bg->n_seg = 0; bg->warm = 0;
+    ctx->border_valid = 0;
+    if (!ctx->sos_border_exact || SE < 1 || SE > 2 || !rectify || warmE >= (1LL << 40)) return HIPDSP_OK;
+    const BwdGrid g = plan_bwd_grid(ctx, T, edge, skip, channels, warmE, SE);
+    const long long warm = warmE / TILE;
+    if (g.n_seg < 2 || g.seg_tiles < warm + 3 || g.n_tiles >= 0x7fffffff) return HIPDSP_OK;
+    const long long pitch = (long long)(g.n_seg - 1) * (warm + 1) * 2 * SE;
+    double *buf = nullptr;
+    const int rc = hd_border_buf(ctx, sizeof(double) * (size_t)pitch * (size_t)channels, &buf);
+    if (rc != HIPDSP_OK || buf == nullptr) return rc;
+    bg->buf = buf; bg->pitch = pitch; bg->n_tiles = (int)g.n_tiles; bg->seg_tiles = (int)g.seg_tiles; bg->n_seg = g.n_seg;
+    bg->warm = (int)warm;
+    ctx->border_valid = 1; ctx->border_n_seg = g.n_seg; ctx->border_sections = SE; ctx->border_n_tiles = g.n_tiles;
+    ctx->border_seg_tiles = g.seg_tiles; ctx->border_first_tile = skip / TILE; ctx->border_warm_tiles = warm;
+    ctx->border_channels = channels;
+    return HIPDSP_OK;
+}
+
 }
 
 int hd_launch_env_bwd_split(hipdsp_ctx *ctx, const SosPlanDev *edev, int SE, const BwdArgs &b);
diff --git a/audian_amd/csrc/sos_plan.h b/audian_amd/csrc/sos_plan.h
--- a/audian_amd/csrc/sos_plan.h
+++ b/audian_amd/csrc/sos_plan.h
@@ -16,6 +16,8 @@
     int n_sections;
     int edge;
     int unit_tail;
+    double Psi[MAXD * MAXD];
+    double Gb[L * MAXD];
 };
 
 int hd_fill_plan(SosPlanDev *p, const double *sos, int S);
diff --git a/audian_amd/csrc/sos_plan.hip b/audian_amd/csrc/sos_plan.hip
--- a/audian_amd/csrc/sos_plan.hip
+++ b/audian_amd/csrc/sos_plan.hip
@@ -40,14 +40,79 @@
     return n;
 }
 
-void cascade_step(const double coef[MAXS][5], int S, double *z, double x)
-{
-    double cur = x;
+template <class R>
+R cascade_step(const double coef[MAXS][5], int S, R *z, R x)
+{
+    R cur = x;
     for (int s = 0; s < S; s++) {
-        double y = coef[s][0] * cur + z[2 * s];
+        R y = coef[s][0] * cur + z[2 * s];
         z[2 * s] = coef[s][1] * cur - coef[s][3] * y + z[2 * s + 1];
         z[2 * s + 1] = coef[s][2] * cur - coef[s][4] * y;
         cur = y;
+    }
+    return cur;
+}
+
+void fill_border_tables(SosPlanDev *p, int S)
+{
+    typedef long double R;
+    const int D = 2 * S;
+    R A[MAXD][MAXD], B[MAXD], C[MAXD], d;
+    for (int c = 0; c < D; c++) {
+        R z[MAXD] = {0};
+        z[c] = 1;
+        C[c] = cascade_step<R>(p->coef, S, z, 0);
+        for (int r = 0; r < D; r++) A[r][c] = z[r];
+    }
+    {
+        R z[MAXD] = {0};
+        d = cascade_step<R>(p->coef, S, z, 1);
+        for (int r = 0; r < D; r++) B[r] = z[r];
+    }
+    auto mul = [D](const R (&x)[MAXD][MAXD], const R (&y)[MAXD][MAXD], R (&o)[MAXD][MAXD]) {
+        R t[MAXD][MAXD];
+        for (int i = 0; i < D; i++)
+            for (int j = 0; j < D; j++) {
+                R s = 0;
+                for (int k = 0; k < D; k++) s += x[i][k] * y[k][j];
+                t[i][j] = s;
+            }
+        for (int i = 0; i < D; i++)
+            for (int j = 0; j < D; j++) o[i][j] = t[i][j];
+    };
+    R psi[MAXD][MAXD], P[MAXD][MAXD], t[MAXD][MAXD];
+    for (int i = 0; i < D; i++)
+        for (int j = 0; j < D; j++) { psi[i][j] = B[i] * C[j]; P[i][j] = A[i][j]; }
+    for (int it = 0; it < 64; it++) {
+        mul(P, psi, t);
+        mul(t, P, t);
+        for (int i = 0; i < D; i++)
+            for (int j = 0; j < D; j++) psi[i][j] += t[i][j];
+        mul(P, P, P);
+    }
+    R g[MAXD];
+    for (int i = 0; i < D; i++) {
+        R s = 0;
+        for (int j = 0; j < D; j++) s += psi[i][j] * B[j];
+        g[i] = s;
+    }
+    R g0[MAXD];
+    for (int i = 0; i < D; i++) {
+        R s = d * B[i];
+        for (int j = 0; j < D; j++) s += A[i][j] * g[j];
+        g0[i] = s;
+    }
+    for (int i = 0; i < D; i++)
+        for (int j = 0; j < D; j++) p->Psi[i * D + j] = (double)psi[i][j];
+    for (int j = 0; j < L; j++) {
+        for (int r = 0; r < D; r++) p->Gb[j * D + r] = (double)g0[r];
+        R n[MAXD];
+        for (int r = 0; r < D; r++) {
+            R s = 0;
+            for (int c = 0; c < D; c++) s += A[r][c] * g0[c];
+            n[r] = s;
+        }
+        for (int r = 0; r < D; r++) g0[r] = n[r];
     }
 }
 
@@ -78,12 +143,12 @@
     for (int c = 0; c < D; c++) {
         double z[MAXD] = {0};
         z[c] = 1.0;
-        cascade_step(p->coef, S, z, 0.0);
+        cascade_step<double>(p->coef, S, z, 0.0);
         for (int r = 0; r < D; r++) A.v[r][c] = z[r];
     }
     {
         double z[MAXD] = {0};
-        cascade_step(p->coef, S, z, 1.0);
+        cascade_step<double>(p->coef, S, z, 1.0);
         for (int r = 0; r < D; r++) B[r] = z[r];
     }
     {
@@ -130,6 +195,7 @@
         m = q + 1;
     }
     p->warm = m * TILE;
+    if (p->warm < (1LL << 40)) fill_border_tables(p, S);
     double scale = 1.0;
     for (int s = 0; s < S; s++) {
         const double *c = sos + 6 * s;
@@ -224,6 +290,26 @@
     return HIPDSP_OK;
 }
 
+int hipdsp_sos_border_host(const double *host_sos, int n_sections, double *psi, double *gamma0, double *gb)
+{
+    HD_REQUIRE(host_sos != nullptr, "host_sos is NULL");
+    if (n_sections < 1 || n_sections > MAXS) {
+        hipdsp_set_error("n_sections %d not in 1..%d", n_sections, MAXS);
+        return HIPDSP_ERR_UNSUPPORTED;
+    }
+    SosPlanDev tmp;
+    int rc = fill_plan(&tmp, host_sos, n_sections);
+    if (rc != HIPDSP_OK) return rc;
+    const int D = 2 * n_sections;
+    if (psi)
+        for (int k = 0; k < D * D; k++) psi[k] = tmp.Psi[k];
+    if (gamma0)
+        for (int k = 0; k < D; k++) gamma0[k] = tmp.Gb[k];
+    if (gb)
+        for (int k = 0; k < L * D; k++) gb[k] = tmp.Gb[k];
+    return HIPDSP_OK;
+}
+
 int hipdsp_sos_segments_host(int64_t n_cus, int waves_max, int per_simd, int max_segments, int64_t frames,
                              int64_t channels, int64_t warmup, int64_t *segment_frames, int *n_segments)
 {
diff --git a/audian_amd/hipdsp.py b/audian_amd/hipdsp.py
--- a/audian_amd/hipdsp.py
+++ b/audian_amd/hipdsp.py
@@ -30,6 +30,11 @@
 
     def set_option(self, name, value):
         check(lib.hipdsp_ctx_set_option(self._h, name.encode(), int(value)))
+
+    def envelope_sweep_info(self):
+        n, seg, warm, exact = ctypes.c_int64(), ctypes.c_int64(), ctypes.c_int64(), ctypes.c_int()
+        check(lib.hipdsp_envelope_sweep_info(self._h, ctypes.byref(n), ctypes.byref(seg), ctypes.byref(warm), ctypes.byref(exact)))
+        return int(n.value), int(seg.value), int(warm.value), bool(exact.value)
 
     def set_mid_event(self, ev):
         check(lib.hipdsp_ctx_set_mid_event(self._h, ev if ev is not None else ctypes.c_void_p(0)))
diff --git a/include/hip_dsp.h b/include/hip_dsp.h
--- a/include/hip_dsp.h
+++ b/include/hip_dsp.h
@@ -33,6 +33,8 @@
 int hipdsp_ctx_synchronize(hipdsp_ctx *ctx);
 int hipdsp_ctx_set_max_segments(hipdsp_ctx *ctx, int max_segments);
 int hipdsp_ctx_set_option(hipdsp_ctx *ctx, const char *name, long long value);
+int hipdsp_envelope_sweep_info(hipdsp_ctx *ctx, int64_t *n_segments, int64_t *segment_tiles, int64_t *warmup_tiles,
+                               int *from_border_states);
 int hipdsp_ctx_reserve(hipdsp_ctx *ctx, size_t bytes);
 
 
@@ -90,6 +92,7 @@
 int hipdsp_sosplan_upload(hipdsp_ctx *ctx, hipdsp_sosplan *plan);
 int hipdsp_sos_plan_host(const double *host_sos, int n_sections, int64_t *warmup, int *edge,
                          double *zi);
+int hipdsp_sos_border_host(const double *host_sos, int n_sections, double *psi, double *gamma0, double *gb);
 int hipdsp_sos_segments_host(int64_t n_cus, int waves_max, int per_simd, int max_segments, int64_t frames,
                              int64_t channels, int64_t warmup, int64_t *segment_frames,
                              int *n_segments);
```
